# wenet-e2e/wesep

Hardware: AMD Instinct MI355X
Metric: utterances/sec (4 s, 16 kHz, 2-spk) fwd+bwd, pBSRNN (higher is better)
Workload: dtype bf16x3+fp16x2+fp16x1 split products (+fp8 lo terms), fp32 accumulate; 1 GPU; pBSRNN FiLM multi-fuse, 6 repeats, feature_dim 128, fixed 256-d embeddings; fwd + SI-SDR + bwd + per-tensor clip + Adam-L2; bf16x3 (x-projections, projections, d(hcat), BN / mask GEMMs) + fp16x2 (recurrent products of all four recurrence kernels, d(xn)) + fp16x1 (LSTM weight gradients); 2-byte saved gates / d(gates); fp32 accumulate; BPTT kernels: W_hh as fp16 hi + block-scaled FP8 lo; the lo term; rows_per_gpu=32, global_rows=32, samples_per_row=64000, parallelism=dp1

## Files before the change

### include/wesep_hip.h

```cpp
#ifndef WESEP_HIP_H_
#define WESEP_HIP_H_

#ifdef __cplusplus
extern "C" {
#endif

#define WS_ABI_VERSION 20
#define WS_OK 0
#define WS_ERR_INVALID (-1)
#define WS_ERR_LAUNCH (-2)

int ws_abi_version(void);
const char* ws_last_error(void);

#define WS_PROF_LSTM_FWD 0
#define WS_PROF_LSTM_BWD 1
#define WS_PROF_GEMM_NT 2
#define WS_PROF_GEMM_TN 3
#define WS_PROF_NKINDS 4
int ws_prof_enable(int on);
int ws_prof_collect(int kind, double* total_ms, long long* launches);
int ws_debug_dirty_lds(float value, int nblocks, int spins, float* sink, void* stream);
int ws_debug_occupy(int nblocks, int usec, const unsigned* stop, float* sink, void* stream);

// ... 123 lines not shown
                            float* pout, unsigned* counter, float* fslab, float* da, float* db, unsigned* fcounter,
                            void* stream);

typedef struct ws_lstm_args {
  float* gates;
  float* cbuf;
  float* hcat;
  const float* dhcat;
  const float* wpack;
  long long sq_s1, sq_s2, step_rows;
  int nseq, sq_div, L, mode;
  const unsigned* run_if;
  const float* gates_in;
  float* dgates;
  int gfmt;
  int rfmt;
  const unsigned* amax;
  float* dxn;
  long long dxn_dir_stride;
  const float* wxpack;
} ws_lstm_args;
#define WS_GATES_F32 0
#define WS_GATES_H2 1
#define WS_GATES_H2S 2
#define WS_GATES_H2F 3
#define WS_DGATES_EXP 8
#define WS_LSTM_F32_MT1 1
#define WS_LSTM_F32_MT2 2
#define WS_LSTM_BF16X3 3
#define WS_LSTM_BF16X3_BLK 4
#define WS_LSTM_BF16X3_BLK16 5
#define WS_LSTM_H 256
#define WS_LSTM_FWD_H2P 16
#define WS_LSTM_PACK_FLOATS (2 * 4 * WS_LSTM_H * WS_LSTM_H)
int ws_lstm_pack(const float* whh_f, const float* whh_r, float* pack_fwd, float* pack_bwd,
                 int mode, void* stream);
int ws_lstm_pack_bwd_f8(const float* whh_f, const float* whh_r, float* pack_bwd, void* stream);
#define WS_LSTM_DX_PACK_FLOATS (16 * (48 * 1024 + 64) / 4)
int ws_lstm_pack_dx_f8(const float* wcat, float* pack, void* stream);
int ws_lstm_fwd(const ws_lstm_args* a, void* stream);
int ws_lstm_bwd(const ws_lstm_args* a, void* stream);
typedef struct ws_lstm_cluster_args {
  float* gates;
  float* cbuf;
  float* hcat;
  const float* dhcat;
  const float* whh_f;
  const float* whh_r;
  void* xchg;
  unsigned* flags;
  unsigned* status;
  int nseq, L;
  int dbg, gfmt;
  const float* gates_in;
} ws_lstm_cluster_args;
int ws_lstm_fwd_cluster(const ws_lstm_cluster_args* a, void* stream);
typedef struct ws_lstm_cluster2_args {
  float* gates;
  float* cbuf;
  float* hcat;
  const float* xn;
  const float* wcat;
  const float* bcat;
  const float* whh_f;
  const float* whh_r;
  void* xchg;
// ... 433 lines not shown
```

### wesep_amd/_lib.py

```python
import ctypes as C
import os

import numpy as np
import torch

_HERE = os.path.dirname(os.path.abspath(__file__))
LIB_PATH = os.environ.get("WESEP_HIP_LIB") or os.path.join(_HERE, "libwesep_hip.so")

WS_OK = 0
PROF_LSTM_FWD, PROF_LSTM_BWD, PROF_GEMM_NT, PROF_GEMM_TN = 0, 1, 2, 3
LSTM_H = 256
ABI_VERSION = 20
GATES_F32, GATES_H2, GATES_H2S, GATES_H2F = 0, 1, 2, 3
DGATES_EXP = 8


def dgates_scale(amax_bits: int) -> float:
    e = (int(amax_bits) >> 23) & 0xFF
    return 1.0 if e in (0, 255) else 2.0 ** (min(max(DGATES_EXP + 254 - e, 1), 253) - 127)


LSTM_F32_MT1, LSTM_F32_MT2, LSTM_BF16X3, LSTM_BF16X3_BLK, LSTM_BF16X3_BLK16 = 1, 2, 3, 4, 5
LSTM_FWD_H2P = 16
LSTM_PACK_FLOATS = 2 * 4 * LSTM_H * LSTM_H

_p = C.c_void_p
_ll = C.c_longlong
_i = C.c_int
_f = C.c_float


class ConvView(C.Structure):
    _fields_ = [(n, _i) for n in ("on", "mode", "H", "W", "C", "Ho", "Wo", "k", "sh", "sw", "p", "dil", "ldp")]


class Conv3x3PackSrc(C.Structure):
    _fields_ = [("w", _p), ("s_row", _ll), ("s_col", _ll), ("s_tap", _ll), ("col_off", _i), ("cols", _i)]


class Conv3x3PackArgs(C.Structure):
    _fields_ = [("src", Conv3x3PackSrc * 5), ("out", _p), ("Cin", _i), ("Cout", _i), ("nsrc", _i), ("flip", _i)]


class Conv3x3Args(C.Structure):
    _fields_ = [(n, _p) for n in ("X", "W", "bias", "R", "Y")] + [(n, _ll) for n in ("ldx", "ldw", "ldy")] + \
               [(n, _i) for n in ("B", "H", "Wd", "Cin", "Cout", "pad_")]


class Conv3x3WgradArgs(C.Structure):
    _fields_ = [(n, _p) for n in ("G", "X", "slab", "bslab")] + [(n, _ll) for n in ("ldg", "ldx", "slab_stride", "bslab_stride")] + \
               [(n, _i) for n in ("B", "H", "Wd", "Wx", "sw", "Cin", "Nn", "nsplit", "tiles_per_split", "pad_")]


class HeadsArgs(C.Structure):
    _fields_ = [(n, _p) for n in ("x", "dy", "slope", "gamma", "beta", "y", "stats", "dx", "slab")] + \
               [(n, _ll) for n in ("ldx", "lddx")] + [(n, _i) for n in ("B", "T", "Tp", "Q", "nh", "ch", "nwg")] + \
# ... 331 lines not shown
```

### wesep_amd/blstm_core.py

```python
import math
import os
from typing import NamedTuple

import numpy as np
import torch

from . import _lib as L
from . import dev

H = L.LSTM_H
G4 = 4 * H
N = 128


def _empty(dev_, *shape):
    return torch.empty(*shape, device=dev_, dtype=torch.float32)


def _reduce_new(slab, nsplit, stride, shape):
    out = _empty(slab.device, *shape)
    dev.reduce_slabs(slab, nsplit, stride, int(np.prod(shape)), out)
    return out


# ... 295 lines not shown
            return out
        if kind in ("wihT", "wihT16", "wihT8"):
            out = _empty(d, N * 2 * G4)
            dev.pack_w(W("cat")[0], N, 2 * G4, N, out, trans=True, order=1, f16={"wihT": 0, "wihT16": 1, "wihT8": 2}[kind])
            return out
        if kind == "pw":
            return proj_w.contiguous()
        if kind in ("proj", "proj16"):
            out = _empty(d, N * 2 * H)
            dev.pack_w(W("pw"), N, 2 * H, 2 * H, out, order=1, f16=kind == "proj16")
            return out
        if kind == "projT":
            out = _empty(d, 2 * H * N)
            dev.pack_w(W("pw"), 2 * H, N, 2 * H, out, trans=True, order=0)
            return out
        raise KeyError(kind)


class BlstmPlan(NamedTuple):
    nb: int
    lmode: int
    cluster: bool
    fwd: str
    bptt: str
    grad: bool
    gfmt: int
    g_fmt: int
    a16: bool
    pair_rfmt: int
    band_rfmt: int
    band_dx: bool
    a_fmt: int
    h2p: bool = False


_WIHT_KIND = {0: "wihT", 1: "wihT", 2: "wihT16", 3: "wihT8"}


def make_plan(seq, device, grad, gn_geo=None, ragged=False) -> BlstmPlan:
    lmode = dev.lstm_blk_mode(seq.nseq)
    cluster = dev.lstm_cluster_ok(seq, device)
    bptt = _bptt_kind(seq, device, cluster)
    gfmt = L.GATES_F32 if bptt == "cluster" else dev.gates_fmt()
    h2 = gfmt != L.GATES_F32
    if ragged:
        fwd = "cluster" if cluster else "stream"
    elif dev.lstm_fuse_ok(seq.nseq, cluster):
        fwd = "fused"
    elif cluster:
        fwd = "cluster2" if h2 and dev.lstm_cluster2_on() else "cluster"
    else:
        fwd = "stream"
    g_fmt = {L.GATES_H2: 1, L.GATES_H2F: 2}.get(gfmt, 0)
    brf = band_rfmt(gfmt, lmode) if grad and bptt == "stream" else 0
    a16 = gfmt == L.GATES_H2F and grad and tnb_a16()
    h2p = (a16 and dev.h2p_on(device) and not ragged and fwd in ("fused", "cluster2", "stream")
           and (fwd != "fused" or bool(dev.lstm_fused_hfmt(gfmt) & 1)))
    return BlstmPlan(
        nb=dev.bl_num_blocks(seq), lmode=lmode, cluster=cluster, fwd=fwd, bptt=bptt, grad=grad, gfmt=gfmt, g_fmt=g_fmt,
        a16=a16, pair_rfmt=pair_rfmt(gfmt) if grad and bptt == "pair" else 0,
        band_rfmt=brf, band_dx=bool(brf) and gn_geo is not None and band_dx(brf, seq, gn_geo), a_fmt=dxn_fmt(g_fmt), h2p=h2p)


def consume_once(ctx, who):
    if ctx.consumed:
        raise L.WesepHipError(f"{who}: second backward through the same graph (retain_graph / multi-loss loops): "
                              "the blocked path consumes its saved gates in place; run the forward again")
    ctx.consumed = True


def blstm_forward(plan, W, x, seq, res, bias, norm=None, steps=None, film=None):
    d = x.device
    norm = dict(norm or {})
    if film is not None:
        if res is not x or steps is not None:
            raise L.WesepHipError("blstm_forward: film= folds ONE affine into operand and residual (res is x), no step counts")
        norm["film"] = film
    rk = dict(film=film) if film is not None else {}
    if steps is not None and (plan.fwd in ("fused", "cluster2") or plan.grad):
        raise L.WesepHipError(f"blstm_forward: per-sequence step counts with forward branch '{plan.fwd}', grad={plan.grad}: "
                              "only the branches over precomputed gates know them, and only the forward")
    lens = dict(steps=steps[0], steps_div=steps[1]) if steps is not None else {}
    nb, gfmt, lmode = plan.nb, plan.gfmt, plan.lmode
    h2 = gfmt != L.GATES_F32
    wcat, bcat = W("cat")
    whf, whr = W("whh")
    xn = _empty(d, nb, 32 * N)
    cbuf, hcat = _empty(d, nb, 32 * 2 * H), _empty(d, nb, 32 * 2 * H)
    gates = _empty(d, dev.blh_floats(nb, 2 * G4)) if h2 else _empty(d, nb, 32 * 2 * G4)
    xn16 = _empty(d, dev.blh_floats(nb, N)) if plan.a16 else None
    h2p = plan.h2p
    planes = dict(h2p=True) if h2p else {}
    hcat16 = _empty(d, dev.blh_floats(nb, 2 * H)) if plan.a16 and not h2p else None
    if plan.fwd == "fused":
        dev.gemm_p2b(A=x, lda=N, sm=seq, Wpack=None, N=0, C_out=None, A_bl=xn, A_bl16=xn16, **norm)
        hf = dev.lstm_fused_hfmt(gfmt)
        dev.lstm_fwd_fused(gates, cbuf, hcat, xn, W("fused8" if hf & 4 else "fused16" if hf else "fused"), bcat, seq, gfmt=gfmt,
                           hfmt=hf | (8 if h2p else 0))
    elif plan.fwd == "cluster2":
        dev.gemm_p2b(A=x, lda=N, sm=seq, Wpack=None, N=0, C_out=None, A_bl=xn, A_bl16=xn16, **norm)
        tw = dev.lstm_fwd_cluster2(gates, cbuf, hcat, xn, wcat, bcat, whf, whr, seq, dbg=_cluster_dbg(), **planes)
        pre = dev.fallback_scratch(d, nb * 32 * 2 * G4)
        dev.gemm_p2b(A=x, lda=N, sm=seq, Wpack=W("wih"), N=2 * G4, C_out=pre, bias=bcat, run_if=tw, **norm)
        dev.lstm_fwd(gates, cbuf, hcat, W("hh")[0], seq, lmode, run_if=tw, gfmt=gfmt, gates_in=pre, **planes)
        del pre
    else:
        pre = _empty(d, nb, 32 * 2 * G4) if h2 else gates
        xproj = dict(A=x, lda=N, sm=seq, Wpack=W("wih"), N=2 * G4, C_out=pre, bias=bcat, A_bl=xn, A_bl16=xn16, **norm, **lens)
        rec = dict(gfmt=gfmt, gates_in=pre) if h2 else {}
        dev.gemm_p2b(**xproj)
        if _h2_probe() & 768 and not torch.cuda.is_available():
            pre.copy_(pre.half().float() if _h2_probe() & 256 else pre.bfloat16().float())
        if plan.fwd == "cluster":
            tw = dev.lstm_fwd_cluster(gates, cbuf, hcat, whf, whr, seq, dbg=_cluster_dbg(), **rec)
            if not h2:
                dev.gemm_p2b(run_if=tw, **xproj)
            dev.lstm_fwd(gates, cbuf, hcat, W("hh")[0], seq, lmode, run_if=tw, **rec)
        else:
            dev.lstm_fwd(gates, cbuf, hcat, W("hh")[0], seq, lmode, **planes, **rec)
        del pre
    out = torch.empty_like(res)
    if h2p:
        dev.gemm_b2p(A=hcat, K=2 * H, sm=seq, Wpack=W("proj16"), C_out=out, ldc=N, bias=bias, R=res, a_fmt=4, **rk)
    else:
        dev.gemm_b2p(A=hcat, K=2 * H, sm=seq, Wpack=W("proj"), C_out=out, ldc=N, bias=bias, R=res, a16_out=hcat16, **rk)
    if _h2_probe() and not h2:
        if _h2_probe() & 1:
            _probe_round(gates, "f16")
        if _h2_probe() & 8:
            _probe_round(gates, "u16")
        if _h2_probe() & 4:
            _probe_round(cbuf, "f16")
    if plan.grad:
        W("projT")
        if not plan.band_dx:
            W(_WIHT_KIND[plan.a_fmt])
        if plan.bptt == "pair":
            W("hhp16" if plan.pair_rfmt else "hhp")
        if (plan.bptt == "stream" and not plan.band_rfmt) or (plan.bptt == "pair" and h2):
            W("hh")
        if plan.bptt == "stream" and plan.band_rfmt:
            W("hh8")
            if plan.band_dx:
                W("wx8")
    return out, (gates, cbuf, hcat, xn16 if plan.a16 else xn, hcat16)


def blstm_bptt(plan, W, gates, cbuf, hcat, dout, seq, release):
    d = dout.device
    nb, gfmt = plan.nb, plan.gfmt
    dh, dout_bl = _empty(d, nb, 32 * 2 * H), _empty(d, nb, 32 * N)
    dxn2 = None
    amax = amax_word(d) if gfmt == L.GATES_H2F else None
    dev.gemm_p2b(A=dout, lda=N, sm=seq, Wpack=W("projT"), N=2 * H, C_out=dh, A_bl=dout_bl, amax=amax)
    if _h2_probe() & 16:
        _probe_round(dh, "bf16")
    ready = mark_wgrads_ready(d) if release else None
    if plan.bptt == "cluster":
        dg = gates
        dev.lstm_bwd_cluster(gates, cbuf, dh, *W("whh"), seq)
    elif gfmt == L.GATES_F32:
        dg = gates
        if plan.bptt == "pair":
            dev.lstm_bwd_pair(gates, cbuf, dh, W("hhp"), seq, dbg=_pair_dbg())
        else:
            dev.lstm_bwd(gates, cbuf, hcat, dh, W("hh")[1], seq, plan.lmode)
    elif plan.bptt == "pair":
        dg = _empty(d, nb, 32 * 2 * G4) if gfmt == L.GATES_H2S else _empty(d, dev.blh_floats(nb, 2 * G4))
        rf = plan.pair_rfmt
        tw = dev.lstm_bwd_pair(gates, cbuf, dh, W("hhp16" if rf else "hhp"), seq, gfmt=gfmt, dgates=dg, repairable=True,
                               dbg=_pair_dbg(), amax=amax, rfmt=rf, dbg_buf=_pair_stamp_buf(d, seq.L))
        dev.lstm_bwd(gates, cbuf, hcat, dh, W("hh")[1], seq, plan.lmode, gfmt=gfmt, dgates=dg, run_if=tw, amax=amax)
    else:
        dg = _empty(d, nb, 32 * 2 * G4) if gfmt == L.GATES_H2S else gates
        brf = plan.band_rfmt
        if plan.band_dx:
            dxn2 = _empty(d, 2, dout.numel() // N, N)
        dev.lstm_bwd(gates, cbuf, hcat, dh, W("hh8") if brf else W("hh")[1], seq, plan.lmode, gfmt=gfmt,
                     dgates=dg if gfmt == L.GATES_H2S else None, amax=amax, rfmt=brf, dxn=dxn2,
                     wxpack=W("wx8") if dxn2 is not None else None)
    if _h2_probe() & 2 and gfmt == L.GATES_F32:
        _probe_round(gates, "bf16", packed=True)
    if _h2_probe() & 32 and gfmt == L.GATES_F32 and not torch.cuda.is_available():
        amax = float(dh.abs().max())
        S = 2.0 ** (10 - math.floor(math.log2(amax))) if amax > 0 and math.isfinite(amax) else 1.0
        sc = gates * S
        _PROBE_SAT[0] += int((sc.abs() > 65504.0).sum())
        _PROBE_SAT[1] = max(_PROBE_SAT[1], float(sc.abs().max()) / 65504.0)
        gates.copy_(sc.clamp(-65504.0, 65504.0).half().float() / S)
    if ready is not None:
        flush_deferred_wgrads(d, ready)
    return dg, dout_bl, amax, dxn2


def weight_grads(gates, xn, hcat, dout_bl, seq, nb, g_fmt=0, amax=None, hcat16=None, h2p=False):
    d = gates.device
    if h2p:
        hcat16 = dev.h2p_hi(hcat, nb)
    a_fmt = 1 if hcat16 is not None else 0
    if _h2_probe() & 192 and not torch.cuda.is_available() and not a_fmt:
        rnd = (lambda t: t.half().float()) if _h2_probe() & 64 else (lambda t: t.bfloat16().float())
        xn, hcat = rnd(xn), rnd(hcat)
    if os.environ.get("WESEP_PROBE_SKIP_WGRAD") == "1":
        z_ = lambda *s_: torch.zeros(*s_, device=d)
        return [z_(G4, N), z_(G4, H), z_(G4), z_(G4), z_(G4, N), z_(G4, H), z_(G4), z_(G4), z_(N, 2 * H), z_(N)]
    if _h2_probe() & 1024 and not torch.cuda.is_available() and amax is not None:
        S = L.dgates_scale(int(amax.reshape(-1)[0]))
        hcat = hcat.half().float()
        dout_bl = (dout_bl * S).half().float() / S
    ns, bps = dev.tnb_splits(nb, (2 * H) // 128)
    slab, aslab = _empty(d, ns, 2 * H * N), _empty(d, ns, N)
    if h2p:
        dev.gemm_tnb_h16(G=hcat16, g_width=2 * H, g_off=0, g_cols=2 * H, A0=dout_bl, a0_width=N, a0_off=0, nblk=nb, L_=seq.L,
# ... 45 lines not shown
```

### wesep_amd/csrc/lstm.hip

```cpp
#include "common.h"

#define LH WS_LSTM_H
#define LG (4 * LH)
#define HL_LD 68
#define DG_LD 260

__device__ __forceinline__ f32x4 mfma16(float a, float b, f32x4 c) {
  return __builtin_amdgcn_mfma_f32_16x16x4f32(a, b, c, 0, 0, 0);
}

__device__ __forceinline__ float fast_sigmoid(float x) {
  return __builtin_amdgcn_rcpf(1.f + __expf(-x));
}
__device__ __forceinline__ float fast_tanh(float x) {
  const float ax = fabsf(x);
  const float e = __expf(-2.f * ax);
  const float t = (1.f - e) * __builtin_amdgcn_rcpf(1.f + e);
  return copysignf(t, x);
}

__global__ void lstm_pack_kernel(const float* __restrict__ whh_f, const float* __restrict__ whh_r,
                                 float* __restrict__ pf, float* __restrict__ pb) {
  const int total = 2 * LG * LH;
  for (int idx = blockIdx.x * blockDim.x + threadIdx.x; idx < total; idx += gridDim.x * blockDim.x) {
// ... 316 lines not shown
      f32x4 a[MT];
#pragma unroll
      for (int mt = 0; mt < MT; ++mt)
        a[mt] = *reinterpret_cast<const f32x4*>(arow + mt * (64 * DG_LD) + 4 * ks4);
#pragma unroll
      for (int q = 0; q < 4; ++q)
#pragma unroll
        for (int s = 0; s < 2; ++s)
#pragma unroll
          for (int mt = 0; mt < MT; ++mt) dh[mt][s] = mfma16(a[mt][q], bcur[s][q], dh[mt][s]);
      bcur[0] = bnxt[0];
      bcur[1] = bnxt[1];
    }
    __syncthreads();
  }
}

static int lstm_check(const ws_lstm_args* a, bool bwd, const char* who) {
  WS_REQUIRE(a && a->gates && a->cbuf && a->hcat && a->wpack, "%s: null pointer", who);
  WS_REQUIRE(!bwd || a->dhcat, "%s: null dhcat", who);
  WS_REQUIRE(a->nseq > 0 && a->L > 0 && a->sq_div > 0, "%s: bad nseq/L/sq_div", who);
  WS_REQUIRE((a->mode & 255) >= WS_LSTM_F32_MT1 && (a->mode & 255) <= WS_LSTM_BF16X3_BLK16, "%s: bad mode %d", who,
             a->mode);
  WS_REQUIRE(!a->run_if || (!bwd && (a->mode & 255) >= WS_LSTM_BF16X3) || (bwd && (a->mode & 255) >= WS_LSTM_BF16X3_BLK),
             "%s: run_if is honoured by the split-bf16 forward kernels and the blocked-layout BPTT kernels only", who);
  WS_REQUIRE(a->gfmt >= WS_GATES_F32 && a->gfmt <= WS_GATES_H2F, "%s: bad gfmt %d", who, a->gfmt);
  WS_REQUIRE(a->gfmt != WS_GATES_H2F || !bwd || a->amax, "%s: WS_GATES_H2F needs amax", who);
  WS_REQUIRE(a->gfmt == WS_GATES_F32 || (a->mode & 255) >= WS_LSTM_BF16X3_BLK,
             "%s: gfmt %d is a format of the blocked-layout modes", who, a->gfmt);
  WS_REQUIRE(a->gfmt == WS_GATES_F32 || bwd || a->gates_in, "%s: gfmt %d needs gates_in (the fp32 pre-activations)", who,
             a->gfmt);
  WS_REQUIRE(a->gfmt != WS_GATES_H2S || !bwd || a->dgates, "%s: WS_GATES_H2S needs dgates", who);
  WS_REQUIRE(a->gfmt == WS_GATES_F32 || ((a->mode >> 8) & 7) == 0, "%s: probe builds are WS_GATES_F32 only", who);
  WS_REQUIRE(a->rfmt == 0 || ((a->rfmt == 2 || a->rfmt == 3) && bwd && a->mode == WS_LSTM_BF16X3_BLK && a->gfmt == WS_GATES_H2F) ||
                 (a->rfmt == WS_LSTM_FWD_H2P && !bwd && (a->mode == WS_LSTM_BF16X3_BLK || a->mode == WS_LSTM_BF16X3_BLK16)),
             "%s: rfmt %d (2 / 3 = fp16 recurrence on fp16 + FP8 weights, 3: the lo term on the FP8 MFMA: ws_lstm_bwd, "
             "WS_LSTM_BF16X3_BLK, WS_GATES_H2F only; 16 = hcat out as two fp16 planes: ws_lstm_fwd, blocked-layout modes only)",
             who, a->rfmt);
  WS_REQUIRE(!a->dxn || (bwd && a->rfmt == 2 && a->wxpack && a->dxn_dir_stride > 0 && a->dxn_dir_stride < (1ll << 29) && !a->run_if),
             "%s: dxn (d(xn) inside the BPTT, ABI v19) needs rfmt 2, wxpack (ws_lstm_pack_dx_f8), 0 < dxn_dir_stride < 2^29 floats "
             "(32-bit store offsets) and no run_if", who);
  return WS_OK;
}

extern "C" int ws_lstm_fwd(const ws_lstm_args* a, void* stream) {
  int rc = lstm_check(a, false, "ws_lstm_fwd");
  if (rc != WS_OK) return rc;
  hipStream_t s = (hipStream_t)stream;
  const int per = 16 * a->mode;
  dim3 grid((a->nseq + per - 1) / per, 2), block(512);
  const bool timed = a->run_if == nullptr;
  if (timed) ws_prof_begin(WS_PROF_LSTM_FWD, s);
  if ((a->mode & 255) == WS_LSTM_BF16X3_BLK16)
    ws_launch_lstm_fwd_s16(a, s);
  else if ((a->mode & 255) >= WS_LSTM_BF16X3)
    ws_launch_lstm_fwd_bf16(a, s);
  else if (a->mode == WS_LSTM_F32_MT1)
    hipLaunchKernelGGL((lstm_fwd_kernel<1>), grid, block, 0, s, *a);
  else
    hipLaunchKernelGGL((lstm_fwd_kernel<2>), grid, block, 0, s, *a);
  if (timed) ws_prof_end(WS_PROF_LSTM_FWD, s);
  return ws_check_launch("ws_lstm_fwd");
}

extern "C" int ws_lstm_bwd(const ws_lstm_args* a, void* stream) {
  int rc = lstm_check(a, true, "ws_lstm_bwd");
  if (rc != WS_OK) return rc;
  hipStream_t s = (hipStream_t)stream;
  const int per = 16 * a->mode;
  dim3 grid((a->nseq + per - 1) / per, 2), block(512);
  const bool timed = a->run_if == nullptr;
  if (timed) ws_prof_begin(WS_PROF_LSTM_BWD, s);
// ... 12 lines not shown
```

### wesep_amd/csrc/lstm_bf16.hip

```cpp
#include <stdlib.h>

#include "lstm_bf16_common.h"

__global__ void lstm_pack_bf16_kernel(const float* __restrict__ whh_f, const float* __restrict__ whh_r,
                                      __bf16* __restrict__ pf, __bf16* __restrict__ pb) {
  const int total = 2 * LG * LH;
  for (int idx = blockIdx.x * blockDim.x + threadIdx.x; idx < total; idx += gridDim.x * blockDim.x) {
    {
      int r = idx;
      const int j = r & 7; r >>= 3;
      const int lane = r & 63; r >>= 6;
      const int g = r & 3; r >>= 2;
      const int ks = r & 15; r >>= 4;
      const int w = r & 7; r >>= 3;
      const int d = r;
      const float* W = d ? whh_r : whh_f;
      const int row = g * 256 + 32 * w + (lane & 31);
      const int k = 16 * ks + 8 * (lane >> 5) + j;
      const float v = W[row * LH + k];
      const __bf16 hi = (__bf16)v;
      const long long unit = ((((long long)(d * 8 + w) * 16 + ks) * 4 + g) * 2) * 64 + lane;
      pf[unit * 8 + j] = hi;
      pf[(unit + 64) * 8 + j] = (__bf16)(v - (float)hi);
    }
// ... 82 lines not shown
    v0[i] = 256.f * W[row * 128 + u];
    v1[i] = 256.f * W[(row + 1) * 128 + u];
    m = fmaxf(m, fmaxf(fabsf(v0[i]), fabsf(v1[i])));
  }
#pragma unroll
  for (int o = 32; o > 0; o >>= 1) m = fmaxf(m, __shfl_xor(m, o));
  if ((tid & 63) == 0) red[tid >> 6] = m;
  __syncthreads();
  m = red[0];
#pragma unroll
  for (int i = 1; i < 8; ++i) m = fmaxf(m, red[i]);
  const int eb = (int)((__builtin_bit_cast(unsigned, m) >> 23) & 0xffu);
  const float S = (eb > 19 && eb < 255) ? __builtin_bit_cast(float, (unsigned)(eb - 19) << 23) : 1.f;
  char* ob = px + (long long)(d * 8 + w) * WS_DX_REGION;
  if (tid == 0) reinterpret_cast<float*>(ob + 48 * 1024)[grp] = S;
#pragma unroll
  for (int i = 0; i < 2; ++i) {
    const int pi = tid + 512 * i, j2 = pi & 3, lane = (pi >> 2) & 63, f = pi >> 8;
    const _Float16 h0 = (_Float16)v0[i], h1 = (_Float16)v1[i];
    typedef _Float16 f16x2 __attribute__((ext_vector_type(2)));
    typedef short s16x2 __attribute__((ext_vector_type(2)));
    char* cb = ob + (2 * grp + (f >> 1)) * 3072;
    *reinterpret_cast<f16x2*>(cb + (f & 1) * 1024 + lane * 16 + j2 * 4) = f16x2{h0, h1};
    const s16x2 c = __builtin_amdgcn_cvt_scalef32_pk_fp8_f32(s16x2{0, 0}, v0[i] - (float)h0, v1[i] - (float)h1, S, false);
    *reinterpret_cast<short*>(cb + 2048 + (f & 1) * 512 + lane * 8 + j2 * 2) = c[0];
  }
}

int ws_launch_lstm_pack_dx_f8(const float* wcat, float* pack, hipStream_t s) {
  hipLaunchKernelGGL(lstm_pack_dx_f8_kernel, dim3(128), dim3(512), 0, s, wcat, reinterpret_cast<char*>(pack));
  return 0;
}

template <bool BLK, int DBG, int GF = 0, bool H2P = false>
__global__ __launch_bounds__(512, 2) void lstm_fwd_bf16_kernel(const ws_lstm_args p) {
  static_assert(!H2P || (BLK && DBG == 0), "the fp16 planes are a format of the blocked layout");
  __shared__ __attribute__((aligned(16))) __bf16 hl[2][2][SQ * HROW];
  __shared__ __attribute__((aligned(16))) float cl[SQ * (LH + 4)];
  if (p.run_if && *p.run_if == 0u) return;
  const int d = blockIdx.y;
  const int tid = threadIdx.x, lane = tid & 63, l31 = lane & 31, half = lane >> 5;
  const int w = __builtin_amdgcn_readfirstlane(tid >> 6);
  const int L = p.L;

  {
    uint32_t* z = reinterpret_cast<uint32_t*>(&hl[0][0][0]);
    for (int i = tid; i < 2 * SQ * HROW / 2; i += 512) z[i] = 0u;
  }
  const int ss = min((int)blockIdx.x * SQ + l31, p.nseq - 1);
  const long long rowbase =
      BLK ? 0 : (long long)(ss / p.sq_div) * p.sq_s1 + (long long)(ss % p.sq_div) * p.sq_s2;
  const int ubase = 32 * w + 4 * half;
  const int glane = ((d * 256 + 8 * w + half) * 32 + l31) * 16;
  const int clane = ((d * 64 + 8 * w + half) * 32 + l31) * 16;
  auto goff = [&](int t, int g, int j) -> long long {
    return ((rowbase + (long long)t * p.step_rows) * 2 + d) * LG + g * 256 + ubase + 8 * j;
  };
  auto coff = [&](int t, int j) -> long long {
    return (rowbase + (long long)t * p.step_rows) * (2 * LH) + d * LH + ubase + 8 * j;
  };
  const float* gsrc = GF ? p.gates_in : p.gates;
  auto grs = [&](int t) { return mkrsrc(gsrc + (long long)(blockIdx.x * L + t) * (SQ * 2 * LG), SQ * 2 * LG * 4); };
  auto hrs = [&](int t) { return mkrsrc(p.gates + (long long)(blockIdx.x * L + t) * (SQ * LG), SQ * 2 * LG * 2); };
  auto crs = [&](float* b, int t) { return mkrsrc(b + (long long)(blockIdx.x * L + t) * (SQ * 2 * LH), SQ * 2 * LH * 4); };
  const char* hplane = reinterpret_cast<const char*>(p.hcat);
  const long long hlo_off = ws_h2p_plane((long long)gridDim.x * L);
  auto prs = [&](int t, int pl) {
    return mkrsrc(reinterpret_cast<const float*>(hplane + pl * hlo_off + (long long)(blockIdx.x * L + t) * (SQ * 2 * LH * 2)),
                  SQ * 2 * LH * 2);
  };
  auto ld_gate = [&](int t, int g, int j) -> f32x4 {
    if constexpr (BLK) return bld(grs(t), glane, (g * 64 + 2 * j) * 512);
    else return *reinterpret_cast<const f32x4*>(p.gates + goff(t, g, j));
  };
  auto st_gate = [&](const f32x4& v, int t, int g, int j) {
    if constexpr (GF != 0) bst8(g == 2 ? enc_u16x4<true>(v) : enc_u16x4<false>(v), hrs(t), glane >> 1, (g * 64 + 2 * j) * 256);
    else if constexpr (BLK) bst(v, grs(t), glane, (g * 64 + 2 * j) * 512);
    else *reinterpret_cast<f32x4*>(p.gates + goff(t, g, j)) = v;
  };
  auto st_ch = [&](const f32x4& v, float* b, int t, int j) {
    if constexpr (BLK) bst(v, crs(b, t), clane, 2 * j * 512);
    else *reinterpret_cast<f32x4*>(b + coff(t, j)) = v;
  };

  float* cme = &cl[l31 * (LH + 4) + ubase];
#pragma unroll
  for (int j = 0; j < 4; ++j) *reinterpret_cast<f32x4*>(cme + 8 * j) = f32x4{0.f, 0.f, 0.f, 0.f};

  const __amdgpu_buffer_rsrc_t wrs = __builtin_amdgcn_make_buffer_rsrc(
      const_cast<float*>(p.wpack) + (long long)(d * 8 + w) * (16 * 8 * 64 * 4), 0, 16 * 8 * 1024, 0x00020000);
  const int wlane = lane * 16;
  bf16x8 wr[2][8];
#pragma unroll
  for (int s = 0; s < 2; ++s)
#pragma unroll
    for (int f = 0; f < 8; ++f) wr[s][f] = wload(wrs, wlane + (f & 3) * 1024, s * 8192 + (f >> 2) * 4096);

  f32x4 xg[4][4];
  {
    const int t0 = d == 0 ? 0 : L - 1;
#pragma unroll
    for (int gi = 0; gi < 4; ++gi)
#pragma unroll
// ... 55 lines not shown
#pragma unroll
    for (int j = 0; j < 4; ++j) {
      f32x4 pre[4];
#pragma unroll
      for (int g = 0; g < 4; ++g)
#pragma unroll
        for (int r = 0; r < 4; ++r) pre[g][r] = acc[g][4 * j + r];
      f32x4 vi, vf, vg, vo, vc, vh;
      const f32x4 cold = *reinterpret_cast<const f32x4*>(cme + 8 * j);
#pragma unroll
      for (int r = 0; r < 4; ++r) {
        const float ig = fsig(pre[0][r]);
        const float fg = fsig(pre[1][r]);
        const float gg = ftanh(pre[2][r]);
        const float og = fsig(pre[3][r]);
        const float cn = fg * cold[r] + ig * gg;
        vi[r] = ig;
        vf[r] = fg;
        vg[r] = gg;
        vo[r] = og;
        vc[r] = cn;
        vh[r] = og * ftanh(cn);
      }
      bf16x4 h_hi, h_lo;
      split4(vh, h_hi, h_lo);
      *reinterpret_cast<bf16x4*>(nhi + 8 * j) = h_hi;
      *reinterpret_cast<bf16x4*>(nlo + 8 * j) = h_lo;
      *reinterpret_cast<f32x4*>(cme + 8 * j) = vc;
      if (!(DBG & 1) || step == L - 1) {
        st_gate(vi, t, 0, j);
        st_gate(vf, t, 1, j);
        st_gate(vg, t, 2, j);
        st_gate(vo, t, 3, j);
        st_ch(vc, p.cbuf, t, j);
        if constexpr (H2P) {
          u32x2 ph, pl;
          enc_h2p(vh, ph, pl);
          bst8(ph, prs(t, 0), clane >> 1, j * 512);
          bst8(pl, prs(t, 1), clane >> 1, j * 512);
        } else if constexpr (BLK) st_ch(pack_hl4(h_hi, h_lo), p.hcat, t, j);
        else st_ch(vh, p.hcat, t, j);
      }
      __builtin_amdgcn_sched_barrier(0);
    }
    __syncthreads();
  }
}

template <bool BLK, int DBG, int GF = 0, int RF = 0, bool DX = false>
__global__ __launch_bounds__(512, 2) void lstm_bwd_bf16_kernel(const ws_lstm_args p) {
  static_assert(RF == 0 || (BLK && GF == WS_GATES_H2F), "the fp16 recurrence takes the scaled-fp16 d(gates) of WS_GATES_H2F");
  static_assert(!DX || RF == 2, "d(xn) in the BPTT rides on the fp16 d(gates) image of rfmt 2");
  __shared__ __attribute__((aligned(16))) __bf16 dgl[RF ? 1 : 2][SQ * DROW];
  __shared__ __attribute__((aligned(16))) f32x4 xred[DX ? 8 * 2 * 64 : 1];
  if (p.run_if && *p.run_if == 0u) return;
  const int d = blockIdx.y, bx = blockIdx.x;
  const int tid = threadIdx.x, lane = tid & 63, l31 = lane & 31, half = lane >> 5;
  const int w = __builtin_amdgcn_readfirstlane(tid >> 6);
  const int L = p.L;
  const int ss = min(bx * SQ + l31, p.nseq - 1);
  const long long rowbase =
      BLK ? 0 : (long long)(ss / p.sq_div) * p.sq_s1 + (long long)(ss % p.sq_div) * p.sq_s2;
  const int ubase = 32 * w + 4 * half;
  const int glane = ((d * 256 + 8 * w + half) * 32 + l31) * 16;
  const int clane = ((d * 64 + 8 * w + half) * 32 + l31) * 16;
  auto goff = [&](int t, int g, int j) -> long long {
    return ((rowbase + (long long)t * p.step_rows) * 2 + d) * LG + g * 256 + ubase + 8 * j;
  };
  auto coff = [&](int t, int j) -> long long {
    return (rowbase + (long long)t * p.step_rows) * (2 * LH) + d * LH + ubase + 8 * j;
  };
  float* gdst = GF == WS_GATES_H2S ? p.dgates : p.gates;
  auto grs = [&](int t) { return mkrsrc(gdst + (long long)(bx * L + t) * (SQ * 2 * LG), SQ * 2 * LG * 4); };
  auto hrs = [&](int t) { return mkrsrc(p.gates + (long long)(bx * L + t) * (SQ * LG), SQ * 2 * LG * 2); };
  constexpr bool G2 = GF == WS_GATES_H2 || GF == WS_GATES_H2F;
  float* hdst = (G2 && p.dgates) ? p.dgates : p.gates;
  auto ors = [&](int t) { return mkrsrc(hdst + (long long)(bx * L + t) * (SQ * LG), SQ * 2 * LG * 2); };
  const float dS = GF == WS_GATES_H2F ? ws_dgates_scale(*p.amax) : 1.f;
  auto crs = [&](const float* b, int t) { return mkrsrc(b + (long long)(bx * L + t) * (SQ * 2 * LH), SQ * 2 * LH * 4); };
  typedef typename gate_cell<GF>::type gcell;
  auto ld_gate = [&](int t, int g, int j) -> gcell {
    if constexpr (GF != 0) return bld8(hrs(t), glane >> 1, (g * 64 + 2 * j) * 256);
    else if constexpr (BLK) return bld(grs(t), glane, (g * 64 + 2 * j) * 512);
    else return *reinterpret_cast<const f32x4*>(p.gates + goff(t, g, j));
  };
  auto st_gate = [&](const f32x4& v, int t, int g, int j) {
    if constexpr (BLK) bst(v, grs(t), glane, (g * 64 + 2 * j) * 512);
    else *reinterpret_cast<f32x4*>(p.gates + goff(t, g, j)) = v;
  };
  auto ld_ch = [&](const float* b, int t, int j) -> f32x4 {
    if constexpr (BLK) return bld(crs(b, t), clane, 2 * j * 512);
    else return *reinterpret_cast<const f32x4*>(b + coff(t, j));
  };

  const int kpar = DX ? (w >> 2) : 0;
  const __amdgpu_buffer_rsrc_t wrs = __builtin_amdgcn_make_buffer_rsrc(
      const_cast<float*>(p.wpack) + (long long)(d * 8 + w) * (64 * 2 * 64 * 4), 0, 64 * 2 * 1024, 0x00020000);
  const int wlane = lane * 16;
  bf16x8 wr[2][RF ? 4 : 8];
  u32x2 wq[2][RF ? 4 : 1];
  float wS[RF ? 8 : 1];
  int wE[RF == 3 ? 8 : 1];
  auto wfill = [&](int s, int chunk, int zo) {
    if constexpr (RF != 0) {
#pragma unroll
      for (int q = 0; q < 4; ++q) {
        const int fq = q ^ kpar;
        wr[s][q] = wload(wrs, wlane, zo + chunk * 6144 + fq * 1024);
        wq[s][q] = __builtin_bit_cast(u32x2, __builtin_amdgcn_raw_buffer_load_b64(wrs, lane * 8, zo + chunk * 6144 + 4096 + fq * 512, 0));
      }
    } else {
#pragma unroll
      for (int f = 0; f < 8; ++f) wr[s][f] = wload(wrs, wlane + (f & 3) * 1024, zo + chunk * 8192 + (f >> 2) * 4096);
    }
  };
  typedef _Float16 f16x8 __attribute__((ext_vector_type(8)));
  typedef _Float16 f16x2 __attribute__((ext_vector_type(2)));
  const __amdgpu_buffer_rsrc_t xrs = __builtin_amdgcn_make_buffer_rsrc(
      const_cast<char*>(reinterpret_cast<const char*>(p.wxpack)) + (DX ? (long long)(d * 8 + w) * WS_DX_REGION : 0), 0,
      DX ? WS_DX_REGION : 0, 0x00020000);
  bf16x8 xr[2][DX ? 2 : 1];
  u32x2 xq[2][DX ? 2 : 1];
  float xS[DX ? 8 : 1];
  f32x16 dxa;
  auto xfill = [&](int s, int chunk, int zo) {
    if constexpr (DX) {
#pragma unroll
      for (int q = 0; q < 2; ++q) {
        xr[s][q] = wload(xrs, wlane + q * 1024, zo + chunk * 3072);
        xq[s][q] = __builtin_bit_cast(u32x2, __builtin_amdgcn_raw_buffer_load_b64(xrs, lane * 8 + q * 512, zo + chunk * 3072 + 2048, 0));
      }
    }
  };
  if constexpr (RF != 0) {
    const float* st = p.wpack + (long long)(d * 8 + w) * (64 * 2 * 64 * 4) + 96 * 256;
#pragma unroll
    for (int g8 = 0; g8 < 8; ++g8) wS[g8] = __builtin_bit_cast(float, __builtin_amdgcn_readfirstlane(__builtin_bit_cast(int, st[g8])));
    if constexpr (RF == 3) {
#pragma unroll
      for (int g8 = 0; g8 < 8; ++g8) wE[g8] = (__builtin_bit_cast(int, wS[g8]) >> 23) & 255;
    }
  }
  if constexpr (DX) {
    const float* st = reinterpret_cast<const float*>(reinterpret_cast<const char*>(p.wxpack) + (long long)(d * 8 + w) * WS_DX_REGION + 48 * 1024);
#pragma unroll
    for (int g8 = 0; g8 < 8; ++g8) xS[g8] = __builtin_bit_cast(float, __builtin_amdgcn_readfirstlane(__builtin_bit_cast(int, st[g8])));
  }
  unsigned xoff = 0u;
  if constexpr (DX) {
    const int sq = bx * SQ + l31;
    const long long row = (long long)(sq / p.sq_div) * p.sq_s1 + (long long)(sq % p.sq_div) * p.sq_s2;
    xoff = sq < p.nseq ? (unsigned)(row * 512 + (32 * (w & 3) + 16 * kpar + 4 * half) * 4) : 0x80000000u;
  }
  const __amdgpu_buffer_rsrc_t xors = __builtin_amdgcn_make_buffer_rsrc(
      DX ? p.dxn + (long long)d * p.dxn_dir_stride : nullptr, 0, DX ? (unsigned)(p.dxn_dir_stride * 4) : 0u, 0x00020000);
  gcell n_i[4], n_f[4], n_g[4], n_o[4];
  f32x4 n_dh[4], n_cp[4], c_cur[4], dc[4];
  f32x16 dhr;
  const f32x4 zero4v = {0.f, 0.f, 0.f, 0.f};
#pragma unroll
  for (int j = 0; j < 4; ++j) dc[j] = zero4v;
#pragma unroll
  for (int i = 0; i < 16; ++i) dhr[i] = 0.f;

  auto load_step = [&](int t, int j) {
    n_i[j] = ld_gate(t, 0, j);
    n_f[j] = ld_gate(t, 1, j);
    n_g[j] = ld_gate(t, 2, j);
    n_o[j] = ld_gate(t, 3, j);
    n_dh[j] = ld_ch(p.dhcat, t, j);
    const int tp = d == 0 ? max(t - 1, 0) : min(t + 1, L - 1);
    n_cp[j] = ld_ch(p.cbuf, tp, j);
  };
  {
    const int t0 = d == 0 ? L - 1 : 0;
#pragma unroll
    for (int j = 0; j < 4; ++j) {
      load_step(t0, j);
      c_cur[j] = ld_ch(p.cbuf, t0, j);
    }
  }
  __builtin_amdgcn_sched_barrier(0);
  wfill(0, 0, 0);
  xfill(0, 0, 0);
  wfill(1, 1, 0);
  xfill(1, 1, 0);
  __builtin_amdgcn_sched_barrier(0);

  for (int step = 0; step < L; ++step) {
    const int t = d == 0 ? L - 1 - step : step;
    const int sn = min(step + 1, L - 1);
    const int tn = d == 0 ? L - 1 - sn : sn;
    const bool has_prev = d == 0 ? (t > 0) : (t < L - 1);
    int zo = 0;
    asm volatile("" : "+s"(zo));
    __bf16* dhi = &dgl[0][l31 * DROW + ubase];
    __bf16* dlo = &dgl[RF ? 0 : 1][l31 * DROW + ubase];
#pragma unroll
    for (int j = 0; j < 4; ++j) {
      f32x4 pi, pf, pg, po;
      const f32x4 vi = gate_val<false>(n_i[j]), vf = gate_val<false>(n_f[j]), vg = gate_val<true>(n_g[j]),
                  vo = gate_val<false>(n_o[j]);
#pragma unroll
      for (int r = 0; r < 4; ++r) {
        const float ig = vi[r], fg = vf[r], gg = vg[r], og = vo[r];
        const float dhv = dh_in<GF>(n_dh[j][r], dhr[4 * j + r], dS);
        const float tc = ftanh(c_cur[j][r]);
        const float dov = dhv * tc;
        const float dcv = dc[j][r] + dhv * og * (1.f - tc * tc);
        dc[j][r] = dcv * fg;
        pi[r] = dcv * gg * ig * (1.f - ig);
        pf[r] = dcv * (has_prev ? n_cp[j][r] : 0.f) * fg * (1.f - fg);
        pg[r] = dcv * ig * (1.f - gg * gg);
        po[r] = dov * og * (1.f - og);
      }
      c_cur[j] = n_cp[j];
      const bool st = !(DBG & 1) || step == L - 1;
      auto emit = [&](const f32x4& v, int g) {
        if constexpr (RF != 0) {
          const u32x2 code = enc_f16x4(v);
          *reinterpret_cast<u32x2*>(dhi + 256 * g + 8 * j) = code;
          if (st) bst8(code, ors(t), glane >> 1, (g * 64 + 2 * j) * 256);
          return;
        }
        bf16x4 hi, lo;
        split4(v, hi, lo);
        *reinterpret_cast<bf16x4*>(dhi + 256 * g + 8 * j) = hi;
        *reinterpret_cast<bf16x4*>(dlo + 256 * g + 8 * j) = lo;
        if (st) {
          if constexpr (G2) bst8(enc_dgates<GF>(v, hi), ors(t), glane >> 1, (g * 64 + 2 * j) * 256);
          else if constexpr (BLK) st_gate(pack_hl4(hi, lo), t, g, j);
          else st_gate(v, t, g, j);
        }
      };
      emit(pi, 0);
      emit(pf, 1);
      emit(pg, 2);
      emit(po, 3);
      if (!(DBG & 2)) load_step(tn, j);
      __builtin_amdgcn_sched_barrier(0);
    }
    __syncthreads();

    const __bf16* bhi = &dgl[0][l31 * DROW + 8 * half];
    const __bf16* blo = &dgl[RF ? 0 : 1][l31 * DROW + 8 * half];
// ... 98 lines not shown
    if constexpr (DX) {
      const float us = (1.f / 256.f) / dS;
      const unsigned trow = (unsigned)t * (unsigned)p.step_rows * 512u;
#pragma unroll
      for (int i = 0; i < 2; ++i) {
        const f32x4 o = xred[((w ^ 4) * 2 + i) * 64 + lane];
        __builtin_amdgcn_raw_buffer_store_b128(__builtin_bit_cast(u32x4, (keep[i] + o) * us), xors, xoff + trow + 32 * i, 0, 0);
      }
    }
  }
}

#define WS_DBG_DISPATCH(KERNEL)                                                          \
  if ((a->mode & 255) == WS_LSTM_BF16X3_BLK && a->gfmt == WS_GATES_H2) {                 \
    hipLaunchKernelGGL((KERNEL<true, 0, WS_GATES_H2>), grid, block, 0, s, *a);           \
  } else if ((a->mode & 255) == WS_LSTM_BF16X3_BLK && a->gfmt == WS_GATES_H2S) {         \
    hipLaunchKernelGGL((KERNEL<true, 0, WS_GATES_H2S>), grid, block, 0, s, *a);          \
  } else if ((a->mode & 255) == WS_LSTM_BF16X3_BLK && a->gfmt == WS_GATES_H2F) {         \
    hipLaunchKernelGGL((KERNEL<true, 0, WS_GATES_H2F>), grid, block, 0, s, *a);          \
  } else if ((a->mode & 255) == WS_LSTM_BF16X3_BLK) {                                    \
    switch ((a->mode >> 8) & 7) {                                                        \
      case 0: hipLaunchKernelGGL((KERNEL<true, 0>), grid, block, 0, s, *a); break;       \
      case 1: hipLaunchKernelGGL((KERNEL<true, 1>), grid, block, 0, s, *a); break;       \
      case 2: hipLaunchKernelGGL((KERNEL<true, 2>), grid, block, 0, s, *a); break;       \
      case 4: hipLaunchKernelGGL((KERNEL<true, 4>), grid, block, 0, s, *a); break;       \
      default: hipLaunchKernelGGL((KERNEL<true, 7>), grid, block, 0, s, *a); break;      \
    }                                                                                    \
  } else {                                                                               \
    hipLaunchKernelGGL((KERNEL<false, 0>), grid, block, 0, s, *a);                       \
  }

int ws_launch_lstm_fwd_bf16(const ws_lstm_args* a, hipStream_t s) {
  dim3 grid((a->nseq + SQ - 1) / SQ, 2), block(512);
  if (a->rfmt == WS_LSTM_FWD_H2P) {
    if (a->gfmt == WS_GATES_H2) hipLaunchKernelGGL((lstm_fwd_bf16_kernel<true, 0, WS_GATES_H2, true>), grid, block, 0, s, *a);
    else if (a->gfmt == WS_GATES_H2S) hipLaunchKernelGGL((lstm_fwd_bf16_kernel<true, 0, WS_GATES_H2S, true>), grid, block, 0, s, *a);
    else if (a->gfmt == WS_GATES_H2F) hipLaunchKernelGGL((lstm_fwd_bf16_kernel<true, 0, WS_GATES_H2F, true>), grid, block, 0, s, *a);
    else hipLaunchKernelGGL((lstm_fwd_bf16_kernel<true, 0, 0, true>), grid, block, 0, s, *a);
    return 0;
  }
  WS_DBG_DISPATCH(lstm_fwd_bf16_kernel)
  return 0;
}

int ws_launch_lstm_bwd_bf16(const ws_lstm_args* a, hipStream_t s) {
  dim3 grid((a->nseq + SQ - 1) / SQ, 2), block(512);
  if (a->rfmt == 2 && a->dxn) {
    hipLaunchKernelGGL((lstm_bwd_bf16_kernel<true, 0, WS_GATES_H2F, 2, true>), grid, block, 0, s, *a);
    return 0;
  }
  if (a->rfmt == 2) {
    hipLaunchKernelGGL((lstm_bwd_bf16_kernel<true, 0, WS_GATES_H2F, 2>), grid, block, 0, s, *a);
    return 0;
  }
  if (a->rfmt == 3) {
    hipLaunchKernelGGL((lstm_bwd_bf16_kernel<true, 0, WS_GATES_H2F, 3>), grid, block, 0, s, *a);
    return 0;
  }
  WS_DBG_DISPATCH(lstm_bwd_bf16_kernel)
  return 0;
}
```

### wesep_amd/csrc/lstm_bf16_common.h

```cpp
#pragma once
#include "common.h"

typedef __bf16 bf16x8 __attribute__((ext_vector_type(8)));
typedef __bf16 bf16x4 __attribute__((ext_vector_type(4)));

#define LH WS_LSTM_H
#define LG (4 * LH)
#define SQ 32
#define HROW 264
#define DROW 1032

typedef unsigned int u32x4 __attribute__((ext_vector_type(4)));

__device__ __forceinline__ bf16x8 wload(__amdgpu_buffer_rsrc_t rsrc, int voff, int soff) {
  return __builtin_bit_cast(bf16x8, __builtin_amdgcn_raw_buffer_load_b128(rsrc, voff, soff, 0));
}

__device__ __forceinline__ __amdgpu_buffer_rsrc_t mkrsrc(const float* base, unsigned bytes) {
  return __builtin_amdgcn_make_buffer_rsrc(const_cast<float*>(base), 0, bytes, 0x00020000);
}
#ifndef WS_STREAM_AUX
#define WS_STREAM_AUX 2
#endif
__device__ __forceinline__ f32x4 bld(__amdgpu_buffer_rsrc_t r, int voff, int soff) {
// ... 79 lines not shown
}
template <bool TANH>
__device__ __forceinline__ f32x4 dec_u16x4(const u32x2& c) {
  const float s = TANH ? 1.f / WS_U16_TANH : 1.f / WS_U16_SIG, o = TANH ? -1.f : 0.f;
  f32x4 v;
  v[0] = __builtin_fmaf((float)(c[0] & 0xffffu), s, o);
  v[1] = __builtin_fmaf((float)(c[0] >> 16), s, o);
  v[2] = __builtin_fmaf((float)(c[1] & 0xffffu), s, o);
  v[3] = __builtin_fmaf((float)(c[1] >> 16), s, o);
  return v;
}
__device__ __forceinline__ u32x2 bf16x4_bits(const bf16x4& v) { return __builtin_bit_cast(u32x2, v); }
typedef _Float16 f16x4 __attribute__((ext_vector_type(4)));
__device__ __forceinline__ u32x2 enc_f16x4(const f32x4& vs) {
  f16x4 h;
#pragma unroll
  for (int j = 0; j < 4; ++j) h[j] = (_Float16)vs[j];
  return __builtin_bit_cast(u32x2, h);
}
__device__ __forceinline__ void enc_h2p(const f32x4& vh, u32x2& hi, u32x2& lo) {
  f16x4 h, l;
#pragma unroll
  for (int j = 0; j < 4; ++j) {
    float x = vh[j];
    asm volatile("" : "+v"(x));
    h[j] = (_Float16)x;
    l[j] = (_Float16)(x - (float)h[j]);
  }
  hi = __builtin_bit_cast(u32x2, h);
  lo = __builtin_bit_cast(u32x2, l);
}
__device__ __forceinline__ long long ws_h2p_plane(long long nblk) { return nblk * (SQ * 2 * LH * 2); }

template <int GF>
__device__ __forceinline__ u32x2 enc_dgates(const f32x4& v, const bf16x4& hi) {
  if constexpr (GF == WS_GATES_H2F) return enc_f16x4(v);
  else return bf16x4_bits(hi);
}
template <int GF>
__device__ __forceinline__ float dh_in(float dh, float rec, float S) {
  if constexpr (GF == WS_GATES_H2F) return __builtin_fmaf(dh, S, rec);
  else return dh + rec;
}

template <int GF> struct gate_cell { typedef f32x4 type; };
template <> struct gate_cell<WS_GATES_H2> { typedef u32x2 type; };
template <> struct gate_cell<WS_GATES_H2S> { typedef u32x2 type; };
template <> struct gate_cell<WS_GATES_H2F> { typedef u32x2 type; };
template <bool TANH> __device__ __forceinline__ f32x4 gate_val(const f32x4& c) { return c; }
template <bool TANH> __device__ __forceinline__ f32x4 gate_val(const u32x2& c) { return dec_u16x4<TANH>(c); }
```

### wesep_amd/csrc/lstm_bf16_s16.hip

```cpp
#include "lstm_bf16_common.h"

#define S16 16

__device__ __forceinline__ f32x4 mfma16(bf16x8 a, bf16x8 b, f32x4 c) {
  return __builtin_amdgcn_mfma_f32_16x16x32_bf16(a, b, c, 0, 0, 0);
}

__global__ void lstm_pack_s16_kernel(const float* __restrict__ whh_f, const float* __restrict__ whh_r,
                                     __bf16* __restrict__ pf, __bf16* __restrict__ pb) {
  const int total = 2 * LG * LH;
  for (int idx = blockIdx.x * blockDim.x + threadIdx.x; idx < total; idx += gridDim.x * blockDim.x) {
    {
      int r = idx;
      const int j = r & 7; r >>= 3;
      const int lane = r & 63; r >>= 6;
      const int tile = r & 7; r >>= 3;
      const int ks = r & 7; r >>= 3;
      const int w = r & 7; r >>= 3;
      const int d = r;
      const float* W = d ? whh_r : whh_f;
      const int row = (tile >> 1) * 256 + 32 * w + 16 * (tile & 1) + (lane & 15);
      const int k = 32 * ks + 8 * (lane >> 4) + j;
      const float v = W[row * LH + k];
      const __bf16 hi = (__bf16)v;
      const long long unit = ((((long long)(d * 8 + w) * 8 + ks) * 8 + tile) * 2) * 64 + lane;
      pf[unit * 8 + j] = hi;
      pf[(unit + 64) * 8 + j] = (__bf16)(v - (float)hi);
    }
    {
      int r = idx;
      const int j = r & 7; r >>= 3;
      const int lane = r & 63; r >>= 6;
      const int tu = r & 1; r >>= 1;
      const int ks = r & 31; r >>= 5;
      const int w = r & 7; r >>= 3;
      const int d = r;
      const float* W = d ? whh_r : whh_f;
      const int row = 32 * ks + 8 * (lane >> 4) + j;
      const int u = 32 * w + 16 * tu + (lane & 15);
      const float v = W[row * LH + u];
      const __bf16 hi = (__bf16)v;
      const long long unit = ((((long long)(d * 8 + w) * 32 + ks) * 2 + tu) * 2) * 64 + lane;
      pb[unit * 8 + j] = hi;
      pb[(unit + 64) * 8 + j] = (__bf16)(v - (float)hi);
    }
  }
}

int ws_launch_lstm_pack_s16(const float* whh_f, const float* whh_r, float* pack_fwd, float* pack_bwd,
                            hipStream_t s) {
  hipLaunchKernelGGL(lstm_pack_s16_kernel, dim3(512), dim3(256), 0, s, whh_f, whh_r,
                     reinterpret_cast<__bf16*>(pack_fwd), reinterpret_cast<__bf16*>(pack_bwd));
  return 0;
}

template <int GF, bool H2P = false>
__global__ __launch_bounds__(512, 2) void lstm_fwd_s16_kernel(const ws_lstm_args p) {
  __shared__ __attribute__((aligned(16))) __bf16 hl[2][2][S16 * HROW];
  __shared__ __attribute__((aligned(16))) float cl[S16 * (LH + 4)];
  if (p.run_if && *p.run_if == 0u) return;
  const int d = blockIdx.y;
  const int tile = blockIdx.x >> 1, hb = blockIdx.x & 1;
  const int tid = threadIdx.x, lane = tid & 63, n = lane & 15, mq = lane >> 4;
  const int w = __builtin_amdgcn_readfirstlane(tid >> 6);
  const int L = p.L;
  {
    uint32_t* z = reinterpret_cast<uint32_t*>(&hl[0][0][0]);
    for (int i = tid; i < 2 * S16 * HROW / 2; i += 512) z[i] = 0u;
  }
  const int glane = ((d * 256 + 8 * w + mq) * 32 + 16 * hb + n) * 16;
  const int clane = ((d * 64 + 8 * w + mq) * 32 + 16 * hb + n) * 16;
  const float* gsrc = GF ? p.gates_in : p.gates;
  auto grs = [&](int t) { return mkrsrc(gsrc + (long long)(tile * L + t) * (SQ * 2 * LG), SQ * 2 * LG * 4); };
  auto hrs = [&](int t) { return mkrsrc(p.gates + (long long)(tile * L + t) * (SQ * LG), SQ * 2 * LG * 2); };
  auto crs = [&](float* b, int t) { return mkrsrc(b + (long long)(tile * L + t) * (SQ * 2 * LH), SQ * 2 * LH * 4); };
  auto ld_gate = [&](int t, int g, int tu) -> f32x4 { return bld(grs(t), glane, (g * 64 + 4 * tu) * 512); };
  auto st_gate = [&](const f32x4& v, int t, int g, int tu) {
    if constexpr (GF != 0) bst8(g == 2 ? enc_u16x4<true>(v) : enc_u16x4<false>(v), hrs(t), glane >> 1, (g * 64 + 4 * tu) * 256);
    else bst(v, grs(t), glane, (g * 64 + 4 * tu) * 512);
  };
  auto st_ch = [&](const f32x4& v, float* b, int t, int tu) { bst(v, crs(b, t), clane, 4 * tu * 512); };
  const char* hplane = reinterpret_cast<const char*>(p.hcat);
  const long long hlo_off = ws_h2p_plane((long long)(gridDim.x >> 1) * L);
  auto prs = [&](int t, int pl) {
    return mkrsrc(reinterpret_cast<const float*>(hplane + pl * hlo_off + (long long)(tile * L + t) * (SQ * 2 * LH * 2)), SQ * 2 * LH * 2);
  };

  const int ubase = 32 * w + 4 * mq;
  float* cme = &cl[n * (LH + 4) + ubase];
#pragma unroll
  for (int tu = 0; tu < 2; ++tu) *reinterpret_cast<f32x4*>(cme + 16 * tu) = f32x4{0.f, 0.f, 0.f, 0.f};

  const __amdgpu_buffer_rsrc_t wrs = __builtin_amdgcn_make_buffer_rsrc(
      const_cast<float*>(p.wpack) + (long long)(d * 8 + w) * (8 * 16 * 64 * 4), 0, 8 * 16 * 1024, 0x00020000);
  const int wlane = lane * 16;
  bf16x8 wr[2][16];
#pragma unroll
  for (int s = 0; s < 2; ++s)
#pragma unroll
    for (int f = 0; f < 16; ++f) wr[s][f] = wload(wrs, wlane + (f & 3) * 1024, s * 16384 + (f >> 2) * 4096);

  f32x4 xg[4][2];
  {
    const int t0 = d == 0 ? 0 : L - 1;
#pragma unroll
    for (int g = 0; g < 4; ++g)
#pragma unroll
      for (int tu = 0; tu < 2; ++tu) xg[g][tu] = ld_gate(t0, g, tu);
  }
  __syncthreads();

  for (int step = 0; step < L; ++step) {
    const int t = d == 0 ? step : L - 1 - step;
    const int cur = step & 1;
    int zo = 0;
    asm volatile("" : "+s"(zo));
    const __bf16* hhi = &hl[cur][0][n * HROW + 8 * mq];
    const __bf16* hlo = &hl[cur][1][n * HROW + 8 * mq];
    f32x4 acc[4][2];
// ... 39 lines not shown
    for (int tu = 0; tu < 2; ++tu)
#pragma unroll
      for (int g = 0; g < 4; ++g) xg[g][tu] = ld_gate(tn, g, tu);
    __builtin_amdgcn_sched_barrier(0);
    __bf16* nhi = &hl[cur ^ 1][0][n * HROW + ubase];
    __bf16* nlo = &hl[cur ^ 1][1][n * HROW + ubase];
#pragma unroll
    for (int tu = 0; tu < 2; ++tu) {
      f32x4 vi, vf, vg, vo, vc, vh;
      const f32x4 cold = *reinterpret_cast<const f32x4*>(cme + 16 * tu);
#pragma unroll
      for (int r = 0; r < 4; ++r) {
        const float ig = fsig(acc[0][tu][r]);
        const float fg = fsig(acc[1][tu][r]);
        const float gg = ftanh(acc[2][tu][r]);
        const float og = fsig(acc[3][tu][r]);
        const float cn = fg * cold[r] + ig * gg;
        vi[r] = ig;
        vf[r] = fg;
        vg[r] = gg;
        vo[r] = og;
        vc[r] = cn;
        vh[r] = og * ftanh(cn);
      }
      bf16x4 h_hi, h_lo;
      split4(vh, h_hi, h_lo);
      *reinterpret_cast<bf16x4*>(nhi + 16 * tu) = h_hi;
      *reinterpret_cast<bf16x4*>(nlo + 16 * tu) = h_lo;
      *reinterpret_cast<f32x4*>(cme + 16 * tu) = vc;
      st_gate(vi, t, 0, tu);
      st_gate(vf, t, 1, tu);
      st_gate(vg, t, 2, tu);
      st_gate(vo, t, 3, tu);
      st_ch(vc, p.cbuf, t, tu);
      if constexpr (H2P) {
        u32x2 ph, pl;
        enc_h2p(vh, ph, pl);
        bst8(ph, prs(t, 0), clane >> 1, 2 * tu * 512);
        bst8(pl, prs(t, 1), clane >> 1, 2 * tu * 512);
      } else {
        st_ch(pack_hl4(h_hi, h_lo), p.hcat, t, tu);
      }
      __builtin_amdgcn_sched_barrier(0);
    }
    __syncthreads();
  }
}


#ifndef S16_DBG
#define S16_DBG 0
#endif
template <int GF>
__global__ __launch_bounds__(512, 2) void lstm_bwd_s16_kernel(const ws_lstm_args p) {
  __shared__ __attribute__((aligned(16))) __bf16 dgl[2][S16 * DROW];
  if (p.run_if && *p.run_if == 0u) return;
  const int d = blockIdx.y;
  const int tile = blockIdx.x >> 1, hb = blockIdx.x & 1;
  const int tid = threadIdx.x, lane = tid & 63, n = lane & 15, mq = lane >> 4;
  const int w = __builtin_amdgcn_readfirstlane(tid >> 6);
  const int L = p.L;
  const int glane = ((d * 256 + 8 * w + mq) * 32 + 16 * hb + n) * 16;
  const int clane = ((d * 64 + 8 * w + mq) * 32 + 16 * hb + n) * 16;
  float* gdst = GF == WS_GATES_H2S ? p.dgates : p.gates;
  auto grs = [&](int t) { return mkrsrc(gdst + (long long)(tile * L + t) * (SQ * 2 * LG), SQ * 2 * LG * 4); };
  auto hrs = [&](int t) { return mkrsrc(p.gates + (long long)(tile * L + t) * (SQ * LG), SQ * 2 * LG * 2); };
  constexpr bool G2 = GF == WS_GATES_H2 || GF == WS_GATES_H2F;
  float* hdst = (G2 && p.dgates) ? p.dgates : p.gates;
  auto ors = [&](int t) { return mkrsrc(hdst + (long long)(tile * L + t) * (SQ * LG), SQ * 2 * LG * 2); };
  const float dS = GF == WS_GATES_H2F ? ws_dgates_scale(*p.amax) : 1.f;
  auto crs = [&](const float* b, int t) { return mkrsrc(b + (long long)(tile * L + t) * (SQ * 2 * LH), SQ * 2 * LH * 4); };
  typedef typename gate_cell<GF>::type gcell;
  auto ld_gate = [&](int t, int g, int tu) -> gcell {
    if constexpr (GF != 0) return bld8(hrs(t), glane >> 1, (g * 64 + 4 * tu) * 256);
    else return bld(grs(t), glane, (g * 64 + 4 * tu) * 512);
  };
  auto st_gate = [&](const f32x4& v, int t, int g, int tu) { bst(v, grs(t), glane, (g * 64 + 4 * tu) * 512); };
  auto ld_ch = [&](const float* b, int t, int tu) -> f32x4 { return bld(crs(b, t), clane, 4 * tu * 512); };
  const int ubase = 32 * w + 4 * mq;

  const __amdgpu_buffer_rsrc_t wrs = __builtin_amdgcn_make_buffer_rsrc(
      const_cast<float*>(p.wpack) + (long long)(d * 8 + w) * (32 * 4 * 64 * 4), 0, 32 * 4 * 1024, 0x00020000);
  const int wlane = lane * 16;
  bf16x8 wr[2][16];
#pragma unroll
  for (int s = 0; s < 2; ++s)
#pragma unroll
    for (int f = 0; f < 16; ++f) wr[s][f] = wload(wrs, wlane + (f & 3) * 1024, s * 16384 + (f >> 2) * 4096);

  gcell n_i[2], n_f[2], n_g[2], n_o[2];
  f32x4 n_dh[2], n_cp[2], c_cur[2], dc[2], dhr[2];
  const f32x4 zero4v = {0.f, 0.f, 0.f, 0.f};
#pragma unroll
  for (int tu = 0; tu < 2; ++tu) dc[tu] = dhr[tu] = zero4v;
  auto load_step = [&](int t, int tu) {
    n_i[tu] = ld_gate(t, 0, tu);
    n_f[tu] = ld_gate(t, 1, tu);
    n_g[tu] = ld_gate(t, 2, tu);
    n_o[tu] = ld_gate(t, 3, tu);
    n_dh[tu] = ld_ch(p.dhcat, t, tu);
    const int tp = d == 0 ? max(t - 1, 0) : min(t + 1, L - 1);
    n_cp[tu] = ld_ch(p.cbuf, tp, tu);
  };
  {
    const int t0 = d == 0 ? L - 1 : 0;
#pragma unroll
    for (int tu = 0; tu < 2; ++tu) {
      load_step(t0, tu);
      c_cur[tu] = ld_ch(p.cbuf, t0, tu);
    }
  }

  for (int step = 0; step < L; ++step) {
    const int t = d == 0 ? L - 1 - step : step;
    const int sn = min(step + 1, L - 1);
    const int tn = d == 0 ? L - 1 - sn : sn;
    const bool has_prev = d == 0 ? (t > 0) : (t < L - 1);
    int zo = 0;
    asm volatile("" : "+s"(zo));
    __bf16* dhi = &dgl[0][n * DROW + ubase];
    __bf16* dlo = &dgl[1][n * DROW + ubase];
#pragma unroll
    for (int tu = 0; tu < 2; ++tu) {
      f32x4 pi, pf, pg, po;
      const f32x4 vi = gate_val<false>(n_i[tu]), vf = gate_val<false>(n_f[tu]), vg = gate_val<true>(n_g[tu]),
                  vo = gate_val<false>(n_o[tu]);
#pragma unroll
      for (int r = 0; r < 4; ++r) {
        const float ig = vi[r], fg = vf[r], gg = vg[r], og = vo[r];
        const float dhv = dh_in<GF>(n_dh[tu][r], dhr[tu][r], dS);
        const float tc = ftanh(c_cur[tu][r]);
        const float dov = dhv * tc;
        const float dcv = dc[tu][r] + dhv * og * (1.f - tc * tc);
        dc[tu][r] = dcv * fg;
        pi[r] = dcv * gg * ig * (1.f - ig);
        pf[r] = dcv * (has_prev ? n_cp[tu][r] : 0.f) * fg * (1.f - fg);
        pg[r] = dcv * ig * (1.f - gg * gg);
        po[r] = dov * og * (1.f - og);
      }
      c_cur[tu] = n_cp[tu];
      auto emit = [&](const f32x4& v, int g) {
        bf16x4 hi, lo;
        split4(v, hi, lo);
        *reinterpret_cast<bf16x4*>(dhi + 256 * g + 16 * tu) = hi;
        *reinterpret_cast<bf16x4*>(dlo + 256 * g + 16 * tu) = lo;
        if constexpr (G2) bst8(enc_dgates<GF>(v, hi), ors(t), glane >> 1, (g * 64 + 4 * tu) * 256);
        else if (!(S16_DBG & 2)) st_gate(pack_hl4(hi, lo), t, g, tu);
      };
      emit(pi, 0);
      emit(pf, 1);
      emit(pg, 2);
      emit(po, 3);
      if (!(S16_DBG & 1)) load_step(tn, tu);
      __builtin_amdgcn_sched_barrier(0);
    }
    __syncthreads();

    const __bf16* bhi = &dgl[0][n * DROW + 8 * mq];
    const __bf16* blo = &dgl[1][n * DROW + 8 * mq];
    f32x4 acc[2];
#pragma unroll
    for (int ch = 0; ch < 8; ++ch) {
      const int s = ch & 1;
#pragma unroll
      for (int q = 0; q < 4; ++q) {
        const int ks = 4 * ch + q;
        const bf16x8 bh = *reinterpret_cast<const bf16x8*>(bhi + 32 * ks);
        const bf16x8 bl = *reinterpret_cast<const bf16x8*>(blo + 32 * ks);
#pragma unroll
        for (int tu = 0; tu < 2; ++tu) {
          const int f = (q * 2 + tu) * 2;
          if (ks == 0)
            acc[tu] = mfma16(wr[s][f], bh, zero4v);
          else
            acc[tu] = mfma16(wr[s][f], bh, acc[tu]);
        }
#pragma unroll
        for (int tu = 0; tu < 2; ++tu) acc[tu] = mfma16(wr[s][(q * 2 + tu) * 2 + 1], bh, acc[tu]);
#pragma unroll
        for (int tu = 0; tu < 2; ++tu) acc[tu] = mfma16(wr[s][(q * 2 + tu) * 2], bl, acc[tu]);
      }
      const int cn = (ch + 2) & 7;
      if (!(S16_DBG & 4)) {
#pragma unroll
      for (int f = 0; f < 16; ++f)
        wr[s][f] = wload(wrs, wlane + (f & 3) * 1024, zo + cn * 16384 + (f >> 2) * 4096);
      }
      __builtin_amdgcn_sched_barrier(0);
    }
    dhr[0] = acc[0];
    dhr[1] = acc[1];
    __syncthreads();
  }
}

int ws_launch_lstm_fwd_s16(const ws_lstm_args* a, hipStream_t s) {
  dim3 grid(2 * ((a->nseq + SQ - 1) / SQ), 2), block(512);
  const bool h2p = a->rfmt == WS_LSTM_FWD_H2P;
  if (a->gfmt && h2p) hipLaunchKernelGGL((lstm_fwd_s16_kernel<WS_GATES_H2, true>), grid, block, 0, s, *a);
  else if (h2p) hipLaunchKernelGGL((lstm_fwd_s16_kernel<0, true>), grid, block, 0, s, *a);
  else if (a->gfmt) hipLaunchKernelGGL(lstm_fwd_s16_kernel<WS_GATES_H2>, grid, block, 0, s, *a);
  else hipLaunchKernelGGL(lstm_fwd_s16_kernel<0>, grid, block, 0, s, *a);
  return 0;
}

int ws_launch_lstm_bwd_s16(const ws_lstm_args* a, hipStream_t s) {
  dim3 grid(2 * ((a->nseq + SQ - 1) / SQ), 2), block(512);
  if (a->gfmt == WS_GATES_H2) hipLaunchKernelGGL(lstm_bwd_s16_kernel<WS_GATES_H2>, grid, block, 0, s, *a);
  else if (a->gfmt == WS_GATES_H2S) hipLaunchKernelGGL(lstm_bwd_s16_kernel<WS_GATES_H2S>, grid, block, 0, s, *a);
  else if (a->gfmt == WS_GATES_H2F) hipLaunchKernelGGL(lstm_bwd_s16_kernel<WS_GATES_H2F>, grid, block, 0, s, *a);
  else hipLaunchKernelGGL(lstm_bwd_s16_kernel<0>, grid, block, 0, s, *a);
  return 0;
}
```

### wesep_amd/csrc/lstm_cluster2.hip

```cpp
#include "lstm_bf16_common.h"

typedef __attribute__((address_space(1))) unsigned gu32;
#define SC1 16
#define C2_SEQ 64
#define C2_SPIN_LIMIT (1u << 15)
#define C2_TAGS 0x40004000u

__device__ __forceinline__ void split8h(const f32x4& a, const f32x4& b, f16x8& hi, f16x8& lo) {
  const float v[8] = {a[0], a[1], a[2], a[3], b[0], b[1], b[2], b[3]};
#pragma unroll
  for (int j = 0; j < 8; ++j) {
    const float s = 256.f * v[j];
    hi[j] = (_Float16)s;
    lo[j] = (_Float16)(s - (float)hi[j]);
  }
}

__device__ __forceinline__ void split8b(const f32x4& a, const f32x4& b, bf16x8& hi, bf16x8& lo) {
  const float v[8] = {a[0], a[1], a[2], a[3], b[0], b[1], b[2], b[3]};
#pragma unroll
  for (int j = 0; j < 8; ++j) {
    const float s = 256.f * v[j];
    hi[j] = (__bf16)s;
    lo[j] = (__bf16)(s - (float)hi[j]);
// ... 92 lines not shown
      split8h(*reinterpret_cast<const f32x4*>(wr + 16 * ks), *reinterpret_cast<const f32x4*>(wr + 16 * ks + 4), wh[ks], wl[ks]);
  }
  {
    const float* xr = p.wcat + ((long long)d * LG + wrow) * 128 + 8 * half;
#pragma unroll
    for (int q = 0; q < 4; ++q) {
      const int ks = 4 * st + q;
      bf16x8 hi, lo;
      split8b(*reinterpret_cast<const f32x4*>(xr + 16 * ks), *reinterpret_cast<const f32x4*>(xr + 16 * ks + 4), hi, lo);
      wih[((uo * 2 + 0) * 8 + ks) * 64 + lane] = hi;
      wih[((uo * 2 + 1) * 8 + ks) * 64 + lane] = lo;
    }
  }
  if (tid < 128)
    reinterpret_cast<float*>(bias_l)[tid] = 256.f * p.bcat[(long long)d * LG + (tid >> 5) * LH + 32 * j + (tid & 31)];
  {
    uint32_t* z = reinterpret_cast<uint32_t*>(hl);
    for (int i = tid; i < C2_SEQ * HROW / 2; i += 512) z[i] = 0u;
    if (tid == 0) dead_s = 0;
  }
  const int mt = tid & 255;
  const int m_uo = (mt >> 6) & 3, m_n = mt & 31, m_half = (mt >> 5) & 1;
  const int gvo = ((d * 256 + 8 * j + 2 * m_uo + m_half) * 32 + m_n) * 16;
  const int cvo = ((d * 64 + 8 * j + 2 * m_uo + m_half) * 32 + m_n) * 16;
  const int gts = (int)(L * gblk * 4), cts = (int)(L * cblk * 4);
  auto hrs = [&](int t) { return mkrsrc(p.gates + ((long long)2 * cc * L + t) * (gblk / 2), 0x7fffffffu); };
  auto crs = [&](float* b, int t) { return mkrsrc(b + ((long long)2 * cc * L + t) * cblk, 0x7fffffffu); };
  const bool h2p = (p.rfmt & 2) != 0;
  const char* hplane = reinterpret_cast<const char*>(p.hcat);
  const long long hlo_off = ws_h2p_plane((long long)ntile * L);
  auto prs = [&](int t, int pl) {
    return mkrsrc(reinterpret_cast<const float*>(hplane + pl * hlo_off + ((long long)2 * cc * L + t) * (cblk * 2)), 0x7fffffffu);
  };
  const char* xbase = reinterpret_cast<const char*>(p.xn);
  auto xld = [&](int t, int q) -> f32x4 {
    const long long blk = (long long)(2 * cc + st) * L + t;
    return bld(mkrsrc(reinterpret_cast<const float*>(xbase + blk * 16384), 16384), (mt + 256 * q) * 16, 0);
  };
  const __amdgpu_buffer_rsrc_t xrs = __builtin_amdgcn_make_buffer_rsrc(
      reinterpret_cast<char*>(p.xchg) + (long long)c * (2 * 8 * 4096), 0, 2 * 8 * 4096, 0x00020000);
  const int mycell = ((w * 32 + n) * 2 + half) * 8;
  unsigned* tword = p.tword;

  auto step_time = [&](int s) { return d == 0 ? s : L - 1 - s; };
  f32x16 acc0;
  auto xpart = [&]() {
#pragma unroll
    for (int q = 0; q < 4; ++q) {
      const f32x4 b4 = bias_l[q * 8 + 2 * uo + half];
      acc0[4 * q] = b4[0], acc0[4 * q + 1] = b4[1], acc0[4 * q + 2] = b4[2], acc0[4 * q + 3] = b4[3];
    }
    const f32x4* xc = xb + st * 1024 + n;
    const bf16x8* wa = &wih[(uo * 2) * 8 * 64 + lane];
#pragma unroll
    for (int ks = 0; ks < 8; ++ks) {
      bf16x4 h0, l0, h1, l1;
      unpack_hl4(xc[(4 * ks + 2 * half) * 32], h0, l0);
      unpack_hl4(xc[(4 * ks + 2 * half + 1) * 32], h1, l1);
      const bf16x8 bh = __builtin_shufflevector(h0, h1, 0, 1, 2, 3, 4, 5, 6, 7);
      const bf16x8 bl = __builtin_shufflevector(l0, l1, 0, 1, 2, 3, 4, 5, 6, 7);
      acc0 = mfma32(wa[ks * 64], bh, acc0);
      acc0 = mfma32(wa[(8 + ks) * 64], bh, acc0);
      acc0 = mfma32(wa[ks * 64], bl, acc0);
    }
  };

  f32x4 c4 = {0.f, 0.f, 0.f, 0.f};
  f32x4 xreg[4];
#pragma unroll
  for (int q = 0; q < 4; ++q) xb[st * 1024 + mt + 256 * q] = xld(step_time(0), q);
  __syncthreads();
  xpart();
#pragma unroll
  for (int q = 0; q < 4; ++q) xreg[q] = xld(step_time(min(1, L - 1)), q);
  __syncthreads();

  auto hbm_out = [&](int tprev) {
#pragma unroll
    for (int e = 0; e < 2; ++e) {
      const int ct = mt + 256 * e;
#pragma unroll
      for (int g2 = 0; g2 < 2; ++g2) {
        const u32x4 pr = __builtin_bit_cast(u32x4, outl[g2][ct]);
        bst8(u32x2{pr[0], pr[1]}, hrs(tprev), (gvo + e * gts) >> 1, (2 * g2) * 64 * 256);
        bst8(u32x2{pr[2], pr[3]}, hrs(tprev), (gvo + e * gts) >> 1, (2 * g2 + 1) * 64 * 256);
      }
      bst(e == 0 ? c4 : outc[mt], crs(p.cbuf, tprev), cvo + e * cts, 0);
      if (h2p) {
        const u32x4 hc = __builtin_bit_cast(u32x4, outl[2][ct]);
        bst8(u32x2{hc[0], hc[1]}, prs(tprev, 0), (cvo + e * cts) >> 1, 0);
        bst8(u32x2{hc[2], hc[3]}, prs(tprev, 1), (cvo + e * cts) >> 1, 0);
      } else {
        bst(outl[2][ct], crs(p.hcat, tprev), cvo + e * cts, 0);
      }
    }
  };

  for (int step = 0; step < L; ++step) {
    const int par = step & 1;
    const unsigned tag = ((step >> 1) & 1) ? C2_TAGS : 0u;
    C2TS(0);
#pragma unroll
    for (int q = 0; q < 4; ++q) xb[st * 1024 + mt + 256 * q] = xreg[q];
    {
      const int t2 = step_time(min(step + 2, L - 1));
#pragma unroll
      for (int q = 0; q < 4; ++q) xreg[q] = xld(t2, q);
    }
    C2TS(7);
    {
      const _Float16* hb = &hl[(st * 32 + n) * HROW + 8 * half];
      v8i b8;
#pragma unroll
      for (int ks = 0; ks < 16; ++ks) {
        const f16x8 b = *reinterpret_cast<const f16x8*>(hb + 16 * ks);
        acc0 = mfma16h(wh[ks], b, acc0);
        if constexpr (F8) {
          typedef _Float16 f16x2 __attribute__((ext_vector_type(2)));
          typedef short s16x2 __attribute__((ext_vector_type(2)));
#pragma unroll
// ... 76 lines not shown
      }
      C2TS(5);
      _Float16* hrow = &hl[(((mt >> 7) & 1) * 32 + (mt & 31)) * HROW + 8 * ((mt >> 5) & 3)];
#pragma unroll
      for (int jj = 0; jj < 8; ++jj) {
        u32x4 v = pv[jj];
        v[0] &= ~C2_TAGS, v[1] &= ~C2_TAGS, v[2] &= ~C2_TAGS, v[3] &= ~C2_TAGS;
        *reinterpret_cast<u32x4*>(hrow + 32 * jj) = v;
      }
      C2TS(6);
    }
    __syncthreads();
  }
  if (xrole) hbm_out(step_time(L - 1));
}

extern "C" int ws_lstm_fwd_cluster2(const ws_lstm_cluster2_args* a, void* stream) {
  WS_REQUIRE(a && a->gates && a->cbuf && a->hcat && a->xn && a->wcat && a->bcat && a->whh_f && a->whh_r && a->xchg &&
                 a->tword,
             "ws_lstm_fwd_cluster2: null pointer");
  WS_REQUIRE(a->nseq > 0 && a->nseq % 64 == 0 && a->L > 0, "ws_lstm_fwd_cluster2: nseq must be a multiple of 64");
  const int ncl = a->nseq / 32, nwg = ncl * 8;
  int dev = 0, cus = 0;
  (void)hipGetDevice(&dev);
  (void)hipDeviceGetAttribute(&cus, hipDeviceAttributeMultiprocessorCount, dev);
  WS_REQUIRE(nwg <= cus, "ws_lstm_fwd_cluster2: %d workgroups must be co-resident but the device has %d CUs", nwg, cus);
  const int grid = 64 * ((ncl + 7) / 8);
  hipStream_t s = (hipStream_t)stream;
  hipError_t e = hipMemsetAsync(a->xchg, 0x40, (size_t)ncl * (2 * 8 * 4096), s);
  WS_REQUIRE(e == hipSuccess, "ws_lstm_fwd_cluster2: hipMemsetAsync failed");
  e = hipMemsetAsync(a->tword, 0, sizeof(unsigned), s);
  WS_REQUIRE(e == hipSuccess, "ws_lstm_fwd_cluster2: hipMemsetAsync failed");
  ws_prof_begin(WS_PROF_LSTM_FWD, s);
  WS_REQUIRE((a->rfmt & ~3) == 0,
             "ws_lstm_fwd_cluster2: rfmt %d (bit 0: the lo term of W_hh on the FP8 MFMA; bit 1: hcat out as two fp16 planes)", a->rfmt);
  if (a->rfmt & 1) {
    if (a->dbg & 2048) hipLaunchKernelGGL((lstm_fwd_cluster2_kernel<false, true, true>), dim3(grid), dim3(512), 0, s, *a);
    else if (a->dbg & 8) hipLaunchKernelGGL((lstm_fwd_cluster2_kernel<true, false, true>), dim3(grid), dim3(512), 0, s, *a);
    else hipLaunchKernelGGL((lstm_fwd_cluster2_kernel<false, false, true>), dim3(grid), dim3(512), 0, s, *a);
  } else if (a->dbg & 2048) hipLaunchKernelGGL((lstm_fwd_cluster2_kernel<false, true>), dim3(grid), dim3(512), 0, s, *a);
  else if (a->dbg & 8) hipLaunchKernelGGL((lstm_fwd_cluster2_kernel<true>), dim3(grid), dim3(512), 0, s, *a);
  else hipLaunchKernelGGL((lstm_fwd_cluster2_kernel<false>), dim3(grid), dim3(512), 0, s, *a);
  ws_prof_end(WS_PROF_LSTM_FWD, s);
  return ws_check_launch("ws_lstm_fwd_cluster2");
}
```

### wesep_amd/csrc/lstm_fused.hip

```cpp
#include <stdlib.h>

#include "lstm_bf16_common.h"

#define XROW 136
#define FKS 24
#define H8ROW 272

template <bool H16>
__global__ void lstm_pack_fused_kernel(const float* __restrict__ wih_f, const float* __restrict__ wih_r,
                                       const float* __restrict__ whh_f, const float* __restrict__ whh_r,
                                       __bf16* __restrict__ pf) {
  const int total = 2 * 8 * FKS * 4 * 64 * 8;
  for (int idx = blockIdx.x * blockDim.x + threadIdx.x; idx < total; idx += gridDim.x * blockDim.x) {
    int r = idx;
    const int j = r & 7; r >>= 3;
    const int lane = r & 63; r >>= 6;
    const int g = r & 3; r >>= 2;
    const int ks = r % FKS; r /= FKS;
    const int w = r & 7; r >>= 3;
    const int d = r;
    const int row = g * 256 + 32 * w + (lane & 31);
    float v;
    if (ks < 8) {
      const float* W = d ? wih_r : wih_f;
// ... 75 lines not shown
  for (int j = 0; j < 32; ++j) {
    const float s = 256.f * W[(j >> 4) * 32 + (j & 15)];
    res[j] = s - (float)(_Float16)s;
    mx = fmaxf(mx, fabsf(res[j]));
  }
#pragma unroll
  for (int o = 32; o >= 1; o >>= 1) mx = fmaxf(mx, __shfl_xor(mx, o));
  int E = 0;
  if (mx > 0.f) E = ((__float_as_int(mx) >> 23) & 255) - 127 - 7;
  E = max(E, -126);
  const float inv = __int_as_float((127 - E) << 23);
  unsigned char* reg = pk + (long long)(d * 8 + w) * F8_REGION;
  unsigned int* o = reinterpret_cast<unsigned int*>(reg + F8_HPART + q * F8_KSTEP + 4096 + lane * 16);
#pragma unroll
  for (int j = 0; j < 32; j += 4) {
    int v = 0;
    v = __builtin_amdgcn_cvt_pk_fp8_f32(res[j] * inv, res[j + 1] * inv, v, false);
    v = __builtin_amdgcn_cvt_pk_fp8_f32(res[j + 2] * inv, res[j + 3] * inv, v, true);
    o[(j >> 4) * 256 + ((j & 15) >> 2)] = (unsigned int)v;
  }
  if (lane == 0) reg[F8_SCALES + q] = (unsigned char)(127 + E);
}

extern "C" int ws_lstm_pack_fused_h8(const float* wih_f, const float* wih_r, const float* whh_f, const float* whh_r,
                                     float* pack, void* stream) {
  WS_REQUIRE(wih_f && wih_r && whh_f && whh_r && pack, "ws_lstm_pack_fused_h8: null pointer");
  static_assert(2 * 8 * F8_REGION <= WS_LSTM_FUSED_PACK_FLOATS * 4, "the F8 stream fits the pack of the other formats");
  unsigned char* pk = reinterpret_cast<unsigned char*>(pack);
  hipLaunchKernelGGL(lstm_pack_fused_h8_hi_kernel, dim3(512), dim3(256), 0, (hipStream_t)stream, wih_f, wih_r, whh_f, whh_r, pk);
  hipLaunchKernelGGL(lstm_pack_fused_h8_lo_kernel, dim3(2 * 8 * 16), dim3(64), 0, (hipStream_t)stream, whh_f, whh_r, pk);
  return ws_check_launch("ws_lstm_pack_fused_h8");
}

template <int GF, bool H16 = false, bool F8 = false, bool H2P = false>
__global__ __launch_bounds__(512, 1) void lstm_fwd_fused_kernel(const ws_lstm_fused_args p) {
  static_assert(!F8 || H16, "the FP8 lo term belongs to the fp16-h kernel");
  static_assert(!H2P || H16, "the fp16 planes are written by the fp16-h kernels");
  __shared__ __attribute__((aligned(16))) __bf16 hl[2][2][SQ * HROW];
  __shared__ __attribute__((aligned(16))) __bf16 xl[2][2][SQ * XROW];
  __shared__ __attribute__((aligned(16))) float cl[SQ * (LH + 4)];
  const int d = blockIdx.y;
  const int tid = threadIdx.x, lane = tid & 63, l31 = lane & 31, half = lane >> 5;
  const int w = __builtin_amdgcn_readfirstlane(tid >> 6);
  const int L = p.L;

  {
    uint32_t* z = reinterpret_cast<uint32_t*>(&hl[0][0][0]);
    for (int i = tid; i < 2 * SQ * HROW / 2; i += 512) z[i] = 0u;
  }
  const int ubase = 32 * w + 4 * half;
  const int glane = ((d * 256 + 8 * w + half) * 32 + l31) * 16;
  const int clane = ((d * 64 + 8 * w + half) * 32 + l31) * 16;
  auto grs = [&](int t) { return mkrsrc(p.gates + (long long)(blockIdx.x * L + t) * (SQ * 2 * LG), SQ * 2 * LG * 4); };
  auto crs = [&](float* b, int t) { return mkrsrc(b + (long long)(blockIdx.x * L + t) * (SQ * 2 * LH), SQ * 2 * LH * 4); };
  auto xrs = [&](int t) { return mkrsrc(p.xn + (long long)(blockIdx.x * L + t) * (SQ * 128), SQ * 128 * 4); };
  auto hrs = [&](int t) { return mkrsrc(p.gates + (long long)(blockIdx.x * L + t) * (SQ * LG), SQ * 2 * LG * 2); };
  auto st_gate = [&](const f32x4& v, int t, int g, int j) {
    if constexpr (GF != 0) bst8(g == 2 ? enc_u16x4<true>(v) : enc_u16x4<false>(v), hrs(t), glane >> 1, (g * 64 + 2 * j) * 256);
    else bst(v, grs(t), glane, (g * 64 + 2 * j) * 512);
  };
  auto st_ch = [&](const f32x4& v, float* b, int t, int j) { bst(v, crs(b, t), clane, 2 * j * 512); };
  const char* hplane = reinterpret_cast<const char*>(p.hcat);
  const long long hlo_off = ws_h2p_plane((long long)gridDim.x * L);
  auto prs = [&](int t, int pl) {
    return mkrsrc(reinterpret_cast<const float*>(hplane + pl * hlo_off + (long long)(blockIdx.x * L + t) * (SQ * 2 * LH * 2)),
                  SQ * 2 * LH * 2);
  };
  auto ld_x = [&](int t, int q) -> f32x4 { return bld(xrs(t), tid * 16, q * 8192); };
  auto st_x = [&](const f32x4& v, int buf, int q) {
    const int u = tid + 512 * q, quad = u >> 5, slot = u & 31;
    bf16x4 hi, lo;
    unpack_hl4(v, hi, lo);
    *reinterpret_cast<bf16x4*>(&xl[buf][0][slot * XROW + 4 * quad]) = hi;
    *reinterpret_cast<bf16x4*>(&xl[buf][1][slot * XROW + 4 * quad]) = lo;
  };

  float* cme = &cl[l31 * (LH + 4) + ubase];
#pragma unroll
  for (int j = 0; j < 4; ++j) *reinterpret_cast<f32x4*>(cme + 8 * j) = f32x4{0.f, 0.f, 0.f, 0.f};

  f32x4 bias[4][4];
#pragma unroll
  for (int g = 0; g < 4; ++g)
#pragma unroll
    for (int j = 0; j < 4; ++j)
      bias[g][j] = *reinterpret_cast<const f32x4*>(p.bias + d * LG + g * 256 + ubase + 8 * j) * (H16 ? 256.f : 1.f);

  const __amdgpu_buffer_rsrc_t wrs =
      F8 ? __builtin_amdgcn_make_buffer_rsrc(reinterpret_cast<unsigned char*>(const_cast<float*>(p.wpack)) +
                                                 (long long)(d * 8 + w) * F8_REGION, 0, F8_REGION, 0x00020000)
         : __builtin_amdgcn_make_buffer_rsrc(const_cast<float*>(p.wpack) + (long long)(d * 8 + w) * (FKS * 8 * 64 * 4), 0,
                                             FKS * 8 * 1024, 0x00020000);
  const int wlane = lane * 16;
  bf16x8 wr[2][8];
  auto refill = [&](int s, int kn, int zo) {
#pragma unroll
    for (int f = 0; f < 8; ++f) {
      if (F8 && kn >= 8) {
        if (f < 6) wr[s][f] = wload(wrs, wlane + f * 1024, zo + F8_HPART + (kn - 8) * F8_KSTEP);
      } else {
// ... 98 lines not shown
#pragma unroll
      for (int r = 0; r < 4; ++r) {
        const float ig = H16 ? c2_sig256(acc[0][4 * j + r]) : fsig(acc[0][4 * j + r]);
        const float fg = H16 ? c2_sig256(acc[1][4 * j + r]) : fsig(acc[1][4 * j + r]);
        const float gg = H16 ? c2_tanh256(acc[2][4 * j + r]) : ftanh(acc[2][4 * j + r]);
        const float og = H16 ? c2_sig256(acc[3][4 * j + r]) : fsig(acc[3][4 * j + r]);
        const float cn = fg * cold[r] + ig * gg;
        vi[r] = ig;
        vf[r] = fg;
        vg[r] = gg;
        vo[r] = og;
        vc[r] = cn;
        vh[r] = og * ftanh(cn);
      }
      bf16x4 h_hi, h_lo;
      split4(vh, h_hi, h_lo);
      if constexpr (H16) {
        *reinterpret_cast<u32x2*>(nhi + 8 * j) = enc_f16x4(vh);
        if constexpr (F8) {
          int c8 = 0;
          c8 = __builtin_amdgcn_cvt_pk_fp8_f32(vh[0], vh[1], c8, false);
          c8 = __builtin_amdgcn_cvt_pk_fp8_f32(vh[2], vh[3], c8, true);
          *reinterpret_cast<int*>(reinterpret_cast<unsigned char*>(&hl[cur ^ 1][1][0]) + l31 * H8ROW + ubase + 8 * j) = c8;
        }
      } else {
        *reinterpret_cast<bf16x4*>(nhi + 8 * j) = h_hi;
        *reinterpret_cast<bf16x4*>(nlo + 8 * j) = h_lo;
      }
      *reinterpret_cast<f32x4*>(cme + 8 * j) = vc;
      st_gate(vi, t, 0, j);
      st_gate(vf, t, 1, j);
      st_gate(vg, t, 2, j);
      st_gate(vo, t, 3, j);
      st_ch(vc, p.cbuf, t, j);
      if constexpr (H2P) {
        u32x2 ph, pl;
        enc_h2p(vh, ph, pl);
        bst8(ph, prs(t, 0), clane >> 1, j * 512);
        bst8(pl, prs(t, 1), clane >> 1, j * 512);
      } else {
        st_ch(pack_hl4(h_hi, h_lo), p.hcat, t, j);
      }
      __builtin_amdgcn_sched_barrier(0);
    }
    __syncthreads();
  }
}


struct fused64_lds {
  f32x4 xw[2][1024];
  __bf16 hl[2][2 * SQ * HROW];
  f32x4 c0l[8 * 2 * 4 * 32];
  float bs[LG];
};
template <int GF, bool W1 = false, bool H16 = false, bool F8 = false, bool H2P = false>
__device__ __forceinline__ void lstm_fwd_fused64_body(const ws_lstm_fused_args& p) {
  static_assert(!(W1 && H16), "W1 is a measurement build of the three-term kernel");
  static_assert(!H2P || H16, "the fp16 planes are written by the fp16-h kernels");
  static_assert(!F8 || H16, "the FP8 lo term belongs to the fp16-h kernel");
  __shared__ __attribute__((aligned(16))) fused64_lds sm;
  auto& xw = sm.xw;
  auto& hl = sm.hl;
  auto& c0l = sm.c0l;
  auto& bs = sm.bs;
  const int d = blockIdx.y;
  const int tid = threadIdx.x, lane = tid & 63, l31 = lane & 31, half = lane >> 5;
  const int w = __builtin_amdgcn_readfirstlane(tid >> 6);
  const int L = p.L;
  const int ntile = (p.nseq + SQ - 1) / SQ;
  const int tile0 = 2 * blockIdx.x;
  const unsigned live1 = tile0 + 1 < ntile ? 1u : 0u;

  {
    uint32_t* z = reinterpret_cast<uint32_t*>(&hl[0][0]);
    for (int i = tid; i < 2 * 2 * SQ * HROW / 2; i += 512) z[i] = 0u;
    for (int i = tid; i < LG; i += 512) bs[i] = (H16 ? 256.f : 1.f) * p.bias[d * LG + i];
  }
  const int ubase = 32 * w + 4 * half;
  const int glane = ((d * 256 + 8 * w + half) * 32 + l31) * 16;
  const int clane = ((d * 64 + 8 * w + half) * 32 + l31) * 16;
  auto blk = [&](int e, int t) { return (long long)((tile0 + e) * L + t); };
  auto lim = [&](int e, unsigned bytes) { return e == 0 ? bytes : bytes * live1; };
  auto grs = [&](int e, int t) { return mkrsrc(p.gates + blk(e, t) * (SQ * 2 * LG), lim(e, SQ * 2 * LG * 4)); };
  auto hrs = [&](int e, int t) { return mkrsrc(p.gates + blk(e, t) * (SQ * LG), lim(e, SQ * 2 * LG * 2)); };
  auto st_gate = [&](const f32x4& v, int e, int t, int g, int j) {
    if constexpr (GF != 0) bst8(g == 2 ? enc_u16x4<true>(v) : enc_u16x4<false>(v), hrs(e, t), glane >> 1, (g * 64 + 2 * j) * 256);
    else bst(v, grs(e, t), glane, (g * 64 + 2 * j) * 512);
  };
  auto crs = [&](float* b, int e, int t) { return mkrsrc(b + blk(e, t) * (SQ * 2 * LH), lim(e, SQ * 2 * LH * 4)); };
  auto xrs = [&](int e, int t) { return mkrsrc(p.xn + blk(e, t) * (SQ * 128), lim(e, SQ * 128 * 4)); };
  const char* hplane = reinterpret_cast<const char*>(p.hcat);
  const long long hlo_off = ws_h2p_plane((long long)ntile * L);
  auto prs = [&](int e, int t, int pl) {
    return mkrsrc(reinterpret_cast<const float*>(hplane + pl * hlo_off + blk(e, t) * (SQ * 2 * LH * 2)), lim(e, SQ * 2 * LH * 2));
  };
  auto dma_x = [&](int e, int t) {
#pragma unroll
    for (int q = 0; q < 2; ++q)
      __builtin_amdgcn_raw_ptr_buffer_load_lds(xrs(e, t), (__attribute__((address_space(3))) void*)&xw[e][512 * q + 64 * w], 16,
                                               lane * 16, (512 * q + 64 * w) * 16, 0, WS_STREAM_AUX);
  };

  f32x4* c0 = &c0l[((w * 2 + half) * 4) * 32 + l31];
#pragma unroll
  for (int j = 0; j < 4; ++j) c0[32 * j] = f32x4{0.f, 0.f, 0.f, 0.f};
  f32x4 c1[4];
#pragma unroll
  for (int j = 0; j < 4; ++j) c1[j] = f32x4{0.f, 0.f, 0.f, 0.f};

  const __amdgpu_buffer_rsrc_t wrs =
      F8 ? __builtin_amdgcn_make_buffer_rsrc(reinterpret_cast<unsigned char*>(const_cast<float*>(p.wpack)) +
                                                 (long long)(d * 8 + w) * F8_REGION, 0, F8_REGION, 0x00020000)
         : __builtin_amdgcn_make_buffer_rsrc(const_cast<float*>(p.wpack) + (long long)(d * 8 + w) * (FKS * 8 * 64 * 4), 0,
                                             FKS * 8 * 1024, 0x00020000);
  const int wlane = lane * 16;
  bf16x8 wr[2][8];
  auto refill = [&](int s, int kn, int zo) {
#pragma unroll
    for (int f = 0; f < 8; ++f) {
      if (F8 && kn >= 8) {
        if (f < 6) wr[s][f] = wload(wrs, wlane + f * 1024, zo + F8_HPART + (kn - 8) * F8_KSTEP);
      } else if (!W1 || !(f & 1)) {
        wr[s][f] = wload(wrs, wlane + (f & 3) * 1024, zo + kn * 8192 + (f >> 2) * 4096);
      }
    }
  };
  refill(0, 0, 0);
  refill(1, 1, 0);
// ... 117 lines not shown
          const float fg = H16 ? c2_sig256(acc[e][1][4 * j + r]) : fsig(acc[e][1][4 * j + r]);
          const float gg = H16 ? c2_tanh256(acc[e][2][4 * j + r]) : ftanh(acc[e][2][4 * j + r]);
          const float og = H16 ? c2_sig256(acc[e][3][4 * j + r]) : fsig(acc[e][3][4 * j + r]);
          const float cn = fg * cold[r] + ig * gg;
          vi[r] = ig;
          vf[r] = fg;
          vg[r] = gg;
          vo[r] = og;
          vc[r] = cn;
          vh[r] = og * ftanh(cn);
        }
        bf16x4 h_hi, h_lo;
        split4(vh, h_hi, h_lo);
        if constexpr (H16) {
          *reinterpret_cast<u32x2*>(nhi + 8 * j) = enc_f16x4(vh);
          if constexpr (F8) {
            int c8 = 0;
            c8 = __builtin_amdgcn_cvt_pk_fp8_f32(vh[0], vh[1], c8, false);
            c8 = __builtin_amdgcn_cvt_pk_fp8_f32(vh[2], vh[3], c8, true);
            *reinterpret_cast<int*>(h8 + (32 * e + l31) * H8ROW + ubase + 8 * j) = c8;
          }
        } else {
          *reinterpret_cast<bf16x4*>(nhi + 8 * j) = h_hi;
          *reinterpret_cast<bf16x4*>(nlo + 8 * j) = h_lo;
        }
        if (e == 0)
          c0[32 * j] = vc;
        else
          c1[j] = vc;
        st_gate(vi, e, t, 0, j);
        st_gate(vf, e, t, 1, j);
        st_gate(vg, e, t, 2, j);
        st_gate(vo, e, t, 3, j);
        bst(vc, crs(p.cbuf, e, t), clane, 2 * j * 512);
        if constexpr (H2P) {
          u32x2 ph, pl;
          enc_h2p(vh, ph, pl);
          bst8(ph, prs(e, t, 0), clane >> 1, j * 512);
          bst8(pl, prs(e, t, 1), clane >> 1, j * 512);
        } else {
          bst(pack_hl4(h_hi, h_lo), crs(p.hcat, e, t), clane, 2 * j * 512);
        }
        __builtin_amdgcn_sched_barrier(0);
      }
    }
    if (p.hfmt & 2) asm volatile("s_waitcnt vmcnt(0)" ::: "memory");
    else if constexpr (H2P) asm volatile("s_waitcnt vmcnt(56)" ::: "memory");
    else asm volatile("s_waitcnt vmcnt(48)" ::: "memory");
    __syncthreads();
  }
}

__global__ __launch_bounds__(512, 1) void lstm_fwd_fused64_kernel(const ws_lstm_fused_args p) {
  lstm_fwd_fused64_body<0>(p);
}
__global__ __launch_bounds__(512, 1) void lstm_fwd_fused64h_kernel(const ws_lstm_fused_args p) {
  lstm_fwd_fused64_body<WS_GATES_H2>(p);
}
__global__ __launch_bounds__(512, 1) void lstm_fwd_fused64h_w1_kernel(const ws_lstm_fused_args p) {
  lstm_fwd_fused64_body<WS_GATES_H2, true>(p);
}
__global__ __launch_bounds__(512, 1) void lstm_fwd_fused64h16_kernel(const ws_lstm_fused_args p) {
  lstm_fwd_fused64_body<WS_GATES_H2, false, true>(p);
}
__global__ __launch_bounds__(512, 1) void lstm_fwd_fused64h8_kernel(const ws_lstm_fused_args p) {
  lstm_fwd_fused64_body<WS_GATES_H2, false, true, true>(p);
}
__global__ __launch_bounds__(512, 1) void lstm_fwd_fused64h16p_kernel(const ws_lstm_fused_args p) {
  lstm_fwd_fused64_body<WS_GATES_H2, false, true, false, true>(p);
}
__global__ __launch_bounds__(512, 1) void lstm_fwd_fused64h8p_kernel(const ws_lstm_fused_args p) {
  lstm_fwd_fused64_body<WS_GATES_H2, false, true, true, true>(p);
}

extern "C" int ws_lstm_fwd_fused(const ws_lstm_fused_args* a, void* stream) {
  WS_REQUIRE(a && a->gates && a->cbuf && a->hcat && a->xn && a->wpack && a->bias, "ws_lstm_fwd_fused: null pointer");
  WS_REQUIRE(a->nseq > 0 && a->L > 0, "ws_lstm_fwd_fused: bad nseq/L");
  WS_REQUIRE(a->gfmt >= WS_GATES_F32 && a->gfmt <= WS_GATES_H2F, "ws_lstm_fwd_fused: gfmt %d", a->gfmt);
  WS_REQUIRE((a->hfmt & ~15) == 0 && (!(a->hfmt & 1) || a->gfmt != WS_GATES_F32) && (!(a->hfmt & 12) || (a->hfmt & 1)),
             "ws_lstm_fwd_fused: hfmt %d (1 = fp16 h, pack from ws_lstm_pack_fused_h16; 5 = + FP8 lo term, pack from "
             "ws_lstm_pack_fused_h8; bit 3 = h out as two fp16 planes, with bit 0; 2-byte gate formats only)", a->hfmt);
  const int ntile = (a->nseq + SQ - 1) / SQ;
  dim3 grid(ntile, 2), block(512);
  hipStream_t s = (hipStream_t)stream;
  const char* env = getenv("WS_FUSED_SEQS");
  static int cus = 0;
  if (!cus && hipDeviceGetAttribute(&cus, hipDeviceAttributeMultiprocessorCount, 0) != hipSuccess) cus = 256;
  const int rounds32 = (2 * ntile + cus - 1) / cus, rounds64 = (2 * ((ntile + 1) / 2) + cus - 1) / cus;
  const bool wide = env ? atoi(env) == 64 : 9 * rounds64 < 5 * rounds32;
  ws_prof_begin(WS_PROF_LSTM_FWD, s);
  const char* w1 = getenv("WS_FUSED_W1");
  const bool h2p = (a->hfmt & 8) != 0;
  if (h2p && (a->hfmt & 4) && wide)
    hipLaunchKernelGGL(lstm_fwd_fused64h8p_kernel, dim3((ntile + 1) / 2, 2), block, 0, s, *a);
  else if (h2p && (a->hfmt & 4))
    hipLaunchKernelGGL((lstm_fwd_fused_kernel<WS_GATES_H2, true, true, true>), grid, block, 0, s, *a);
  else if (h2p && wide)
    hipLaunchKernelGGL(lstm_fwd_fused64h16p_kernel, dim3((ntile + 1) / 2, 2), block, 0, s, *a);
  else if (h2p)
    hipLaunchKernelGGL((lstm_fwd_fused_kernel<WS_GATES_H2, true, false, true>), grid, block, 0, s, *a);
  else if ((a->hfmt & 4) && wide)
    hipLaunchKernelGGL(lstm_fwd_fused64h8_kernel, dim3((ntile + 1) / 2, 2), block, 0, s, *a);
  else if (a->hfmt & 4)
    hipLaunchKernelGGL((lstm_fwd_fused_kernel<WS_GATES_H2, true, true>), grid, block, 0, s, *a);
  else if ((a->hfmt & 1) && wide)
    hipLaunchKernelGGL(lstm_fwd_fused64h16_kernel, dim3((ntile + 1) / 2, 2), block, 0, s, *a);
  else if (a->hfmt & 1)
    hipLaunchKernelGGL((lstm_fwd_fused_kernel<WS_GATES_H2, true>), grid, block, 0, s, *a);
  else if (wide && a->gfmt && w1 && atoi(w1) == 1)
    hipLaunchKernelGGL(lstm_fwd_fused64h_w1_kernel, dim3((ntile + 1) / 2, 2), block, 0, s, *a);
  else if (wide && a->gfmt)
    hipLaunchKernelGGL(lstm_fwd_fused64h_kernel, dim3((ntile + 1) / 2, 2), block, 0, s, *a);
  else if (wide)
    hipLaunchKernelGGL(lstm_fwd_fused64_kernel, dim3((ntile + 1) / 2, 2), block, 0, s, *a);
  else if (a->gfmt)
    hipLaunchKernelGGL(lstm_fwd_fused_kernel<WS_GATES_H2>, grid, block, 0, s, *a);
  else
    hipLaunchKernelGGL(lstm_fwd_fused_kernel<0>, grid, block, 0, s, *a);
  ws_prof_end(WS_PROF_LSTM_FWD, s);
  return ws_check_launch("ws_lstm_fwd_fused");
}
```

### wesep_amd/csrc/lstm_pair.hip

```cpp
#include "lstm_bf16_common.h"

typedef __attribute__((address_space(1))) unsigned gu32;
#define SC1 16
#define PR_ROW 520
#define PR_SPIN_LIMIT (1u << 22)
#define PR_XSLOT 16384

__global__ void lstm_pack_pair_kernel(const float* __restrict__ whh_f, const float* __restrict__ whh_r,
                                      __bf16* __restrict__ out) {
  const int total = 2 * LG * LH;
  for (int idx = blockIdx.x * blockDim.x + threadIdx.x; idx < total; idx += gridDim.x * blockDim.x) {
    int r = idx;
    const int j = r & 7; r >>= 3;
    const int lane = r & 63; r >>= 6;
    const int ks = r & 31; r >>= 5;
    const int w = r & 7; r >>= 3;
    const int hs = r & 1; r >>= 1;
    const int d = r;
    const float* W = d ? whh_r : whh_f;
    const int mt = w < 4 ? 4 * (1 - hs) + w : 4 * hs + (w - 4);
    const int u = 32 * mt + (lane & 31);
    const int kl = 16 * ks + 8 * (lane >> 5) + j;
    const int row = (kl >> 7) * LH + 128 * hs + (kl & 127);
    const float v = W[row * LH + u];
// ... 133 lines not shown
  return ws_check_launch("ws_lstm_pack_pair_f16");
}

extern "C" int ws_lstm_pack_pair(const float* whh_f, const float* whh_r, float* pack, void* stream) {
  WS_REQUIRE(whh_f && whh_r && pack, "ws_lstm_pack_pair: null pointer");
  hipLaunchKernelGGL(lstm_pack_pair_kernel, dim3(512), dim3(256), 0, (hipStream_t)stream, whh_f, whh_r,
                     reinterpret_cast<__bf16*>(pack));
  return ws_check_launch("ws_lstm_pack_pair");
}

__device__ __noinline__ void pair_timed_out(unsigned* tword, unsigned* status) {
  __hip_atomic_store((gu32*)tword, 1u, __ATOMIC_RELAXED, __HIP_MEMORY_SCOPE_AGENT);
  if (status) __hip_atomic_store((gu32*)status, 1u, __ATOMIC_RELAXED, __HIP_MEMORY_SCOPE_AGENT);
}

#define PAIR_RING 4
template <int RF> struct pair_ldsk { static constexpr int value = RF ? 12 : 8; };

typedef _Float16 f16x8 __attribute__((ext_vector_type(8)));
template <int RF>
__device__ __forceinline__ f32x16 pair_mfma(const bf16x8& a, const bf16x8& b, const f32x16& c) {
  if constexpr (RF != 0)
    return __builtin_amdgcn_mfma_f32_32x32x16_f16(__builtin_bit_cast(f16x8, a), __builtin_bit_cast(f16x8, b), c, 0, 0, 0);
  else
    return mfma32(a, b, c);
}

#define TS(k)                                                                                                      \
  if constexpr (V & 2048) {                                                                                        \
    if (pr == 0 && hs == 0 && wx == 0 && lane == 0 && p.dbg_buf)                                                   \
      reinterpret_cast<unsigned long long*>(p.dbg_buf)[(step * 2 + role) * 8 + (k)] = __builtin_readcyclecounter(); \
  }

template <int V, int GF = 0, int RF = 0>
__global__ __launch_bounds__(512, 2) void lstm_bwd_pair_kernel(const ws_lstm_pair_args p) {
  static_assert(RF == 0 || GF == WS_GATES_H2F, "the fp16 recurrence takes the scaled-fp16 d(gates) of WS_GATES_H2F");
  constexpr int PAIR_LDSK = pair_ldsk<RF>::value;
  __shared__ __attribute__((aligned(16))) __bf16 bimg[RF ? 1 : 2][SQ * PR_ROW];
  constexpr int LDSK8 = 27;
  constexpr int LDSB = 6;
  constexpr bool RES = RF >= 2;
  __shared__ __attribute__((aligned(16))) bf16x8 whl[RF == 3 ? 8 * LDSB * 128 : RF == 2 ? 4 * LDSK8 * 64 : 8 * PAIR_LDSK * 64];
  __shared__ __attribute__((aligned(16))) f32x4 rec[2][512];
  const int ntile = (p.nseq + SQ - 1) / SQ, npair = 2 * ntile;
  const int pr = ((int)blockIdx.x >> 4) * 8 + ((int)blockIdx.x & 7), hs = ((int)blockIdx.x >> 3) & 1;
  if (pr >= npair) return;
  long long wall_in = 0;
  if constexpr (V & 2048) wall_in = wall_clock64();
  const int d = pr & 1, tile = pr >> 1;
  const int tid = threadIdx.x, lane = tid & 63, n = lane & 31, half = lane >> 5;
  const int w = __builtin_amdgcn_readfirstlane(tid >> 6);
  const bool xrole = w < 4;
  const int wx = w & 3, role = w >> 2;
  const int L = p.L;

  const int q0 = 8 * wx + 4 * role + half;
  const int gvo = ((d * 256 + 32 * hs + q0) * 32 + n) * 16;
  const int cvo = ((d * 64 + 32 * hs + q0) * 32 + n) * 16;
  float* gdst = GF == WS_GATES_H2S ? p.dgates : p.gates;
  auto grs = [&](int t) { return mkrsrc(gdst + (long long)(tile * L + t) * (SQ * 2 * LG), SQ * 2 * LG * 4); };
  auto hrs = [&](int t) { return mkrsrc(p.gates + (long long)(tile * L + t) * (SQ * LG), SQ * 2 * LG * 2); };
  constexpr bool G2 = GF == WS_GATES_H2 || GF == WS_GATES_H2F;
  float* hdst = (G2 && p.dgates) ? p.dgates : p.gates;
  auto ors = [&](int t) { return mkrsrc(hdst + (long long)(tile * L + t) * (SQ * LG), SQ * 2 * LG * 2); };
  const float dS = GF == WS_GATES_H2F ? ws_dgates_scale(*p.amax) : 1.f;
  auto crs = [&](const float* b, int t) { return mkrsrc(b + (long long)(tile * L + t) * (SQ * 2 * LH), SQ * 2 * LH * 4); };
  typedef typename gate_cell<GF>::type gcell;
  auto ld_gate = [&](int t, int g, int e) -> gcell {
    if constexpr (GF != 0) return bld8(hrs(t), gvo >> 1, (g * 64 + 2 * e) * 256);
    else return bld(grs(t), gvo, (g * 64 + 2 * e) * 512);
  };
  const __amdgpu_buffer_rsrc_t xrs = __builtin_amdgcn_make_buffer_rsrc(
      reinterpret_cast<char*>(p.xchg) + (long long)pr * (4 * PR_XSLOT), 0, 4 * PR_XSLOT, 0x00020000);
  gu32* flags = (gu32*)(p.flags) + pr * 8;
  const int xc0 = ((8 * wx + half) * 32 + n) * 16;

  const char* wbase = reinterpret_cast<const char*>(p.wpack) + (long long)((d * 2 + hs) * 8 + w) * (2 * 32 * 1024);
  bf16x8 wh[32];
#pragma unroll
  for (int ks = 0; ks < 32; ++ks) wh[ks] = *reinterpret_cast<const bf16x8*>(wbase + ks * 1024 + lane * 16);
  bf16x8* wlds = &whl[w * PAIR_LDSK * 64 + lane];
  u32x2* wlds8 = reinterpret_cast<u32x2*>(whl) + w * LDSK8 * 64 + lane;
  u32x2 wq[RF == 2 ? 32 - LDSK8 : 1];
  v8i wq8[RF == 3 ? 8 - LDSB : 1];
  bf16x8* wlds3 = &whl[w * LDSB * 128 + lane];
  int sA = 127;
  float wS = 1.f;
  if constexpr (RF == 3) {
#pragma unroll
    for (int kb = 0; kb < 8; ++kb) {
      const i32x4 p0 = *reinterpret_cast<const i32x4*>(wbase + 32 * 1024 + kb * 2048 + lane * 16);
      const i32x4 p1 = *reinterpret_cast<const i32x4*>(wbase + 32 * 1024 + kb * 2048 + 1024 + lane * 16);
      if (kb < LDSB) {
        wlds3[(2 * kb) * 64] = __builtin_bit_cast(bf16x8, p0);
        wlds3[(2 * kb + 1) * 64] = __builtin_bit_cast(bf16x8, p1);
      } else {
        wq8[kb >= LDSB ? kb - LDSB : 0] = __builtin_shufflevector(p0, p1, 0, 1, 2, 3, 4, 5, 6, 7);
      }
    }
    sA = __builtin_amdgcn_readfirstlane(*reinterpret_cast<const int*>(wbase + 48 * 1024 + 4));
  } else if constexpr (RF == 2) {
#pragma unroll
    for (int ks = 0; ks < LDSK8; ++ks)
      wlds8[ks * 64] = *reinterpret_cast<const u32x2*>(wbase + 32 * 1024 + ks * 512 + lane * 8);
#pragma unroll
    for (int ks = 0; ks < 32 - LDSK8; ++ks)
      wq[ks] = *reinterpret_cast<const u32x2*>(wbase + 32 * 1024 + (LDSK8 + ks) * 512 + lane * 8);
    wS = __builtin_bit_cast(float, __builtin_amdgcn_readfirstlane(*reinterpret_cast<const int*>(wbase + 48 * 1024)));
  } else {
#pragma unroll
    for (int ks = 0; ks < PAIR_LDSK; ++ks)
      wlds[ks * 64] = *reinterpret_cast<const bf16x8*>(wbase + 32 * 1024 + ks * 1024 + lane * 16);
  }
  const __amdgpu_buffer_rsrc_t wrs =
      __builtin_amdgcn_make_buffer_rsrc(const_cast<char*>(wbase) + 32 * 1024, 0, 32 * 1024, 0x00020000);
  const int wlane = lane * 16;
  constexpr int NCH = 32 / PAIR_RING, CH0 = PAIR_LDSK / PAIR_RING;

  rec[0][tid] = rec[1][tid] = f32x4{0.f, 0.f, 0.f, 0.f};
  const f32x4* oth = &rec[role][(wx * 2) * 64 + lane];
  f32x4* mineo = &rec[role ^ 1][(wx * 2) * 64 + lane];

  gcell n_i[2], n_f[2], n_g[2], n_o[2];
  f32x4 n_dh[2], n_cp[2], c_cur[2], dc[2], mine[2];
  const f32x4 zero4v = {0.f, 0.f, 0.f, 0.f};
  auto load_step = [&](int t, int e) {
    n_i[e] = ld_gate(t, 0, e);
    n_f[e] = ld_gate(t, 1, e);
    n_g[e] = ld_gate(t, 2, e);
    n_o[e] = ld_gate(t, 3, e);
    n_dh[e] = bld(crs(p.dhcat, t), cvo, 2 * e * 512);
    const int tp = d == 0 ? max(t - 1, 0) : min(t + 1, L - 1);
    n_cp[e] = bld(crs(p.cbuf, tp), cvo, 2 * e * 512);
  };
  unsigned sink = 0u;
  auto touch = [&](__amdgpu_buffer_rsrc_t r, int voff, int soff) {
    asm volatile("buffer_load_dword %0, %1, %2, %3 offen" : "+v"(sink) : "v"(voff), "s"(r), "s"(soff));
  };
  auto touch_step = [&](int t) {
    const int tp = d == 0 ? max(t - 1, 0) : min(t + 1, L - 1);
#pragma unroll
    for (int e = 0; e < 2; ++e) {
#pragma unroll
      for (int g = 0; g < 4; ++g) touch(hrs(t), gvo >> 1, (g * 64 + 2 * e) * 256);
      touch(crs(p.dhcat, t), cvo, 2 * e * 512);
      touch(crs(p.cbuf, tp), cvo, 2 * e * 512);
    }
  };
  {
    const int t0 = d == 0 ? L - 1 : 0;
#pragma unroll
    for (int e = 0; e < 2; ++e) {
      load_step(t0, e);
      c_cur[e] = bld(crs(p.cbuf, t0), cvo, 2 * e * 512);
      dc[e] = mine[e] = zero4v;
    }
  }
  int dead = 0;
  __syncthreads();
  if constexpr (V & 2048) {
    if (threadIdx.x == 0 && p.dbg_buf) {
      long long* wt = reinterpret_cast<long long*>(p.dbg_buf) + (long long)L * 16 + (pr * 2 + hs) * 4;
      wt[0] = wall_in;
      wt[1] = wall_clock64();
    }
  }

  for (int step = 0; step < L; ++step) {
    const int t = d == 0 ? L - 1 - step : step;
    const int sn = min(step + 1, L - 1);
    const int tn = d == 0 ? L - 1 - sn : sn;
    const bool has_prev = d == 0 ? (t > 0) : (t < L - 1);
    const int par = step & 1;
    int zo = 0;
    asm volatile("" : "+s"(zo));
    f32x4 pk[2][4];
    TS(0);
#pragma unroll
    for (int e = 0; e < 2; ++e) {
      const int q = q0 + 2 * e;
      f32x4 dhr = mine[e] + oth[e * 64];
      if constexpr (RF != 0) dhr *= (1.f / 256.f);
      f32x4 pi, pf, pg, po;
      const f32x4 vi = gate_val<false>(n_i[e]), vf = gate_val<false>(n_f[e]), vg = gate_val<true>(n_g[e]),
                  vo = gate_val<false>(n_o[e]);
#pragma unroll
      for (int r = 0; r < 4; ++r) {
        const float ig = vi[r], fg = vf[r], gg = vg[r], og = vo[r];
        const float dhv = dh_in<GF>(n_dh[e][r], dhr[r], dS);
        const float tc = ftanh(c_cur[e][r]);
        const float dov = dhv * tc;
        const float dcv = dc[e][r] + dhv * og * (1.f - tc * tc);
        dc[e][r] = dcv * fg;
        pi[r] = dcv * gg * ig * (1.f - ig);
        pf[r] = dcv * (has_prev ? n_cp[e][r] : 0.f) * fg * (1.f - fg);
        pg[r] = dcv * ig * (1.f - gg * gg);
        po[r] = dov * og * (1.f - og);
      }
      c_cur[e] = n_cp[e];
      auto emit = [&](const f32x4& v, int g) {
        if constexpr (RF != 0) {
          const u32x2 code = enc_f16x4(v);
          *reinterpret_cast<u32x2*>(&bimg[0][n * PR_ROW + g * 128 + 4 * q]) = code;
          bst8(code, ors(t), gvo >> 1, (g * 64 + 2 * e) * 256);
          return;
        }
        bf16x4 hi, lo;
        split4(v, hi, lo);
        *reinterpret_cast<bf16x4*>(&bimg[0][n * PR_ROW + g * 128 + 4 * q]) = hi;
        *reinterpret_cast<bf16x4*>(&bimg[RF ? 0 : 1][n * PR_ROW + g * 128 + 4 * q]) = lo;
        if constexpr (G2) {
          bst8(enc_dgates<GF>(v, hi), ors(t), gvo >> 1, (g * 64 + 2 * e) * 256);
        } else {
          pk[e][g] = pack_hl4(hi, lo);
          bst(pk[e][g], grs(t), gvo, (g * 64 + 2 * e) * 512);
        }
      };
      emit(pi, 0);
      emit(pf, 1);
      emit(pg, 2);
      emit(po, 3);
    }
    if constexpr (RES) asm volatile("" : "+v"(sink));
    TS(1);
    __syncthreads();
    TS(2);

    if constexpr (RES) touch_step(tn);
// ... 173 lines not shown
        }
      }
      mine[0] = __builtin_bit_cast(f32x4, pv[0]);
      mine[1] = __builtin_bit_cast(f32x4, pv[1]);
      if constexpr (V & 2048) {
        asm volatile("s_waitcnt vmcnt(12)" ::: "memory");
        TS(7);
      }
      mineo[0] = __builtin_bit_cast(f32x4, pv[2]);
      mineo[64] = __builtin_bit_cast(f32x4, pv[3]);
    } else {
      mineo[0] = sum[0];
      mineo[64] = sum[1];
      mine[0] = sum[2];
      mine[1] = sum[3];
      TS(4);
      load_step(tn, 0);
      load_step(tn, 1);
    }
    __syncthreads();
  }
  if constexpr (V & 2048) {
    if (threadIdx.x == 0 && p.dbg_buf)
      reinterpret_cast<long long*>(p.dbg_buf)[(long long)L * 16 + (pr * 2 + hs) * 4 + 2] = wall_clock64();
  }
}

extern "C" int ws_lstm_bwd_pair(const ws_lstm_pair_args* a, void* stream) {
  WS_REQUIRE(a && a->gates && a->cbuf && a->dhcat && a->wpack && a->xchg && a->flags, "ws_lstm_bwd_pair: null pointer");
  WS_REQUIRE(a->nseq > 0 && a->L > 0, "ws_lstm_bwd_pair: nseq and L must be positive");
  WS_REQUIRE(a->gfmt >= WS_GATES_F32 && a->gfmt <= WS_GATES_H2F && (a->gfmt != WS_GATES_H2S || a->dgates) &&
                 (a->gfmt != WS_GATES_H2F || a->amax),
             "ws_lstm_bwd_pair: gfmt %d (WS_GATES_H2S needs dgates, WS_GATES_H2F needs amax)", a->gfmt);
  WS_REQUIRE(a->rfmt == 0 || (a->rfmt >= 1 && a->rfmt <= 3 && a->gfmt == WS_GATES_H2F),
             "ws_lstm_bwd_pair: rfmt %d (1 / 2 / 3 = fp16 recurrence, fp16 + fp16 / fp16 + fp8 weights / + the lo term on the FP8 "
             "MFMA: WS_GATES_H2F only)", a->rfmt);
  const int npair = 2 * ((a->nseq + SQ - 1) / SQ);
  static int cus = 0;
  if (!cus && hipDeviceGetAttribute(&cus, hipDeviceAttributeMultiprocessorCount, 0) != hipSuccess) cus = 0;
  WS_REQUIRE(2 * npair <= cus, "ws_lstm_bwd_pair: %d workgroups must be co-resident but the device has %d CUs", 2 * npair,
             cus);
  const int grid = 16 * ((npair + 7) / 8);
  hipStream_t s = (hipStream_t)stream;
  hipError_t e = hipMemsetAsync(a->flags, 0, ((size_t)npair * 8 + 8) * sizeof(unsigned), s);
  WS_REQUIRE(e == hipSuccess, "ws_lstm_bwd_pair: hipMemsetAsync failed");
  if (a->rfmt != 0) {
    e = hipMemsetAsync(a->xchg, 0x01, (size_t)npair * 4 * PR_XSLOT, s);
    WS_REQUIRE(e == hipSuccess, "ws_lstm_bwd_pair: hipMemsetAsync failed");
  }
  ws_prof_begin(WS_PROF_LSTM_BWD, s);
  if (a->rfmt == 3) {
    WS_REQUIRE(!(a->dbg & 2048), "ws_lstm_bwd_pair: cycle stamps (dbg 2048) exist for rfmt 0 .. 2");
    if (a->dbg & 8) hipLaunchKernelGGL((lstm_bwd_pair_kernel<8, WS_GATES_H2F, 3>), dim3(grid), dim3(512), 0, s, *a);
    else hipLaunchKernelGGL((lstm_bwd_pair_kernel<0, WS_GATES_H2F, 3>), dim3(grid), dim3(512), 0, s, *a);
    ws_prof_end(WS_PROF_LSTM_BWD, s);
    return ws_check_launch("ws_lstm_bwd_pair");
  }
  if (a->rfmt == 2) {
    if (a->dbg & 8) hipLaunchKernelGGL((lstm_bwd_pair_kernel<8, WS_GATES_H2F, 2>), dim3(grid), dim3(512), 0, s, *a);
    else if (a->dbg & 2048) hipLaunchKernelGGL((lstm_bwd_pair_kernel<2048, WS_GATES_H2F, 2>), dim3(grid), dim3(512), 0, s, *a);
    else hipLaunchKernelGGL((lstm_bwd_pair_kernel<0, WS_GATES_H2F, 2>), dim3(grid), dim3(512), 0, s, *a);
    ws_prof_end(WS_PROF_LSTM_BWD, s);
    return ws_check_launch("ws_lstm_bwd_pair");
  }
  if (a->rfmt == 1) {
    if (a->dbg & 8) hipLaunchKernelGGL((lstm_bwd_pair_kernel<8, WS_GATES_H2F, 1>), dim3(grid), dim3(512), 0, s, *a);
    else if (a->dbg & 2048) hipLaunchKernelGGL((lstm_bwd_pair_kernel<2048, WS_GATES_H2F, 1>), dim3(grid), dim3(512), 0, s, *a);
    else hipLaunchKernelGGL((lstm_bwd_pair_kernel<0, WS_GATES_H2F, 1>), dim3(grid), dim3(512), 0, s, *a);
    ws_prof_end(WS_PROF_LSTM_BWD, s);
    return ws_check_launch("ws_lstm_bwd_pair");
  }
  switch ((a->dbg & (8 | 2048)) + a->gfmt) {
    case 0: hipLaunchKernelGGL((lstm_bwd_pair_kernel<0, 0>), dim3(grid), dim3(512), 0, s, *a); break;
    case 1: hipLaunchKernelGGL((lstm_bwd_pair_kernel<0, WS_GATES_H2>), dim3(grid), dim3(512), 0, s, *a); break;
    case 2: hipLaunchKernelGGL((lstm_bwd_pair_kernel<0, WS_GATES_H2S>), dim3(grid), dim3(512), 0, s, *a); break;
    case 3: hipLaunchKernelGGL((lstm_bwd_pair_kernel<0, WS_GATES_H2F>), dim3(grid), dim3(512), 0, s, *a); break;
    case 8: hipLaunchKernelGGL((lstm_bwd_pair_kernel<8, 0>), dim3(grid), dim3(512), 0, s, *a); break;
    case 9: hipLaunchKernelGGL((lstm_bwd_pair_kernel<8, WS_GATES_H2>), dim3(grid), dim3(512), 0, s, *a); break;
    case 10: hipLaunchKernelGGL((lstm_bwd_pair_kernel<8, WS_GATES_H2S>), dim3(grid), dim3(512), 0, s, *a); break;
    case 11: hipLaunchKernelGGL((lstm_bwd_pair_kernel<8, WS_GATES_H2F>), dim3(grid), dim3(512), 0, s, *a); break;
    case 2048: hipLaunchKernelGGL((lstm_bwd_pair_kernel<2048, 0>), dim3(grid), dim3(512), 0, s, *a); break;
    case 2048 + 3: hipLaunchKernelGGL((lstm_bwd_pair_kernel<2048, WS_GATES_H2F>), dim3(grid), dim3(512), 0, s, *a); break;
    default: WS_REQUIRE(false, "ws_lstm_bwd_pair: dbg bits 8 and 2048 are exclusive; cycle stamps: WS_GATES_F32 / H2F only");
// ... 5 lines not shown
```

### wesep_amd/dev.py

```python
import ctypes as C
import os
from typing import NamedTuple, Optional

import numpy as np
import torch

from . import _lib as L

BIG = 1 << 30


def gemm_mode() -> str:
    return os.environ.get("WESEP_GEMM", "bf16x3")


def _mode_bit(mode):
    return 4 if (mode or gemm_mode()) == "bf16x3" else 0
GN_EPS = float(np.finfo(np.float32).eps)


class Rows(NamedTuple):
    div: int
    s1: int
    s2: int
# ... 332 lines not shown
def lstm_blk_mode(nseq: int) -> int:
    env = os.environ.get("WESEP_LSTM_SEQS")
    if env:
        return L.LSTM_BF16X3_BLK16 if env == "16" else L.LSTM_BF16X3_BLK
    return L.LSTM_BF16X3_BLK16 if 2 * (-(-nseq // 32)) <= 128 else L.LSTM_BF16X3_BLK


def lstm_pack(whh_f, whh_r, pack_fwd, pack_bwd, mode=L.LSTM_BF16X3):
    for n, t in (("whh_f", whh_f), ("whh_r", whh_r), ("pack_fwd", pack_fwd), ("pack_bwd", pack_bwd)):
        _chk(t, n)
    L.check(L.lib().ws_lstm_pack(_p(whh_f), _p(whh_r), _p(pack_fwd), _p(pack_bwd), mode,
                                 L.stream_ptr()), "ws_lstm_pack")


def lstm_pack_bwd_f8(whh_f, whh_r, pack_bwd):
    for n, t in (("whh_f", whh_f), ("whh_r", whh_r), ("pack_bwd", pack_bwd)):
        _chk(t, n)
    L.check(L.lib().ws_lstm_pack_bwd_f8(_p(whh_f), _p(whh_r), _p(pack_bwd), L.stream_ptr()), "ws_lstm_pack_bwd_f8")


def lstm_pack_dx_f8(wcat, pack):
    for n, t in (("wcat", wcat), ("pack", pack)):
        _chk(t, n)
    L.check(L.lib().ws_lstm_pack_dx_f8(_p(wcat), _p(pack), L.stream_ptr()), "ws_lstm_pack_dx_f8")


def lstm_cat_ih(wih_f, wih_r, bih_f, bhh_f, bih_r, bhh_r, n_in, wcat, bcat):
    for t in (wih_f, wih_r, bih_f, bhh_f, bih_r, bhh_r, wcat, bcat):
        _chk(t, "lstm_cat_ih arg")
    L.check(L.lib().ws_lstm_cat_ih(_p(wih_f), _p(wih_r), _p(bih_f), _p(bhh_f), _p(bih_r), _p(bhh_r),
                                   n_in, _p(wcat), _p(bcat), L.stream_ptr()), "ws_lstm_cat_ih")


def _bptt_bytes(gfmt: int) -> int:
    return {L.GATES_F32: 40, L.GATES_H2: 24, L.GATES_H2S: 32, L.GATES_H2F: 24}[gfmt]


def gates_fmt() -> int:
    return {"h2": L.GATES_H2F, "h2b": L.GATES_H2, "h2s": L.GATES_H2S, "f32": L.GATES_F32}[os.environ.get("WESEP_GATES", "h2")]


def blh_floats(nblocks: int, C_: int) -> int:
    return nblocks * 32 * C_ // 2


def _lstm_args(gates, cbuf, hcat, wpack, sm: SeqMap, mode, dhcat=None, run_if=None, gfmt=0, gates_in=None, dgates=None,
               amax=None, rfmt=0, dxn=None, wxpack=None):
    for n, t in (("gates", gates), ("cbuf", cbuf), ("hcat", hcat), ("wpack", wpack), ("dhcat", dhcat),
                 ("gates_in", gates_in), ("dgates", dgates), ("dxn", dxn), ("wxpack", wxpack)):
        _chk(t, n)
    a = L.LstmArgs()
    a.gates, a.cbuf, a.hcat, a.dhcat, a.wpack = _p(gates), _p(cbuf), _p(hcat), _p(dhcat), _p(wpack)
    a.sq_s1, a.sq_s2, a.step_rows = sm.s1, sm.s2, sm.step_rows
    a.nseq, a.sq_div, a.L, a.mode = sm.nseq, sm.div, sm.L, mode
    a.run_if = C.c_void_p(run_if.data_ptr()) if run_if is not None else None
    a.gates_in, a.dgates, a.gfmt, a.rfmt = _p(gates_in), _p(dgates), gfmt, rfmt
    a.amax = C.c_void_p(amax.data_ptr()) if amax is not None else None
    if dxn is not None:
        if dxn.dim() != 3 or dxn.shape[0] != 2 or dxn.shape[2] != 128 or getattr(sm, "nvalid", 0):
            raise L.WesepHipError(f"lstm_bwd: dxn must be [2, P, 128] on a sequence map without padding sequences, got {tuple(dxn.shape)}")
        a.dxn, a.dxn_dir_stride, a.wxpack = _p(dxn), dxn.shape[1] * 128, _p(wxpack)
    return a


def lstm_fwd(gates, cbuf, hcat, wpack, sm: SeqMap, mode=L.LSTM_BF16X3, run_if=None, gfmt=0, gates_in=None, h2p=False):
    a = _lstm_args(gates, cbuf, hcat, wpack, sm, mode, run_if=run_if, gfmt=gfmt, gates_in=gates_in,
                   rfmt=L.LSTM_FWD_H2P if h2p else 0)
    if run_if is None:
        u = ALG_LSTM_UNITS or L.LSTM_H
        _alg("lstm_fwd", sm.nseq * sm.L * 2 * u * (16 + (2 if gfmt else 4) * 4 + 8), 2 * sm.nseq * sm.L * 2 * 4 * u * u)
    L.check(L.lib().ws_lstm_fwd(C.byref(a), L.stream_ptr()), "ws_lstm_fwd")


def lstm_bwd(gates, cbuf, hcat, dhcat, wpack, sm: SeqMap, mode=L.LSTM_BF16X3, gfmt=0, dgates=None, run_if=None, amax=None,
             rfmt=0, dxn=None, wxpack=None):
    a = _lstm_args(gates, cbuf, hcat, wpack, sm, mode, dhcat, gfmt=gfmt, dgates=dgates, run_if=run_if, amax=amax, rfmt=rfmt,
                   dxn=dxn, wxpack=wxpack)
    if run_if is None:
        _alg("lstm_bwd", _bptt_bytes(gfmt) * sm.nseq * sm.L * 2 * (ALG_LSTM_UNITS or L.LSTM_H),
             2 * sm.nseq * sm.L * 2 * 4 * (ALG_LSTM_UNITS or L.LSTM_H) ** 2)
    L.check(L.lib().ws_lstm_bwd(C.byref(a), L.stream_ptr()), "ws_lstm_bwd")


_CU_COUNT = {}


def cu_count(device) -> int:
    key = (device.type, device.index)
    if key not in _CU_COUNT:
        _CU_COUNT[key] = torch.cuda.get_device_properties(device).multi_processor_count
    return _CU_COUNT[key]


def lstm_cluster_resident(sm: SeqMap, device) -> bool:
    return sm.nseq % 64 == 0 and (sm.nseq // 32) * 8 <= cu_count(device)


def lstm_cluster_ok(sm: SeqMap, device) -> bool:
    if os.environ.get("WESEP_LSTM_CLUSTER", "1") == "0":
        return False
    return lstm_cluster_resident(sm, device) and sm.L >= 64


class _ClusterScratch:

    def __init__(self, device):
        self.device = device
        self.xchg = None
        self.flags = None
        self.status = torch.zeros(2, device=device, dtype=torch.int32)
        self.host = torch.zeros(2, dtype=torch.int32)
        if device.type == "cuda" and torch.cuda.is_available():
# ... 97 lines not shown
    xchg, flags = sc.get(ncl * 2 * 8 * 8192 // 4, ncl * 8 + 8)
    a = L.LstmClusterArgs()
    a.gates, a.cbuf, a.hcat, a.whh_f, a.whh_r = _p(gates), _p(cbuf), _p(hcat), _p(whh_f), _p(whh_r)
    a.gfmt, a.gates_in = gfmt, _p(gates_in)
    a.xchg, a.flags = C.c_void_p(xchg.data_ptr()), C.c_void_p(flags.data_ptr())
    a.status = C.c_void_p((status if status is not None else sc.status).data_ptr())
    a.nseq, a.L, a.dbg = sm.nseq, sm.L, dbg
    u = ALG_LSTM_UNITS or L.LSTM_H
    _alg("lstm_fwd", sm.nseq * sm.L * 2 * u * (16 + (2 if gfmt else 4) * 4 + 8), 2 * sm.nseq * sm.L * 2 * 4 * u * u)
    L.check(L.lib().ws_lstm_fwd_cluster(C.byref(a), L.stream_ptr()), "ws_lstm_fwd_cluster")
    return flags[ncl * 8:ncl * 8 + 1]


_FALLBACK_SCRATCH = {}


def fallback_scratch(device, nfloats: int) -> torch.Tensor:
    key = (device.type, device.index, L.stream_ptr().value if device.type == "cuda" and torch.cuda.is_available() else 0)
    buf = _FALLBACK_SCRATCH.get(key)
    if buf is None or buf.numel() < nfloats:
        buf = _FALLBACK_SCRATCH[key] = torch.empty(nfloats, device=device, dtype=torch.float32)
    return buf[:nfloats]


def lstm_cluster2_on() -> bool:
    return os.environ.get("WESEP_LSTM_CLUSTER2", "1") != "0"


def cluster2_rfmt() -> int:
    return 1 if os.environ.get("WESEP_CLUSTER2_F8", "0") == "1" else 0


def lstm_fwd_cluster2(gates, cbuf, hcat, xn, wcat, bcat, whh_f, whh_r, sm: SeqMap, status=None, dbg=0, dbg_buf=None, rfmt=None,
                      h2p=False):
    for n, t in (("gates", gates), ("cbuf", cbuf), ("hcat", hcat), ("xn", xn), ("wcat", wcat), ("bcat", bcat),
                 ("whh_f", whh_f), ("whh_r", whh_r)):
        _chk(t, n)
    ncl = sm.nseq // 32
    sc = _cluster_scratch(gates.device)
    xchg, flags = sc.get(ncl * 2 * 8 * 4096 // 4, ncl * 8 + 8)
    a = L.LstmCluster2Args()
    a.gates, a.cbuf, a.hcat, a.xn, a.wcat, a.bcat = _p(gates), _p(cbuf), _p(hcat), _p(xn), _p(wcat), _p(bcat)
    a.whh_f, a.whh_r = _p(whh_f), _p(whh_r)
    tw = flags[ncl * 8:ncl * 8 + 1]
    a.xchg, a.tword = C.c_void_p(xchg.data_ptr()), C.c_void_p(tw.data_ptr())
    a.status = C.c_void_p((status if status is not None else sc.status).data_ptr())
    a.nseq, a.L, a.dbg = sm.nseq, sm.L, dbg
    a.rfmt = (cluster2_rfmt() if rfmt is None else rfmt) | (2 if h2p else 0)
    a.dbg_buf = C.c_void_p(dbg_buf.data_ptr()) if dbg_buf is not None else None
    u = ALG_LSTM_UNITS or L.LSTM_H
    _alg("lstm_fwd", sm.nseq * sm.L * (2 * u * 16 + 4 * 128), 2 * sm.nseq * sm.L * 2 * 4 * u * (u + 128))
    L.check(L.lib().ws_lstm_fwd_cluster2(C.byref(a), L.stream_ptr()), "ws_lstm_fwd_cluster2")
    return tw


def lstm_bwd_cluster(gates, cbuf, dhcat, whh_f, whh_r, sm: SeqMap, status=None, dbg=0):
    for n, t in (("gates", gates), ("cbuf", cbuf), ("dhcat", dhcat), ("whh_f", whh_f), ("whh_r", whh_r)):
        _chk(t, n)
    ncl = sm.nseq // 32
    sc = _cluster_scratch(gates.device)
    xchg, flags = sc.get(ncl * 2 * 64 * 8192 // 4, ncl * 8 + 8)
    a = L.LstmClusterArgs()
    a.gates, a.cbuf, a.dhcat, a.whh_f, a.whh_r = _p(gates), _p(cbuf), _p(dhcat), _p(whh_f), _p(whh_r)
    a.xchg, a.flags = C.c_void_p(xchg.data_ptr()), C.c_void_p(flags.data_ptr())
    a.status = C.c_void_p(status.data_ptr() if status is not None else sc.status.data_ptr() + 4)
    a.nseq, a.L, a.dbg = sm.nseq, sm.L, dbg
    L.check(L.lib().ws_lstm_bwd_cluster(C.byref(a), L.stream_ptr()), "ws_lstm_bwd_cluster")
    return flags[ncl * 8:ncl * 8 + 1]


def lstm_pair_ok(sm: SeqMap, device) -> bool:
    if os.environ.get("WESEP_LSTM_PAIR_BWD", "1") == "0":
        return False
    return 4 * (-(-sm.nseq // 32)) <= cu_count(device) // 2 and sm.L >= 64


def lstm_pack_pair(whh_f, whh_r, pack, f16=False):
    for n, t in (("whh_f", whh_f), ("whh_r", whh_r), ("pack", pack)):
        _chk(t, n)
    fn = (L.lib().ws_lstm_pack_pair, L.lib().ws_lstm_pack_pair_f16, L.lib().ws_lstm_pack_pair_f8,
          L.lib().ws_lstm_pack_pair_f8mx)[int(f16)]
    L.check(fn(_p(whh_f), _p(whh_r), _p(pack), L.stream_ptr()), "ws_lstm_pack_pair")


def lstm_bwd_pair(gates, cbuf, dhcat, wpack, sm: SeqMap, status=None, dbg=0, dbg_buf=None, gfmt=0, dgates=None,
                  repairable=False, amax=None, rfmt=0):
    for n, t in (("gates", gates), ("cbuf", cbuf), ("dhcat", dhcat), ("wpack", wpack), ("dgates", dgates)):
        _chk(t, n)
    npair = 2 * (-(-sm.nseq // 32))
    sc = _cluster_scratch(gates.device)
    xchg, flags = sc.get(npair * 65536 // 4, npair * 8 + 8)
    a = L.LstmPairArgs()
    a.gates, a.cbuf, a.dhcat, a.wpack = _p(gates), _p(cbuf), _p(dhcat), _p(wpack)
    a.xchg, a.flags = C.c_void_p(xchg.data_ptr()), C.c_void_p(flags.data_ptr())
    a.status = C.c_void_p(status.data_ptr() if status is not None else sc.status.data_ptr() + (0 if repairable else 4))
    a.nseq, a.L, a.dbg = sm.nseq, sm.L, dbg
    a.dbg_buf = C.c_void_p(dbg_buf.data_ptr()) if dbg_buf is not None else None
    a.gfmt, a.dgates = gfmt, _p(dgates)
    a.amax = C.c_void_p(amax.data_ptr()) if amax is not None else None
    a.rfmt = rfmt
    _alg("lstm_bwd", _bptt_bytes(gfmt) * sm.nseq * sm.L * 2 * (ALG_LSTM_UNITS or L.LSTM_H),
             2 * sm.nseq * sm.L * 2 * 4 * (ALG_LSTM_UNITS or L.LSTM_H) ** 2)
    L.check(L.lib().ws_lstm_bwd_pair(C.byref(a), L.stream_ptr()), "ws_lstm_bwd_pair")
    return flags[npair * 8:npair * 8 + 1]


class BandTables:

    def __init__(self, band_width, device):
        bw = np.asarray(band_width, dtype=np.int32)
        f0 = np.concatenate([[0], np.cumsum(bw)[:-1]]).astype(np.int32)
        self.nband = len(bw)
        self.nbins = int(bw.sum())
        self.bw_host, self.f0_host = bw, f0
        bob = np.repeat(np.arange(self.nband, dtype=np.int32), bw)
        to = lambda a: torch.from_numpy(np.ascontiguousarray(a)).to(device)
        self.band_of_bin, self.f0, self.bw = to(bob), to(f0), to(bw)
        self.bw2, self.off2 = to(2 * bw), to(2 * f0)

    def c(self):
        b = L.Bands()
        b.band_of_bin = C.c_void_p(self.band_of_bin.data_ptr())
        b.band_f0 = C.c_void_p(self.f0.data_ptr())
        b.band_bw = C.c_void_p(self.bw.data_ptr())
        b.nband, b.nbins = self.nband, self.nbins
        return b


def stft_bandsplit(wav, bands: BandTables, xbs, lengths=None):
    _chk(wav, "wav")
    _chk(xbs, "xbs")
    R, T = wav.shape
    b = bands.c()
    if lengths is not None:
# ... 511 lines not shown
    _chk(src, "src")
    _chk(out, "out")
    _call("ws_bcast_rows", _p(src), scale, rows_per_r, M, Cc, _p(out))


def cross_entropy(logits, label, loss, dlogits):
    _chk(logits, "logits")
    _chk(label, "label", torch.int64)
    _chk(loss, "loss")
    _chk(dlogits, "dlogits")
    R, S = logits.shape
    _call("ws_cross_entropy", _p(logits), C.c_void_p(label.data_ptr()), R, S, _p(loss), _p(dlogits))


def lstm_fuse_ok(nseq: int, cluster: bool) -> bool:
    if os.environ.get("WESEP_LSTM_FUSE", "1") == "0" or cluster:
        return False
    return lstm_blk_mode(nseq) == L.LSTM_BF16X3_BLK


def lstm_fused_hfmt(gfmt) -> int:
    if gfmt == L.GATES_F32 or os.environ.get("WESEP_FUSED_H16", "1") == "0":
        return 0
    return 5 if os.environ.get("WESEP_FUSED_F8", "1") != "0" else 1


def lstm_pack_fused(wih_f, wih_r, whh_f, whh_r, pack, hfmt=0):
    for n, t in (("wih_f", wih_f), ("wih_r", wih_r), ("whh_f", whh_f), ("whh_r", whh_r), ("pack", pack)):
        _chk(t, n)
    _call("ws_lstm_pack_fused_h8" if hfmt & 4 else "ws_lstm_pack_fused_h16" if hfmt & 1 else "ws_lstm_pack_fused",
          _p(wih_f), _p(wih_r), _p(whh_f), _p(whh_r), _p(pack))


def lstm_fwd_fused(gates, cbuf, hcat, xn, wpack, bias, sm: SeqMap, gfmt=0, hfmt=0):
    for n, t in (("gates", gates), ("cbuf", cbuf), ("hcat", hcat), ("xn", xn), ("wpack", wpack), ("bias", bias)):
        _chk(t, n)
    a = L.LstmFusedArgs()
    a.gates, a.cbuf, a.hcat, a.xn, a.wpack, a.bias = _p(gates), _p(cbuf), _p(hcat), _p(xn), _p(wpack), _p(bias)
    a.nseq, a.L, a.gfmt = sm.nseq, sm.L, gfmt
    a.hfmt = hfmt | (2 if os.environ.get("WESEP_FUSED_DRAIN", "0") == "1" else 0)
    u = ALG_LSTM_UNITS or L.LSTM_H
    _alg("lstm_fwd", sm.nseq * sm.L * (2 * u * ((2 if gfmt else 4) * 4 + 8) + 4 * 128), 2 * sm.nseq * sm.L * 2 * 4 * u * (u + 128))
    L.check(L.lib().ws_lstm_fwd_fused(C.byref(a), L.stream_ptr()), "ws_lstm_fwd_fused")


def conv_out(n: int, k: int, s: int, p: int) -> int:
    return (n + 2 * p - k) // s + 1


def im2col(x, R: int, H: int, W: int, Cc: int, k: int, s: int, p: int, patches, ldp: int):
    _chk(x, "x")
    _chk(patches, "patches")
    _call("ws_im2col", _p(x), R, H, W, Cc, k, s, p, ldp, _p(patches))


def col2im(dpatches, R: int, H: int, W: int, Cc: int, k: int, s: int, p: int, dx):
    _chk(dpatches, "dpatches")
    _chk(dx, "dx")
    _call("ws_col2im", _p(dpatches), R, H, W, Cc, k, s, p, _p(dx))


def tstp_fwd(x, R: int, F: int, T: int, Cc: int, stats, eps=1e-7):
    _chk(x, "x")
    _chk(stats, "stats")
    _call("ws_tstp_fwd", _p(x), R, F, T, Cc, eps, _p(stats))


def tstp_bwd(x, stats, dstats, R: int, F: int, T: int, Cc: int, dx):
    for n, t in (("x", x), ("stats", stats), ("dstats", dstats), ("dx", dx)):
        _chk(t, n)
    _call("ws_tstp_bwd", _p(x), _p(stats), _p(dstats), R, F, T, Cc, _p(dx))


def mhastp_sizes(R: int, T: int, Q: int, H: int, layers: int, ds: int, dm: int):
    blk, work = C.c_longlong(0), C.c_longlong(0)
# ... 863 lines not shown
```

Before: 344.2 utterances/s.

## Store LSTM cell state as fp16 between forward and BPTT kernels

Adds a C16 flag that makes the forward LSTM kernels (stream, s16, fused, cluster2) write the saved cell state as fp16. The backward kernels (stream, s16, pair) then read it back as fp16 and widen to fp32 for tanh and the forget-gate product. This halves the cbuf traffic written in forward and read in BPTT, which is meant to ease memory bandwidth in the recurrence. In exchange the cell state loses precision, which could hurt gradient accuracy for large magnitudes, and the flag is on by default for the H2F/h2p configuration.

```diff
diff --git a/include/wesep_hip.h b/include/wesep_hip.h
--- a/include/wesep_hip.h
+++ b/include/wesep_hip.h
@@ -179,6 +179,7 @@
 #define WS_LSTM_BF16X3_BLK16 5
 #define WS_LSTM_H 256
 #define WS_LSTM_FWD_H2P 16
+#define WS_LSTM_C16 32
 #define WS_LSTM_PACK_FLOATS (2 * 4 * WS_LSTM_H * WS_LSTM_H)
 int ws_lstm_pack(const float* whh_f, const float* whh_r, float* pack_fwd, float* pack_bwd,
                  int mode, void* stream);
diff --git a/wesep_amd/_lib.py b/wesep_amd/_lib.py
--- a/wesep_amd/_lib.py
+++ b/wesep_amd/_lib.py
@@ -22,6 +22,7 @@
 
 LSTM_F32_MT1, LSTM_F32_MT2, LSTM_BF16X3, LSTM_BF16X3_BLK, LSTM_BF16X3_BLK16 = 1, 2, 3, 4, 5
 LSTM_FWD_H2P = 16
+LSTM_C16 = 32
 LSTM_PACK_FLOATS = 2 * 4 * LSTM_H * LSTM_H
 
 _p = C.c_void_p
diff --git a/wesep_amd/blstm_core.py b/wesep_amd/blstm_core.py
--- a/wesep_amd/blstm_core.py
+++ b/wesep_amd/blstm_core.py
@@ -351,6 +351,7 @@
     band_dx: bool
     a_fmt: int
     h2p: bool = False
+    c16: bool = False
 
 
 _WIHT_KIND = {0: "wihT", 1: "wihT", 2: "wihT16", 3: "wihT8"}
@@ -375,10 +376,13 @@
     a16 = gfmt == L.GATES_H2F and grad and tnb_a16()
     h2p = (a16 and dev.h2p_on(device) and not ragged and fwd in ("fused", "cluster2", "stream")
            and (fwd != "fused" or bool(dev.lstm_fused_hfmt(gfmt) & 1)))
+    prf = pair_rfmt(gfmt) if grad and bptt == "pair" else 0
+    bdx = bool(brf) and gn_geo is not None and band_dx(brf, seq, gn_geo)
+    c16 = (h2p and grad and gfmt == L.GATES_H2F and dev.c16_on(device) and not ragged and seq.L <= dev.C16_MAX_STEPS
+           and ((bptt == "pair" and prf in (2, 3) and not _pair_stamp_on()) or (bptt == "stream" and not bdx)))
     return BlstmPlan(
         nb=dev.bl_num_blocks(seq), lmode=lmode, cluster=cluster, fwd=fwd, bptt=bptt, grad=grad, gfmt=gfmt, g_fmt=g_fmt,
-        a16=a16, pair_rfmt=pair_rfmt(gfmt) if grad and bptt == "pair" else 0,
-        band_rfmt=brf, band_dx=bool(brf) and gn_geo is not None and band_dx(brf, seq, gn_geo), a_fmt=dxn_fmt(g_fmt), h2p=h2p)
+        a16=a16, pair_rfmt=prf, band_rfmt=brf, band_dx=bdx, a_fmt=dxn_fmt(g_fmt), h2p=h2p, c16=c16)
 
 
 def consume_once(ctx, who):
@@ -405,7 +409,9 @@
     wcat, bcat = W("cat")
     whf, whr = W("whh")
     xn = _empty(d, nb, 32 * N)
-    cbuf, hcat = _empty(d, nb, 32 * 2 * H), _empty(d, nb, 32 * 2 * H)
+    hcat = _empty(d, nb, 32 * 2 * H)
+    cells = dict(c16=True) if plan.c16 else {}
+    cbuf = _empty(d, dev.blh_floats(nb, 2 * H)) if plan.c16 else _empty(d, nb, 32 * 2 * H)
     gates = _empty(d, dev.blh_floats(nb, 2 * G4)) if h2 else _empty(d, nb, 32 * 2 * G4)
     xn16 = _empty(d, dev.blh_floats(nb, N)) if plan.a16 else None
     h2p = plan.h2p
@@ -415,13 +421,13 @@
         dev.gemm_p2b(A=x, lda=N, sm=seq, Wpack=None, N=0, C_out=None, A_bl=xn, A_bl16=xn16, **norm)
         hf = dev.lstm_fused_hfmt(gfmt)
         dev.lstm_fwd_fused(gates, cbuf, hcat, xn, W("fused8" if hf & 4 else "fused16" if hf else "fused"), bcat, seq, gfmt=gfmt,
-                           hfmt=hf | (8 if h2p else 0))
+                           hfmt=hf | (8 if h2p else 0), **cells)
     elif plan.fwd == "cluster2":
         dev.gemm_p2b(A=x, lda=N, sm=seq, Wpack=None, N=0, C_out=None, A_bl=xn, A_bl16=xn16, **norm)
-        tw = dev.lstm_fwd_cluster2(gates, cbuf, hcat, xn, wcat, bcat, whf, whr, seq, dbg=_cluster_dbg(), **planes)
+        tw = dev.lstm_fwd_cluster2(gates, cbuf, hcat, xn, wcat, bcat, whf, whr, seq, dbg=_cluster_dbg(), **planes, **cells)
         pre = dev.fallback_scratch(d, nb * 32 * 2 * G4)
         dev.gemm_p2b(A=x, lda=N, sm=seq, Wpack=W("wih"), N=2 * G4, C_out=pre, bias=bcat, run_if=tw, **norm)
-        dev.lstm_fwd(gates, cbuf, hcat, W("hh")[0], seq, lmode, run_if=tw, gfmt=gfmt, gates_in=pre, **planes)
+        dev.lstm_fwd(gates, cbuf, hcat, W("hh")[0], seq, lmode, run_if=tw, gfmt=gfmt, gates_in=pre, **planes, **cells)
         del pre
     else:
         pre = _empty(d, nb, 32 * 2 * G4) if h2 else gates
@@ -436,7 +442,7 @@
                 dev.gemm_p2b(run_if=tw, **xproj)
             dev.lstm_fwd(gates, cbuf, hcat, W("hh")[0], seq, lmode, run_if=tw, **rec)
         else:
-            dev.lstm_fwd(gates, cbuf, hcat, W("hh")[0], seq, lmode, **planes, **rec)
+            dev.lstm_fwd(gates, cbuf, hcat, W("hh")[0], seq, lmode, **planes, **cells, **rec)
         del pre
     out = torch.empty_like(res)
     if h2p:
@@ -471,6 +477,7 @@
     dh, dout_bl = _empty(d, nb, 32 * 2 * H), _empty(d, nb, 32 * N)
     dxn2 = None
     amax = amax_word(d) if gfmt == L.GATES_H2F else None
+    cells = dict(c16=True) if plan.c16 else {}
     dev.gemm_p2b(A=dout, lda=N, sm=seq, Wpack=W("projT"), N=2 * H, C_out=dh, A_bl=dout_bl, amax=amax)
     if _h2_probe() & 16:
         _probe_round(dh, "bf16")
@@ -488,8 +495,8 @@
         dg = _empty(d, nb, 32 * 2 * G4) if gfmt == L.GATES_H2S else _empty(d, dev.blh_floats(nb, 2 * G4))
         rf = plan.pair_rfmt
         tw = dev.lstm_bwd_pair(gates, cbuf, dh, W("hhp16" if rf else "hhp"), seq, gfmt=gfmt, dgates=dg, repairable=True,
-                               dbg=_pair_dbg(), amax=amax, rfmt=rf, dbg_buf=_pair_stamp_buf(d, seq.L))
-        dev.lstm_bwd(gates, cbuf, hcat, dh, W("hh")[1], seq, plan.lmode, gfmt=gfmt, dgates=dg, run_if=tw, amax=amax)
+                               dbg=_pair_dbg(), amax=amax, rfmt=rf, dbg_buf=_pair_stamp_buf(d, seq.L), **cells)
+        dev.lstm_bwd(gates, cbuf, hcat, dh, W("hh")[1], seq, plan.lmode, gfmt=gfmt, dgates=dg, run_if=tw, amax=amax, **cells)
     else:
         dg = _empty(d, nb, 32 * 2 * G4) if gfmt == L.GATES_H2S else gates
         brf = plan.band_rfmt
@@ -497,7 +504,7 @@
             dxn2 = _empty(d, 2, dout.numel() // N, N)
         dev.lstm_bwd(gates, cbuf, hcat, dh, W("hh8") if brf else W("hh")[1], seq, plan.lmode, gfmt=gfmt,
                      dgates=dg if gfmt == L.GATES_H2S else None, amax=amax, rfmt=brf, dxn=dxn2,
-                     wxpack=W("wx8") if dxn2 is not None else None)
+                     wxpack=W("wx8") if dxn2 is not None else None, **cells)
     if _h2_probe() & 2 and gfmt == L.GATES_F32:
         _probe_round(gates, "bf16", packed=True)
     if _h2_probe() & 32 and gfmt == L.GATES_F32 and not torch.cuda.is_available():
diff --git a/wesep_amd/csrc/lstm.hip b/wesep_amd/csrc/lstm.hip
--- a/wesep_amd/csrc/lstm.hip
+++ b/wesep_amd/csrc/lstm.hip
@@ -372,12 +372,17 @@
              a->gfmt);
   WS_REQUIRE(a->gfmt != WS_GATES_H2S || !bwd || a->dgates, "%s: WS_GATES_H2S needs dgates", who);
   WS_REQUIRE(a->gfmt == WS_GATES_F32 || ((a->mode >> 8) & 7) == 0, "%s: probe builds are WS_GATES_F32 only", who);
-  WS_REQUIRE(a->rfmt == 0 || ((a->rfmt == 2 || a->rfmt == 3) && bwd && a->mode == WS_LSTM_BF16X3_BLK && a->gfmt == WS_GATES_H2F) ||
-                 (a->rfmt == WS_LSTM_FWD_H2P && !bwd && (a->mode == WS_LSTM_BF16X3_BLK || a->mode == WS_LSTM_BF16X3_BLK16)),
+  const int rfmt = a->rfmt & ~WS_LSTM_C16;
+  WS_REQUIRE(rfmt == 0 || ((rfmt == 2 || rfmt == 3) && bwd && a->mode == WS_LSTM_BF16X3_BLK && a->gfmt == WS_GATES_H2F) ||
+                 (rfmt == WS_LSTM_FWD_H2P && !bwd && (a->mode == WS_LSTM_BF16X3_BLK || a->mode == WS_LSTM_BF16X3_BLK16)),
              "%s: rfmt %d (2 / 3 = fp16 recurrence on fp16 + FP8 weights, 3: the lo term on the FP8 MFMA: ws_lstm_bwd, "
              "WS_LSTM_BF16X3_BLK, WS_GATES_H2F only; 16 = hcat out as two fp16 planes: ws_lstm_fwd, blocked-layout modes only)",
              who, a->rfmt);
-  WS_REQUIRE(!a->dxn || (bwd && a->rfmt == 2 && a->wxpack && a->dxn_dir_stride > 0 && a->dxn_dir_stride < (1ll << 29) && !a->run_if),
+  WS_REQUIRE(!(a->rfmt & WS_LSTM_C16) || (a->gfmt == WS_GATES_H2F && (a->mode == WS_LSTM_BF16X3_BLK || a->mode == WS_LSTM_BF16X3_BLK16) &&
+                                          (bwd ? !a->dxn : rfmt == WS_LSTM_FWD_H2P)),
+             "%s: rfmt %d: cbuf as fp16 (bit WS_LSTM_C16) needs WS_GATES_H2F and a blocked-layout mode; ws_lstm_fwd: with "
+             "WS_LSTM_FWD_H2P; ws_lstm_bwd: no dxn", who, a->rfmt);
+  WS_REQUIRE(!a->dxn || (bwd && rfmt == 2 && a->wxpack && a->dxn_dir_stride > 0 && a->dxn_dir_stride < (1ll << 29) && !a->run_if),
              "%s: dxn (d(xn) inside the BPTT, ABI v19) needs rfmt 2, wxpack (ws_lstm_pack_dx_f8), 0 < dxn_dir_stride < 2^29 floats "
              "(32-bit store offsets) and no run_if", who);
   return WS_OK;
diff --git a/wesep_amd/csrc/lstm_bf16.hip b/wesep_amd/csrc/lstm_bf16.hip
--- a/wesep_amd/csrc/lstm_bf16.hip
+++ b/wesep_amd/csrc/lstm_bf16.hip
@@ -138,9 +138,10 @@
   return 0;
 }
 
-template <bool BLK, int DBG, int GF = 0, bool H2P = false>
+template <bool BLK, int DBG, int GF = 0, bool H2P = false, bool C16 = false>
 __global__ __launch_bounds__(512, 2) void lstm_fwd_bf16_kernel(const ws_lstm_args p) {
   static_assert(!H2P || (BLK && DBG == 0), "the fp16 planes are a format of the blocked layout");
+  static_assert(!C16 || H2P, "the fp16 cell state is written next to the fp16 planes");
   __shared__ __attribute__((aligned(16))) __bf16 hl[2][2][SQ * HROW];
   __shared__ __attribute__((aligned(16))) float cl[SQ * (LH + 4)];
   if (p.run_if && *p.run_if == 0u) return;
@@ -175,6 +176,7 @@
     return mkrsrc(reinterpret_cast<const float*>(hplane + pl * hlo_off + (long long)(blockIdx.x * L + t) * (SQ * 2 * LH * 2)),
                   SQ * 2 * LH * 2);
   };
+  auto c16rs = [&](int t) { return mkrsrc(p.cbuf + (long long)(blockIdx.x * L + t) * (SQ * LH), SQ * 2 * LH * 2); };
   auto ld_gate = [&](int t, int g, int j) -> f32x4 {
     if constexpr (BLK) return bld(grs(t), glane, (g * 64 + 2 * j) * 512);
     else return *reinterpret_cast<const f32x4*>(p.gates + goff(t, g, j));
@@ -296,7 +298,8 @@
         st_gate(vf, t, 1, j);
         st_gate(vg, t, 2, j);
         st_gate(vo, t, 3, j);
-        st_ch(vc, p.cbuf, t, j);
+        if constexpr (C16) bst8(enc_c16(vc), c16rs(t), clane >> 1, j * 512);
+        else st_ch(vc, p.cbuf, t, j);
         if constexpr (H2P) {
           u32x2 ph, pl;
           enc_h2p(vh, ph, pl);
@@ -311,8 +314,9 @@
   }
 }
 
-template <bool BLK, int DBG, int GF = 0, int RF = 0, bool DX = false>
+template <bool BLK, int DBG, int GF = 0, int RF = 0, bool DX = false, bool C16 = false>
 __global__ __launch_bounds__(512, 2) void lstm_bwd_bf16_kernel(const ws_lstm_args p) {
+  static_assert(!C16 || (BLK && GF == WS_GATES_H2F && !DX), "the fp16 cell state comes with the blocked layout and WS_GATES_H2F");
   static_assert(RF == 0 || (BLK && GF == WS_GATES_H2F), "the fp16 recurrence takes the scaled-fp16 d(gates) of WS_GATES_H2F");
   static_assert(!DX || RF == 2, "d(xn) in the BPTT rides on the fp16 d(gates) image of rfmt 2");
   __shared__ __attribute__((aligned(16))) __bf16 dgl[RF ? 1 : 2][SQ * DROW];
@@ -356,6 +360,11 @@
     if constexpr (BLK) return bld(crs(b, t), clane, 2 * j * 512);
     else return *reinterpret_cast<const f32x4*>(b + coff(t, j));
   };
+  typedef typename c_cell<C16>::type ccell;
+  auto ld_c = [&](int t, int j) -> ccell {
+    if constexpr (C16) return bld8(mkrsrc(p.cbuf + (long long)(bx * L + t) * (SQ * LH), SQ * 2 * LH * 2), clane >> 1, j * 512);
+    else return ld_ch(p.cbuf, t, j);
+  };
 
   const int kpar = DX ? (w >> 2) : 0;
   const __amdgpu_buffer_rsrc_t wrs = __builtin_amdgcn_make_buffer_rsrc(
@@ -419,7 +428,8 @@
   const __amdgpu_buffer_rsrc_t xors = __builtin_amdgcn_make_buffer_rsrc(
       DX ? p.dxn + (long long)d * p.dxn_dir_stride : nullptr, 0, DX ? (unsigned)(p.dxn_dir_stride * 4) : 0u, 0x00020000);
   gcell n_i[4], n_f[4], n_g[4], n_o[4];
-  f32x4 n_dh[4], n_cp[4], c_cur[4], dc[4];
+  f32x4 n_dh[4], dc[4];
+  ccell n_cp[4], c_cur[4];
   f32x16 dhr;
   const f32x4 zero4v = {0.f, 0.f, 0.f, 0.f};
 #pragma unroll
@@ -434,14 +444,14 @@
     n_o[j] = ld_gate(t, 3, j);
     n_dh[j] = ld_ch(p.dhcat, t, j);
     const int tp = d == 0 ? max(t - 1, 0) : min(t + 1, L - 1);
-    n_cp[j] = ld_ch(p.cbuf, tp, j);
+    n_cp[j] = ld_c(tp, j);
   };
   {
     const int t0 = d == 0 ? L - 1 : 0;
 #pragma unroll
     for (int j = 0; j < 4; ++j) {
       load_step(t0, j);
-      c_cur[j] = ld_ch(p.cbuf, t0, j);
+      c_cur[j] = ld_c(t0, j);
     }
   }
   __builtin_amdgcn_sched_barrier(0);
@@ -469,12 +479,12 @@
       for (int r = 0; r < 4; ++r) {
         const float ig = vi[r], fg = vf[r], gg = vg[r], og = vo[r];
         const float dhv = dh_in<GF>(n_dh[j][r], dhr[4 * j + r], dS);
-        const float tc = ftanh(c_cur[j][r]);
+        const float tc = ftanh(c_at(c_cur[j], r));
         const float dov = dhv * tc;
         const float dcv = dc[j][r] + dhv * og * (1.f - tc * tc);
         dc[j][r] = dcv * fg;
         pi[r] = dcv * gg * ig * (1.f - ig);
-        pf[r] = dcv * (has_prev ? n_cp[j][r] : 0.f) * fg * (1.f - fg);
+        pf[r] = dcv * (has_prev ? c_at(n_cp[j], r) : 0.f) * fg * (1.f - fg);
         pg[r] = dcv * ig * (1.f - gg * gg);
         po[r] = dov * og * (1.f - og);
       }
@@ -639,6 +649,10 @@
 
 int ws_launch_lstm_fwd_bf16(const ws_lstm_args* a, hipStream_t s) {
   dim3 grid((a->nseq + SQ - 1) / SQ, 2), block(512);
+  if (a->rfmt == (WS_LSTM_FWD_H2P | WS_LSTM_C16)) {
+    hipLaunchKernelGGL((lstm_fwd_bf16_kernel<true, 0, WS_GATES_H2F, true, true>), grid, block, 0, s, *a);
+    return 0;
+  }
   if (a->rfmt == WS_LSTM_FWD_H2P) {
     if (a->gfmt == WS_GATES_H2) hipLaunchKernelGGL((lstm_fwd_bf16_kernel<true, 0, WS_GATES_H2, true>), grid, block, 0, s, *a);
     else if (a->gfmt == WS_GATES_H2S) hipLaunchKernelGGL((lstm_fwd_bf16_kernel<true, 0, WS_GATES_H2S, true>), grid, block, 0, s, *a);
@@ -652,6 +666,13 @@
 
 int ws_launch_lstm_bwd_bf16(const ws_lstm_args* a, hipStream_t s) {
   dim3 grid((a->nseq + SQ - 1) / SQ, 2), block(512);
+  if (a->rfmt & WS_LSTM_C16) {
+    const int rf = a->rfmt & ~WS_LSTM_C16;
+    if (rf == 2) hipLaunchKernelGGL((lstm_bwd_bf16_kernel<true, 0, WS_GATES_H2F, 2, false, true>), grid, block, 0, s, *a);
+    else if (rf == 3) hipLaunchKernelGGL((lstm_bwd_bf16_kernel<true, 0, WS_GATES_H2F, 3, false, true>), grid, block, 0, s, *a);
+    else hipLaunchKernelGGL((lstm_bwd_bf16_kernel<true, 0, WS_GATES_H2F, 0, false, true>), grid, block, 0, s, *a);
+    return 0;
+  }
   if (a->rfmt == 2 && a->dxn) {
     hipLaunchKernelGGL((lstm_bwd_bf16_kernel<true, 0, WS_GATES_H2F, 2, true>), grid, block, 0, s, *a);
     return 0;
diff --git a/wesep_amd/csrc/lstm_bf16_common.h b/wesep_amd/csrc/lstm_bf16_common.h
--- a/wesep_amd/csrc/lstm_bf16_common.h
+++ b/wesep_amd/csrc/lstm_bf16_common.h
@@ -135,6 +135,21 @@
 }
 __device__ __forceinline__ long long ws_h2p_plane(long long nblk) { return nblk * (SQ * 2 * LH * 2); }
 
+__device__ __forceinline__ u32x2 enc_c16(const f32x4& vc) {
+  f16x4 h;
+#pragma unroll
+  for (int j = 0; j < 4; ++j) {
+    float x = vc[j];
+    asm volatile("" : "+v"(x));
+    h[j] = (_Float16)x;
+  }
+  return __builtin_bit_cast(u32x2, h);
+}
+template <bool C16> struct c_cell { typedef f32x4 type; };
+template <> struct c_cell<true> { typedef u32x2 type; };
+__device__ __forceinline__ float c_at(const f32x4& c, int r) { return c[r]; }
+__device__ __forceinline__ float c_at(const u32x2& c, int r) { return (float)__builtin_bit_cast(f16x4, c)[r]; }
+
 template <int GF>
 __device__ __forceinline__ u32x2 enc_dgates(const f32x4& v, const bf16x4& hi) {
   if constexpr (GF == WS_GATES_H2F) return enc_f16x4(v);
diff --git a/wesep_amd/csrc/lstm_bf16_s16.hip b/wesep_amd/csrc/lstm_bf16_s16.hip
--- a/wesep_amd/csrc/lstm_bf16_s16.hip
+++ b/wesep_amd/csrc/lstm_bf16_s16.hip
@@ -54,8 +54,9 @@
   return 0;
 }
 
-template <int GF, bool H2P = false>
+template <int GF, bool H2P = false, bool C16 = false>
 __global__ __launch_bounds__(512, 2) void lstm_fwd_s16_kernel(const ws_lstm_args p) {
+  static_assert(!C16 || H2P, "the fp16 cell state is written next to the fp16 planes");
   __shared__ __attribute__((aligned(16))) __bf16 hl[2][2][S16 * HROW];
   __shared__ __attribute__((aligned(16))) float cl[S16 * (LH + 4)];
   if (p.run_if && *p.run_if == 0u) return;
@@ -85,6 +86,8 @@
   auto prs = [&](int t, int pl) {
     return mkrsrc(reinterpret_cast<const float*>(hplane + pl * hlo_off + (long long)(tile * L + t) * (SQ * 2 * LH * 2)), SQ * 2 * LH * 2);
   };
+
+  auto c16rs = [&](int t) { return mkrsrc(p.cbuf + (long long)(tile * L + t) * (SQ * LH), SQ * 2 * LH * 2); };
 
   const int ubase = 32 * w + 4 * mq;
   float* cme = &cl[n * (LH + 4) + ubase];
@@ -190,7 +193,8 @@
       st_gate(vf, t, 1, tu);
       st_gate(vg, t, 2, tu);
       st_gate(vo, t, 3, tu);
-      st_ch(vc, p.cbuf, t, tu);
+      if constexpr (C16) bst8(enc_c16(vc), c16rs(t), clane >> 1, 2 * tu * 512);
+      else st_ch(vc, p.cbuf, t, tu);
       if constexpr (H2P) {
         u32x2 ph, pl;
         enc_h2p(vh, ph, pl);
@@ -209,8 +213,9 @@
 #ifndef S16_DBG
 #define S16_DBG 0
 #endif
-template <int GF>
+template <int GF, bool C16 = false>
 __global__ __launch_bounds__(512, 2) void lstm_bwd_s16_kernel(const ws_lstm_args p) {
+  static_assert(!C16 || GF == WS_GATES_H2F, "the fp16 cell state comes with WS_GATES_H2F");
   __shared__ __attribute__((aligned(16))) __bf16 dgl[2][S16 * DROW];
   if (p.run_if && *p.run_if == 0u) return;
   const int d = blockIdx.y;
@@ -235,6 +240,11 @@
   };
   auto st_gate = [&](const f32x4& v, int t, int g, int tu) { bst(v, grs(t), glane, (g * 64 + 4 * tu) * 512); };
   auto ld_ch = [&](const float* b, int t, int tu) -> f32x4 { return bld(crs(b, t), clane, 4 * tu * 512); };
+  typedef typename c_cell<C16>::type ccell;
+  auto ld_c = [&](int t, int tu) -> ccell {
+    if constexpr (C16) return bld8(mkrsrc(p.cbuf + (long long)(tile * L + t) * (SQ * LH), SQ * 2 * LH * 2), clane >> 1, 2 * tu * 512);
+    else return ld_ch(p.cbuf, t, tu);
+  };
   const int ubase = 32 * w + 4 * mq;
 
   const __amdgpu_buffer_rsrc_t wrs = __builtin_amdgcn_make_buffer_rsrc(
@@ -247,7 +257,8 @@
     for (int f = 0; f < 16; ++f) wr[s][f] = wload(wrs, wlane + (f & 3) * 1024, s * 16384 + (f >> 2) * 4096);
 
   gcell n_i[2], n_f[2], n_g[2], n_o[2];
-  f32x4 n_dh[2], n_cp[2], c_cur[2], dc[2], dhr[2];
+  f32x4 n_dh[2], dc[2], dhr[2];
+  ccell n_cp[2], c_cur[2];
   const f32x4 zero4v = {0.f, 0.f, 0.f, 0.f};
 #pragma unroll
   for (int tu = 0; tu < 2; ++tu) dc[tu] = dhr[tu] = zero4v;
@@ -258,14 +269,14 @@
     n_o[tu] = ld_gate(t, 3, tu);
     n_dh[tu] = ld_ch(p.dhcat, t, tu);
     const int tp = d == 0 ? max(t - 1, 0) : min(t + 1, L - 1);
-    n_cp[tu] = ld_ch(p.cbuf, tp, tu);
+    n_cp[tu] = ld_c(tp, tu);
   };
   {
     const int t0 = d == 0 ? L - 1 : 0;
 #pragma unroll
     for (int tu = 0; tu < 2; ++tu) {
       load_step(t0, tu);
-      c_cur[tu] = ld_ch(p.cbuf, t0, tu);
+      c_cur[tu] = ld_c(t0, tu);
     }
   }
 
@@ -287,12 +298,12 @@
       for (int r = 0; r < 4; ++r) {
         const float ig = vi[r], fg = vf[r], gg = vg[r], og = vo[r];
         const float dhv = dh_in<GF>(n_dh[tu][r], dhr[tu][r], dS);
-        const float tc = ftanh(c_cur[tu][r]);
+        const float tc = ftanh(c_at(c_cur[tu], r));
         const float dov = dhv * tc;
         const float dcv = dc[tu][r] + dhv * og * (1.f - tc * tc);
         dc[tu][r] = dcv * fg;
         pi[r] = dcv * gg * ig * (1.f - ig);
-        pf[r] = dcv * (has_prev ? n_cp[tu][r] : 0.f) * fg * (1.f - fg);
+        pf[r] = dcv * (has_prev ? c_at(n_cp[tu], r) : 0.f) * fg * (1.f - fg);
         pg[r] = dcv * ig * (1.f - gg * gg);
         po[r] = dov * og * (1.f - og);
       }
@@ -355,7 +366,8 @@
 int ws_launch_lstm_fwd_s16(const ws_lstm_args* a, hipStream_t s) {
   dim3 grid(2 * ((a->nseq + SQ - 1) / SQ), 2), block(512);
   const bool h2p = a->rfmt == WS_LSTM_FWD_H2P;
-  if (a->gfmt && h2p) hipLaunchKernelGGL((lstm_fwd_s16_kernel<WS_GATES_H2, true>), grid, block, 0, s, *a);
+  if (a->rfmt == (WS_LSTM_FWD_H2P | WS_LSTM_C16)) hipLaunchKernelGGL((lstm_fwd_s16_kernel<WS_GATES_H2, true, true>), grid, block, 0, s, *a);
+  else if (a->gfmt && h2p) hipLaunchKernelGGL((lstm_fwd_s16_kernel<WS_GATES_H2, true>), grid, block, 0, s, *a);
   else if (h2p) hipLaunchKernelGGL((lstm_fwd_s16_kernel<0, true>), grid, block, 0, s, *a);
   else if (a->gfmt) hipLaunchKernelGGL(lstm_fwd_s16_kernel<WS_GATES_H2>, grid, block, 0, s, *a);
   else hipLaunchKernelGGL(lstm_fwd_s16_kernel<0>, grid, block, 0, s, *a);
@@ -364,7 +376,8 @@
 
 int ws_launch_lstm_bwd_s16(const ws_lstm_args* a, hipStream_t s) {
   dim3 grid(2 * ((a->nseq + SQ - 1) / SQ), 2), block(512);
-  if (a->gfmt == WS_GATES_H2) hipLaunchKernelGGL(lstm_bwd_s16_kernel<WS_GATES_H2>, grid, block, 0, s, *a);
+  if (a->rfmt & WS_LSTM_C16) hipLaunchKernelGGL((lstm_bwd_s16_kernel<WS_GATES_H2F, true>), grid, block, 0, s, *a);
+  else if (a->gfmt == WS_GATES_H2) hipLaunchKernelGGL(lstm_bwd_s16_kernel<WS_GATES_H2>, grid, block, 0, s, *a);
   else if (a->gfmt == WS_GATES_H2S) hipLaunchKernelGGL(lstm_bwd_s16_kernel<WS_GATES_H2S>, grid, block, 0, s, *a);
   else if (a->gfmt == WS_GATES_H2F) hipLaunchKernelGGL(lstm_bwd_s16_kernel<WS_GATES_H2F>, grid, block, 0, s, *a);
   else hipLaunchKernelGGL(lstm_bwd_s16_kernel<0>, grid, block, 0, s, *a);
diff --git a/wesep_amd/csrc/lstm_cluster2.hip b/wesep_amd/csrc/lstm_cluster2.hip
--- a/wesep_amd/csrc/lstm_cluster2.hip
+++ b/wesep_amd/csrc/lstm_cluster2.hip
@@ -148,6 +148,8 @@
   auto prs = [&](int t, int pl) {
     return mkrsrc(reinterpret_cast<const float*>(hplane + pl * hlo_off + ((long long)2 * cc * L + t) * (cblk * 2)), 0x7fffffffu);
   };
+  const bool c16 = (p.rfmt & 4) != 0;
+  auto c16rs = [&](int t) { return mkrsrc(p.cbuf + ((long long)2 * cc * L + t) * (cblk / 2), 0x7fffffffu); };
   const char* xbase = reinterpret_cast<const char*>(p.xn);
   auto xld = [&](int t, int q) -> f32x4 {
     const long long blk = (long long)(2 * cc + st) * L + t;
@@ -201,7 +203,8 @@
         bst8(u32x2{pr[0], pr[1]}, hrs(tprev), (gvo + e * gts) >> 1, (2 * g2) * 64 * 256);
         bst8(u32x2{pr[2], pr[3]}, hrs(tprev), (gvo + e * gts) >> 1, (2 * g2 + 1) * 64 * 256);
       }
-      bst(e == 0 ? c4 : outc[mt], crs(p.cbuf, tprev), cvo + e * cts, 0);
+      if (c16) bst8(enc_c16(e == 0 ? c4 : outc[mt]), c16rs(tprev), (cvo + e * cts) >> 1, 0);
+      else bst(e == 0 ? c4 : outc[mt], crs(p.cbuf, tprev), cvo + e * cts, 0);
       if (h2p) {
         const u32x4 hc = __builtin_bit_cast(u32x4, outl[2][ct]);
         bst8(u32x2{hc[0], hc[1]}, prs(tprev, 0), (cvo + e * cts) >> 1, 0);
@@ -344,8 +347,9 @@
   e = hipMemsetAsync(a->tword, 0, sizeof(unsigned), s);
   WS_REQUIRE(e == hipSuccess, "ws_lstm_fwd_cluster2: hipMemsetAsync failed");
   ws_prof_begin(WS_PROF_LSTM_FWD, s);
-  WS_REQUIRE((a->rfmt & ~3) == 0,
-             "ws_lstm_fwd_cluster2: rfmt %d (bit 0: the lo term of W_hh on the FP8 MFMA; bit 1: hcat out as two fp16 planes)", a->rfmt);
+  WS_REQUIRE((a->rfmt & ~7) == 0,
+             "ws_lstm_fwd_cluster2: rfmt %d (bit 0: the lo term of W_hh on the FP8 MFMA; bit 1: hcat out as two fp16 planes; bit 2: "
+             "cbuf out as fp16)", a->rfmt);
   if (a->rfmt & 1) {
     if (a->dbg & 2048) hipLaunchKernelGGL((lstm_fwd_cluster2_kernel<false, true, true>), dim3(grid), dim3(512), 0, s, *a);
     else if (a->dbg & 8) hipLaunchKernelGGL((lstm_fwd_cluster2_kernel<true, false, true>), dim3(grid), dim3(512), 0, s, *a);
diff --git a/wesep_amd/csrc/lstm_fused.hip b/wesep_amd/csrc/lstm_fused.hip
--- a/wesep_amd/csrc/lstm_fused.hip
+++ b/wesep_amd/csrc/lstm_fused.hip
@@ -131,9 +131,10 @@
   return ws_check_launch("ws_lstm_pack_fused_h8");
 }
 
-template <int GF, bool H16 = false, bool F8 = false, bool H2P = false>
+template <int GF, bool H16 = false, bool F8 = false, bool H2P = false, bool C16 = false>
 __global__ __launch_bounds__(512, 1) void lstm_fwd_fused_kernel(const ws_lstm_fused_args p) {
   static_assert(!F8 || H16, "the FP8 lo term belongs to the fp16-h kernel");
+  static_assert(!C16 || H2P, "the fp16 cell state is written next to the fp16 planes");
   static_assert(!H2P || H16, "the fp16 planes are written by the fp16-h kernels");
   __shared__ __attribute__((aligned(16))) __bf16 hl[2][2][SQ * HROW];
   __shared__ __attribute__((aligned(16))) __bf16 xl[2][2][SQ * XROW];
@@ -165,6 +166,7 @@
     return mkrsrc(reinterpret_cast<const float*>(hplane + pl * hlo_off + (long long)(blockIdx.x * L + t) * (SQ * 2 * LH * 2)),
                   SQ * 2 * LH * 2);
   };
+  auto c16rs = [&](int t) { return mkrsrc(p.cbuf + (long long)(blockIdx.x * L + t) * (SQ * LH), SQ * 2 * LH * 2); };
   auto ld_x = [&](int t, int q) -> f32x4 { return bld(xrs(t), tid * 16, q * 8192); };
   auto st_x = [&](const f32x4& v, int buf, int q) {
     const int u = tid + 512 * q, quad = u >> 5, slot = u & 31;
@@ -329,7 +331,8 @@
       st_gate(vf, t, 1, j);
       st_gate(vg, t, 2, j);
       st_gate(vo, t, 3, j);
-      st_ch(vc, p.cbuf, t, j);
+      if constexpr (C16) bst8(enc_c16(vc), c16rs(t), clane >> 1, j * 512);
+      else st_ch(vc, p.cbuf, t, j);
       if constexpr (H2P) {
         u32x2 ph, pl;
         enc_h2p(vh, ph, pl);
@@ -351,11 +354,12 @@
   f32x4 c0l[8 * 2 * 4 * 32];
   float bs[LG];
 };
-template <int GF, bool W1 = false, bool H16 = false, bool F8 = false, bool H2P = false>
+template <int GF, bool W1 = false, bool H16 = false, bool F8 = false, bool H2P = false, bool C16 = false>
 __device__ __forceinline__ void lstm_fwd_fused64_body(const ws_lstm_fused_args& p) {
   static_assert(!(W1 && H16), "W1 is a measurement build of the three-term kernel");
   static_assert(!H2P || H16, "the fp16 planes are written by the fp16-h kernels");
   static_assert(!F8 || H16, "the FP8 lo term belongs to the fp16-h kernel");
+  static_assert(!C16 || H2P, "the fp16 cell state is written next to the fp16 planes");
   __shared__ __attribute__((aligned(16))) fused64_lds sm;
   auto& xw = sm.xw;
   auto& hl = sm.hl;
@@ -392,6 +396,7 @@
   auto prs = [&](int e, int t, int pl) {
     return mkrsrc(reinterpret_cast<const float*>(hplane + pl * hlo_off + blk(e, t) * (SQ * 2 * LH * 2)), lim(e, SQ * 2 * LH * 2));
   };
+  auto c16rs = [&](int e, int t) { return mkrsrc(p.cbuf + blk(e, t) * (SQ * LH), lim(e, SQ * 2 * LH * 2)); };
   auto dma_x = [&](int e, int t) {
 #pragma unroll
     for (int q = 0; q < 2; ++q)
@@ -575,7 +580,8 @@
         st_gate(vf, e, t, 1, j);
         st_gate(vg, e, t, 2, j);
         st_gate(vo, e, t, 3, j);
-        bst(vc, crs(p.cbuf, e, t), clane, 2 * j * 512);
+        if constexpr (C16) bst8(enc_c16(vc), c16rs(e, t), clane >> 1, j * 512);
+        else bst(vc, crs(p.cbuf, e, t), clane, 2 * j * 512);
         if constexpr (H2P) {
           u32x2 ph, pl;
           enc_h2p(vh, ph, pl);
@@ -616,13 +622,22 @@
   lstm_fwd_fused64_body<WS_GATES_H2, false, true, true, true>(p);
 }
 
+__global__ __launch_bounds__(512, 1) void lstm_fwd_fused64h16pc_kernel(const ws_lstm_fused_args p) {
+  lstm_fwd_fused64_body<WS_GATES_H2, false, true, false, true, true>(p);
+}
+__global__ __launch_bounds__(512, 1) void lstm_fwd_fused64h8pc_kernel(const ws_lstm_fused_args p) {
+  lstm_fwd_fused64_body<WS_GATES_H2, false, true, true, true, true>(p);
+}
+
 extern "C" int ws_lstm_fwd_fused(const ws_lstm_fused_args* a, void* stream) {
   WS_REQUIRE(a && a->gates && a->cbuf && a->hcat && a->xn && a->wpack && a->bias, "ws_lstm_fwd_fused: null pointer");
   WS_REQUIRE(a->nseq > 0 && a->L > 0, "ws_lstm_fwd_fused: bad nseq/L");
   WS_REQUIRE(a->gfmt >= WS_GATES_F32 && a->gfmt <= WS_GATES_H2F, "ws_lstm_fwd_fused: gfmt %d", a->gfmt);
-  WS_REQUIRE((a->hfmt & ~15) == 0 && (!(a->hfmt & 1) || a->gfmt != WS_GATES_F32) && (!(a->hfmt & 12) || (a->hfmt & 1)),
+  WS_REQUIRE((a->hfmt & ~31) == 0 && (!(a->hfmt & 1) || a->gfmt != WS_GATES_F32) && (!(a->hfmt & 12) || (a->hfmt & 1)) &&
+                 (!(a->hfmt & 16) || (a->hfmt & 8)),
              "ws_lstm_fwd_fused: hfmt %d (1 = fp16 h, pack from ws_lstm_pack_fused_h16; 5 = + FP8 lo term, pack from "
-             "ws_lstm_pack_fused_h8; bit 3 = h out as two fp16 planes, with bit 0; 2-byte gate formats only)", a->hfmt);
+             "ws_lstm_pack_fused_h8; bit 3 = h out as two fp16 planes, with bit 0; bit 4 = cbuf out as fp16, with bit 3; 2-byte gate "
+             "formats only)", a->hfmt);
   const int ntile = (a->nseq + SQ - 1) / SQ;
   dim3 grid(ntile, 2), block(512);
   hipStream_t s = (hipStream_t)stream;
@@ -634,7 +649,15 @@
   ws_prof_begin(WS_PROF_LSTM_FWD, s);
   const char* w1 = getenv("WS_FUSED_W1");
   const bool h2p = (a->hfmt & 8) != 0;
-  if (h2p && (a->hfmt & 4) && wide)
+  if ((a->hfmt & 16) && (a->hfmt & 4) && wide)
+    hipLaunchKernelGGL(lstm_fwd_fused64h8pc_kernel, dim3((ntile + 1) / 2, 2), block, 0, s, *a);
+  else if ((a->hfmt & 16) && (a->hfmt & 4))
+    hipLaunchKernelGGL((lstm_fwd_fused_kernel<WS_GATES_H2, true, true, true, true>), grid, block, 0, s, *a);
+  else if ((a->hfmt & 16) && wide)
+    hipLaunchKernelGGL(lstm_fwd_fused64h16pc_kernel, dim3((ntile + 1) / 2, 2), block, 0, s, *a);
+  else if (a->hfmt & 16)
+    hipLaunchKernelGGL((lstm_fwd_fused_kernel<WS_GATES_H2, true, false, true, true>), grid, block, 0, s, *a);
+  else if (h2p && (a->hfmt & 4) && wide)
     hipLaunchKernelGGL(lstm_fwd_fused64h8p_kernel, dim3((ntile + 1) / 2, 2), block, 0, s, *a);
   else if (h2p && (a->hfmt & 4))
     hipLaunchKernelGGL((lstm_fwd_fused_kernel<WS_GATES_H2, true, true, true>), grid, block, 0, s, *a);
diff --git a/wesep_amd/csrc/lstm_pair.hip b/wesep_amd/csrc/lstm_pair.hip
--- a/wesep_amd/csrc/lstm_pair.hip
+++ b/wesep_amd/csrc/lstm_pair.hip
@@ -189,9 +189,10 @@
       reinterpret_cast<unsigned long long*>(p.dbg_buf)[(step * 2 + role) * 8 + (k)] = __builtin_readcyclecounter(); \
   }
 
-template <int V, int GF = 0, int RF = 0>
+template <int V, int GF = 0, int RF = 0, bool C16 = false>
 __global__ __launch_bounds__(512, 2) void lstm_bwd_pair_kernel(const ws_lstm_pair_args p) {
   static_assert(RF == 0 || GF == WS_GATES_H2F, "the fp16 recurrence takes the scaled-fp16 d(gates) of WS_GATES_H2F");
+  static_assert(!C16 || RF >= 2, "the fp16 cell state comes with the resident-weight kernels");
   constexpr int PAIR_LDSK = pair_ldsk<RF>::value;
   __shared__ __attribute__((aligned(16))) __bf16 bimg[RF ? 1 : 2][SQ * PR_ROW];
   constexpr int LDSK8 = 27;
@@ -227,6 +228,12 @@
     if constexpr (GF != 0) return bld8(hrs(t), gvo >> 1, (g * 64 + 2 * e) * 256);
     else return bld(grs(t), gvo, (g * 64 + 2 * e) * 512);
   };
+  typedef typename c_cell<C16>::type ccell;
+  auto c16rs = [&](int t) { return mkrsrc(p.cbuf + (long long)(tile * L + t) * (SQ * LH), SQ * 2 * LH * 2); };
+  auto ld_c = [&](int t, int e) -> ccell {
+    if constexpr (C16) return bld8(c16rs(t), cvo >> 1, e * 512);
+    else return bld(crs(p.cbuf, t), cvo, 2 * e * 512);
+  };
   const __amdgpu_buffer_rsrc_t xrs = __builtin_amdgcn_make_buffer_rsrc(
       reinterpret_cast<char*>(p.xchg) + (long long)pr * (4 * PR_XSLOT), 0, 4 * PR_XSLOT, 0x00020000);
   gu32* flags = (gu32*)(p.flags) + pr * 8;
@@ -279,7 +286,8 @@
   f32x4* mineo = &rec[role ^ 1][(wx * 2) * 64 + lane];
 
   gcell n_i[2], n_f[2], n_g[2], n_o[2];
-  f32x4 n_dh[2], n_cp[2], c_cur[2], dc[2], mine[2];
+  f32x4 n_dh[2], dc[2], mine[2];
+  ccell n_cp[2], c_cur[2];
   const f32x4 zero4v = {0.f, 0.f, 0.f, 0.f};
   auto load_step = [&](int t, int e) {
     n_i[e] = ld_gate(t, 0, e);
@@ -288,7 +296,7 @@
     n_o[e] = ld_gate(t, 3, e);
     n_dh[e] = bld(crs(p.dhcat, t), cvo, 2 * e * 512);
     const int tp = d == 0 ? max(t - 1, 0) : min(t + 1, L - 1);
-    n_cp[e] = bld(crs(p.cbuf, tp), cvo, 2 * e * 512);
+    n_cp[e] = ld_c(tp, e);
   };
   unsigned sink = 0u;
   auto touch = [&](__amdgpu_buffer_rsrc_t r, int voff, int soff) {
@@ -301,7 +309,8 @@
 #pragma unroll
       for (int g = 0; g < 4; ++g) touch(hrs(t), gvo >> 1, (g * 64 + 2 * e) * 256);
       touch(crs(p.dhcat, t), cvo, 2 * e * 512);
-      touch(crs(p.cbuf, tp), cvo, 2 * e * 512);
+      if constexpr (C16) touch(c16rs(tp), cvo >> 1, e * 512);
+      else touch(crs(p.cbuf, tp), cvo, 2 * e * 512);
     }
   };
   {
@@ -309,7 +318,7 @@
 #pragma unroll
     for (int e = 0; e < 2; ++e) {
       load_step(t0, e);
-      c_cur[e] = bld(crs(p.cbuf, t0), cvo, 2 * e * 512);
+      c_cur[e] = ld_c(t0, e);
       dc[e] = mine[e] = zero4v;
     }
   }
@@ -345,12 +354,12 @@
       for (int r = 0; r < 4; ++r) {
         const float ig = vi[r], fg = vf[r], gg = vg[r], og = vo[r];
         const float dhv = dh_in<GF>(n_dh[e][r], dhr[r], dS);
-        const float tc = ftanh(c_cur[e][r]);
+        const float tc = ftanh(c_at(c_cur[e], r));
         const float dov = dhv * tc;
         const float dcv = dc[e][r] + dhv * og * (1.f - tc * tc);
         dc[e][r] = dcv * fg;
         pi[r] = dcv * gg * ig * (1.f - ig);
-        pf[r] = dcv * (has_prev ? n_cp[e][r] : 0.f) * fg * (1.f - fg);
+        pf[r] = dcv * (has_prev ? c_at(n_cp[e], r) : 0.f) * fg * (1.f - fg);
         pg[r] = dcv * ig * (1.f - gg * gg);
         po[r] = dov * og * (1.f - og);
       }
@@ -590,9 +599,13 @@
   WS_REQUIRE(a->gfmt >= WS_GATES_F32 && a->gfmt <= WS_GATES_H2F && (a->gfmt != WS_GATES_H2S || a->dgates) &&
                  (a->gfmt != WS_GATES_H2F || a->amax),
              "ws_lstm_bwd_pair: gfmt %d (WS_GATES_H2S needs dgates, WS_GATES_H2F needs amax)", a->gfmt);
-  WS_REQUIRE(a->rfmt == 0 || (a->rfmt >= 1 && a->rfmt <= 3 && a->gfmt == WS_GATES_H2F),
+  const int rfmt = a->rfmt & ~WS_LSTM_C16;
+  const bool c16 = (a->rfmt & WS_LSTM_C16) != 0;
+  WS_REQUIRE(rfmt == 0 || (rfmt >= 1 && rfmt <= 3 && a->gfmt == WS_GATES_H2F),
              "ws_lstm_bwd_pair: rfmt %d (1 / 2 / 3 = fp16 recurrence, fp16 + fp16 / fp16 + fp8 weights / + the lo term on the FP8 "
              "MFMA: WS_GATES_H2F only)", a->rfmt);
+  WS_REQUIRE(!c16 || ((rfmt == 2 || rfmt == 3) && !(a->dbg & 2048)),
+             "ws_lstm_bwd_pair: rfmt %d: the fp16 cell state (bit WS_LSTM_C16) goes with rfmt 2 / 3, no cycle stamps", a->rfmt);
   const int npair = 2 * ((a->nseq + SQ - 1) / SQ);
   static int cus = 0;
   if (!cus && hipDeviceGetAttribute(&cus, hipDeviceAttributeMultiprocessorCount, 0) != hipSuccess) cus = 0;
@@ -602,11 +615,19 @@
   hipStream_t s = (hipStream_t)stream;
   hipError_t e = hipMemsetAsync(a->flags, 0, ((size_t)npair * 8 + 8) * sizeof(unsigned), s);
   WS_REQUIRE(e == hipSuccess, "ws_lstm_bwd_pair: hipMemsetAsync failed");
-  if (a->rfmt != 0) {
+  if (rfmt != 0) {
     e = hipMemsetAsync(a->xchg, 0x01, (size_t)npair * 4 * PR_XSLOT, s);
     WS_REQUIRE(e == hipSuccess, "ws_lstm_bwd_pair: hipMemsetAsync failed");
   }
   ws_prof_begin(WS_PROF_LSTM_BWD, s);
+  if (c16) {
+    if (rfmt == 3 && (a->dbg & 8)) hipLaunchKernelGGL((lstm_bwd_pair_kernel<8, WS_GATES_H2F, 3, true>), dim3(grid), dim3(512), 0, s, *a);
+    else if (rfmt == 3) hipLaunchKernelGGL((lstm_bwd_pair_kernel<0, WS_GATES_H2F, 3, true>), dim3(grid), dim3(512), 0, s, *a);
+    else if (a->dbg & 8) hipLaunchKernelGGL((lstm_bwd_pair_kernel<8, WS_GATES_H2F, 2, true>), dim3(grid), dim3(512), 0, s, *a);
+    else hipLaunchKernelGGL((lstm_bwd_pair_kernel<0, WS_GATES_H2F, 2, true>), dim3(grid), dim3(512), 0, s, *a);
+    ws_prof_end(WS_PROF_LSTM_BWD, s);
+    return ws_check_launch("ws_lstm_bwd_pair");
+  }
   if (a->rfmt == 3) {
     WS_REQUIRE(!(a->dbg & 2048), "ws_lstm_bwd_pair: cycle stamps (dbg 2048) exist for rfmt 0 .. 2");
     if (a->dbg & 8) hipLaunchKernelGGL((lstm_bwd_pair_kernel<8, WS_GATES_H2F, 3>), dim3(grid), dim3(512), 0, s, *a);
diff --git a/wesep_amd/dev.py b/wesep_amd/dev.py
--- a/wesep_amd/dev.py
+++ b/wesep_amd/dev.py
@@ -388,8 +388,17 @@
                                    n_in, _p(wcat), _p(bcat), L.stream_ptr()), "ws_lstm_cat_ih")
 
 
-def _bptt_bytes(gfmt: int) -> int:
-    return {L.GATES_F32: 40, L.GATES_H2: 24, L.GATES_H2S: 32, L.GATES_H2F: 24}[gfmt]
+def c16_on(device) -> bool:
+    return device.type == "cuda" and torch.cuda.is_available() and os.environ.get("WESEP_C16", "1") != "0"
+
+
+C16_MAX_STEPS = 32768
+
+
+def _bptt_bytes(gfmt: int, c16=None) -> int:
+    if c16 is None:
+        c16 = gfmt == L.GATES_H2F and torch.cuda.is_available() and os.environ.get("WESEP_C16", "1") != "0"
+    return {L.GATES_F32: 40, L.GATES_H2: 24, L.GATES_H2S: 32, L.GATES_H2F: 24}[gfmt] - (2 if c16 else 0)
 
 
 def gates_fmt() -> int:
@@ -419,21 +428,21 @@
     return a
 
 
-def lstm_fwd(gates, cbuf, hcat, wpack, sm: SeqMap, mode=L.LSTM_BF16X3, run_if=None, gfmt=0, gates_in=None, h2p=False):
+def lstm_fwd(gates, cbuf, hcat, wpack, sm: SeqMap, mode=L.LSTM_BF16X3, run_if=None, gfmt=0, gates_in=None, h2p=False, c16=False):
     a = _lstm_args(gates, cbuf, hcat, wpack, sm, mode, run_if=run_if, gfmt=gfmt, gates_in=gates_in,
-                   rfmt=L.LSTM_FWD_H2P if h2p else 0)
+                   rfmt=(L.LSTM_FWD_H2P if h2p else 0) | (L.LSTM_C16 if c16 else 0))
     if run_if is None:
         u = ALG_LSTM_UNITS or L.LSTM_H
-        _alg("lstm_fwd", sm.nseq * sm.L * 2 * u * (16 + (2 if gfmt else 4) * 4 + 8), 2 * sm.nseq * sm.L * 2 * 4 * u * u)
+        _alg("lstm_fwd", sm.nseq * sm.L * 2 * u * (16 + (2 if gfmt else 4) * 4 + (6 if c16 else 8)), 2 * sm.nseq * sm.L * 2 * 4 * u * u)
     L.check(L.lib().ws_lstm_fwd(C.byref(a), L.stream_ptr()), "ws_lstm_fwd")
 
 
 def lstm_bwd(gates, cbuf, hcat, dhcat, wpack, sm: SeqMap, mode=L.LSTM_BF16X3, gfmt=0, dgates=None, run_if=None, amax=None,
-             rfmt=0, dxn=None, wxpack=None):
-    a = _lstm_args(gates, cbuf, hcat, wpack, sm, mode, dhcat, gfmt=gfmt, dgates=dgates, run_if=run_if, amax=amax, rfmt=rfmt,
-                   dxn=dxn, wxpack=wxpack)
+             rfmt=0, dxn=None, wxpack=None, c16=False):
+    a = _lstm_args(gates, cbuf, hcat, wpack, sm, mode, dhcat, gfmt=gfmt, dgates=dgates, run_if=run_if, amax=amax,
+                   rfmt=rfmt | (L.LSTM_C16 if c16 else 0), dxn=dxn, wxpack=wxpack)
     if run_if is None:
-        _alg("lstm_bwd", _bptt_bytes(gfmt) * sm.nseq * sm.L * 2 * (ALG_LSTM_UNITS or L.LSTM_H),
+        _alg("lstm_bwd", _bptt_bytes(gfmt, c16) * sm.nseq * sm.L * 2 * (ALG_LSTM_UNITS or L.LSTM_H),
              2 * sm.nseq * sm.L * 2 * 4 * (ALG_LSTM_UNITS or L.LSTM_H) ** 2)
     L.check(L.lib().ws_lstm_bwd(C.byref(a), L.stream_ptr()), "ws_lstm_bwd")
 
@@ -597,7 +606,7 @@
 
 
 def lstm_fwd_cluster2(gates, cbuf, hcat, xn, wcat, bcat, whh_f, whh_r, sm: SeqMap, status=None, dbg=0, dbg_buf=None, rfmt=None,
-                      h2p=False):
+                      h2p=False, c16=False):
     for n, t in (("gates", gates), ("cbuf", cbuf), ("hcat", hcat), ("xn", xn), ("wcat", wcat), ("bcat", bcat),
                  ("whh_f", whh_f), ("whh_r", whh_r)):
         _chk(t, n)
@@ -611,10 +620,10 @@
     a.xchg, a.tword = C.c_void_p(xchg.data_ptr()), C.c_void_p(tw.data_ptr())
     a.status = C.c_void_p((status if status is not None else sc.status).data_ptr())
     a.nseq, a.L, a.dbg = sm.nseq, sm.L, dbg
-    a.rfmt = (cluster2_rfmt() if rfmt is None else rfmt) | (2 if h2p else 0)
+    a.rfmt = (cluster2_rfmt() if rfmt is None else rfmt) | (2 if h2p else 0) | (4 if c16 else 0)
     a.dbg_buf = C.c_void_p(dbg_buf.data_ptr()) if dbg_buf is not None else None
     u = ALG_LSTM_UNITS or L.LSTM_H
-    _alg("lstm_fwd", sm.nseq * sm.L * (2 * u * 16 + 4 * 128), 2 * sm.nseq * sm.L * 2 * 4 * u * (u + 128))
+    _alg("lstm_fwd", sm.nseq * sm.L * (2 * u * (14 if c16 else 16) + 4 * 128), 2 * sm.nseq * sm.L * 2 * 4 * u * (u + 128))
     L.check(L.lib().ws_lstm_fwd_cluster2(C.byref(a), L.stream_ptr()), "ws_lstm_fwd_cluster2")
     return tw
 
@@ -649,7 +658,7 @@
 
 
 def lstm_bwd_pair(gates, cbuf, dhcat, wpack, sm: SeqMap, status=None, dbg=0, dbg_buf=None, gfmt=0, dgates=None,
-                  repairable=False, amax=None, rfmt=0):
+                  repairable=False, amax=None, rfmt=0, c16=False):
     for n, t in (("gates", gates), ("cbuf", cbuf), ("dhcat", dhcat), ("wpack", wpack), ("dgates", dgates)):
         _chk(t, n)
     npair = 2 * (-(-sm.nseq // 32))
@@ -663,8 +672,8 @@
     a.dbg_buf = C.c_void_p(dbg_buf.data_ptr()) if dbg_buf is not None else None
     a.gfmt, a.dgates = gfmt, _p(dgates)
     a.amax = C.c_void_p(amax.data_ptr()) if amax is not None else None
-    a.rfmt = rfmt
-    _alg("lstm_bwd", _bptt_bytes(gfmt) * sm.nseq * sm.L * 2 * (ALG_LSTM_UNITS or L.LSTM_H),
+    a.rfmt = rfmt | (L.LSTM_C16 if c16 else 0)
+    _alg("lstm_bwd", _bptt_bytes(gfmt, c16) * sm.nseq * sm.L * 2 * (ALG_LSTM_UNITS or L.LSTM_H),
              2 * sm.nseq * sm.L * 2 * 4 * (ALG_LSTM_UNITS or L.LSTM_H) ** 2)
     L.check(L.lib().ws_lstm_bwd_pair(C.byref(a), L.stream_ptr()), "ws_lstm_bwd_pair")
     return flags[npair * 8:npair * 8 + 1]
@@ -1242,15 +1251,16 @@
           _p(wih_f), _p(wih_r), _p(whh_f), _p(whh_r), _p(pack))
 
 
-def lstm_fwd_fused(gates, cbuf, hcat, xn, wpack, bias, sm: SeqMap, gfmt=0, hfmt=0):
+def lstm_fwd_fused(gates, cbuf, hcat, xn, wpack, bias, sm: SeqMap, gfmt=0, hfmt=0, c16=False):
     for n, t in (("gates", gates), ("cbuf", cbuf), ("hcat", hcat), ("xn", xn), ("wpack", wpack), ("bias", bias)):
         _chk(t, n)
     a = L.LstmFusedArgs()
     a.gates, a.cbuf, a.hcat, a.xn, a.wpack, a.bias = _p(gates), _p(cbuf), _p(hcat), _p(xn), _p(wpack), _p(bias)
     a.nseq, a.L, a.gfmt = sm.nseq, sm.L, gfmt
-    a.hfmt = hfmt | (2 if os.environ.get("WESEP_FUSED_DRAIN", "0") == "1" else 0)
+    a.hfmt = hfmt | (16 if c16 else 0) | (2 if os.environ.get("WESEP_FUSED_DRAIN", "0") == "1" else 0)
     u = ALG_LSTM_UNITS or L.LSTM_H
-    _alg("lstm_fwd", sm.nseq * sm.L * (2 * u * ((2 if gfmt else 4) * 4 + 8) + 4 * 128), 2 * sm.nseq * sm.L * 2 * 4 * u * (u + 128))
+    _alg("lstm_fwd", sm.nseq * sm.L * (2 * u * ((2 if gfmt else 4) * 4 + (6 if a.hfmt & 16 else 8)) + 4 * 128),
+         2 * sm.nseq * sm.L * 2 * 4 * u * (u + 128))
     L.check(L.lib().ws_lstm_fwd_fused(C.byref(a), L.stream_ptr()), "ws_lstm_fwd_fused")
 
 
```

Result: faster. 348.1 utterances/s, median of 6 (+1.2%).
